# deep-art-project/Music

Measured on AMD Instinct MI355X. Metric: audio samples/sec trained (whole node), 30-layer WaveNet @16kHz, higher is better.
Workload: dtype f32 (forward + recompute: f16 2-term split operands, 2^-22 per element; backward products: bf16 2-term split, 2^-17 per element, f32 range; 3 MFMA per product, f32 accumulate)

## Files before the change

### include/wavenet_hip.h

```cpp
#ifndef WAVENET_HIP_H
#define WAVENET_HIP_H
#include <stdint.h>
#ifdef __cplusplus
extern "C" {
#endif

typedef void* wn_stream_t;
enum { WN_F16X3 = 0, WN_F16X1 = 1, WN_BF16X3 = 2, WN_BF16X1 = 3 };
#define WN_ABI_VERSION 9
#define WN_CE_NUM_PARTIALS 1024
#define WN_GUARD_NUM_PARTIALS 256
#define WN_GUARD_PARTIALS_BYTES (WN_GUARD_NUM_PARTIALS * 12)
#define WN_GUARD_STATE_BYTES 48

int wn_version(void);
const char* wn_last_error(void);

int wn_pack_weights(const float* flat, const int32_t* idx, uint16_t* out, int n, int mode,
                    wn_stream_t stream);

int wn_chan_gemm(const float* in0, const float* in1, int64_t in_bstride, int in_pitch, int in_lo, int in_hi,
                 int shift0, int shift1, int ks0, int ks1, const uint16_t* wpack, int mt, int m_valid,
                 float* out, int64_t out_bstride, int out_pitch, int out_shift, const float* bias,
                 const float* resid, int64_t resid_bstride, int resid_pitch, int resid_lo,
                 const float* mask, int64_t mask_bstride, int mask_pitch,
                 int t_lo, int t_hi, int relu_in, int batch, int mode, wn_stream_t stream);

int wn_resblock_fwd(const float* x_in, float* x_out, float* z_out, int64_t x_bstride, int64_t z_bstride,
                    int pitch, const uint16_t* wfg, const uint16_t* wd, const float* bias_f,
                    const float* bias_g, const float* bias_d, int n_f, int n_d, int ch, int d,
                    int t_lo, int t_hi, int z_lo, int write_x, const float* cond, int64_t cond_bstride,
                    int cond_pitch, int cond_mode, int cond_le, int cond_q, const uint16_t* cond_pack,
                    int64_t cond_pack_bstride, const uint8_t* cond_idx, int64_t z_half_stride, int batch, int mode,
                    wn_stream_t stream);

int wn_resblock_bwd(const float* x_in, const float* dy, const float* dz, float* dfg, float* z,
                    int64_t x_bstride, int64_t dz_bstride, int64_t dfg_bstride, int64_t z_bstride,
                    int pitch, const uint16_t* wfg, const uint16_t* wdT, const float* bias_f,
                    const float* bias_g, int n_f, int ch, int d, int t_lo, int t_hi, int z_lo,
                    const float* cond, int64_t cond_bstride, int cond_pitch, int cond_mode, int cond_le, int cond_q,
                    int batch, int mode_fwd, int mode_bwd, wn_stream_t stream);

int wn_skip_epilogue_fwd(const float* z, int64_t z_bstride, int pitch, int ks_skip, const uint16_t* w_skip, const float* bias_skip,
                         float* u, float* h, int64_t s_bstride, const uint16_t* w_p1c, const float* bias_p1,
                         const uint16_t* w_p2c, const float* bias_p2, float* o, int64_t o_bstride, int o_pitch,
                         int s_valid, int q_valid, int t_lo, int t_hi, int batch, int mode, wn_stream_t stream);

int wn_skip_epilogue_bwd(const float* d_o, int64_t o_bstride, int o_pitch, const float* h, const float* u, int64_t s_bstride, int pitch,
                         float* d_h, float* d_u, float* d_z, int64_t z_bstride, const uint16_t* w_p2T, const uint16_t* w_p1Tc,
                         const uint16_t* w_skipTc, int mt_z, int z_valid, int s_valid, int t_lo, int t_hi, int batch, int mode,
                         wn_stream_t stream);

int wn_enc_resblock_fwd(const float* x_in, float* x_out, float* h_out, int64_t x_bstride, int64_t h_bstride, int pitch,
                        const uint16_t* wdil, const uint16_t* wd, const float* bias_dil, const float* bias_d, int n_h,
                        int n_d, int ch, int d, int t_lo, int t_hi, int batch, int mode, wn_stream_t stream);

int wn_enc_resblock_bwd(const float* x_in, const float* dy, const float* h, float* dh, int64_t x_bstride,
                        int64_t h_bstride, int64_t dh_bstride, int pitch, const uint16_t* wdT, int ch, int d, int t_lo,
                        int t_hi, int y_lo, float* slab_dil, float* slab_d, int batch, int mode_bwd, wn_stream_t stream);
int wn_enc_resblock_bwd_slabs(int t_lo, int t_hi, int batch);
int wn_enc_resblock_bwd_pq(const float* x_in, const float* p_in, const float* q_in, int dn, int p_lo, const float* h,
                           float* p_out, float* q_out, int64_t x_bstride, int64_t h_bstride, int pitch, const uint16_t* wdT,
                           const uint16_t* wpq, int ch, int d, int t_lo, int t_hi, float* slab_dil, float* slab_d, int chain,
                           int batch, int mode_bwd, wn_stream_t stream);

int wn_resblock_bwd_ms(const float* x_in, const float* dy, const float* dz, float* dfg, int64_t x_bstride,
                       int64_t dz_bstride, int64_t dfg_bstride, int pitch, const uint16_t* wfg, const uint16_t* wdT,
                       const float* bias_f, const float* bias_g, int n_f, int ch, int d, int t_lo, int t_hi, int z_lo,
                       float* slab_fg, float* slab_d, const float* cond, int64_t cond_bstride, int cond_pitch,
                       int cond_mode, int cond_le, int cond_q, int batch, int mode_fwd, int mode_bwd,
                       wn_stream_t stream);
int wn_resblock_bwd_ms_slabs(int t_lo, int t_hi, int batch);

#define WN_COND_IDX_PAD 64
int wn_resblock_bwd_pq(const float* x_in, const float* p_in, const float* q_in, int dn, int p_lo, const float* dz,
                       float* p_out, float* q_out, int64_t x_bstride, int64_t dz_bstride, int pitch, const uint16_t* wfg,
                       const uint16_t* wdT, const uint16_t* wpq, int ch, int d, int t_lo, int t_hi, int z_lo,
                       float* slab_fg, float* slab_d, const float* cond, int64_t cond_bstride, int cond_pitch, int cond_le,
                       const uint8_t* cond_idx, float* cslab, int64_t dz_half_stride, int chain, int batch, int mode_fwd,
                       int mode_bwd, wn_stream_t stream);
int wn_resblock_bwd_pq_chain_ok(int t_lo, int t_hi, int batch, int d);
int wn_resblock_bwd_pq_slabs(int t_lo, int t_hi, int batch, int d, int chain);
int wn_resblock_bwd_pq_chain_items(int t_lo, int t_hi, int batch, int d, int wg, int* out, int cap);
int wn_resblock_bwd_pq_cond_floats(int t_lo, int t_hi, int batch);
int wn_resblock_bwd_pq_cond_reduce(const float* cslab, const int64_t* slab_off, const int* t_lo, int n_launches, int t_hi, int batch,
                                   int cond_le, float* out, int64_t out_lstride, int64_t out_bstride, int out_pitch,
                                   wn_stream_t stream);
int wn_gate_fwd(const float* fg, int64_t fg_bstride, int dp, int rows, float* z, int64_t z_bstride, int pitch, int t_lo, int t_hi,
                int batch, wn_stream_t stream);
int wn_gate_bwd(const float* fg, int64_t fg_bstride, int dp, int rows, const float* dz, int64_t dz_bstride, float* dfg,
                int64_t dfg_bstride, int pitch, int t_lo, int t_hi, int batch, wn_stream_t stream);
int wn_chunk_softmax_fwd(const float* x, float* y, int64_t nrows, int q, wn_stream_t stream);
int wn_chunk_softmax_bwd(const float* y, const float* dy, float* dx, int64_t nrows, int q, wn_stream_t stream);
int wn_chunk_softmax_ce(const float* x, const int64_t* target, float* probs, float* dx, float* loss_part, int64_t nrows, int q,
                        float inv_n, wn_stream_t stream);
int wn_split16(const float* x, uint16_t* hi, uint16_t* lo, int64_t n, int is_bf16, wn_stream_t stream);
int wn_shift_add(const float* p, const float* q, float* out, int64_t bstride, int pitch, int rows, int dn, int p_lo,
                 int t_lo, int t_hi, int batch, wn_stream_t stream);

int wn_wgrad(const float* a, int64_t a_bstride, int a_pitch, int a_shift, int a_cols,
             const float* b0, const float* b1, int64_t b_bstride, int b_pitch, int b_shift0,
             int b_shift1, int b_cols, int nt_per_tap, int mt, int relu_b, float* c, int ldc,
             int64_t c_slab_stride, int t_lo, int t_hi, int chunk, int batch, int mode, wn_stream_t stream);
int wn_wgrad_slabs(int t_lo, int t_hi, int chunk, int batch);
int wn_causal_wgrad_codes(const int32_t* codes, int scrambled, const float* dx, const float* dx_q, int dn, int p_lo,
                          int64_t dx_bstride, int pitch, int ch, int q, int t, int batch, float* slab, wn_stream_t stream);
int wn_causal_wgrad_codes_slabs(int t, int batch);
int wn_causal_fwd_codes(const int32_t* codes, int scrambled, const float* wt, const float* bias, int n_rows, float* x0,
                        int64_t x_bstride, int pitch, int ch, int q, int t, int batch, wn_stream_t stream);
int wn_reduce_slabs(const int64_t* desc, int n_ops, int64_t total_vec, const float* slab, float* out,
                    wn_stream_t stream);

int wn_bias_grad(const float* a, int64_t a_bstride, int a_pitch, int a_shift, int rows, int t_lo,
                 int t_hi, int batch, float* out, wn_stream_t stream);

int wn_chunk_softmax256_fwd(const float* x, float* y, int64_t nrows, wn_stream_t stream);
int wn_chunk_softmax256_bwd(const float* y, const float* dy, float* dx, int64_t nrows, wn_stream_t stream);
int wn_chunk_softmax256_ce(const float* x, const int64_t* target, float* probs, float* dx,
                           float* loss_part, int64_t nrows, float inv_n, wn_stream_t stream);

int wn_adam_flat(float* p, const float* g, float* m, float* v, int64_t n, float lr, float beta1,
                 float beta2, float eps, float bias_corr1, float bias_corr2, float gscale,
                 wn_stream_t stream);
int wn_sgd_flat(float* p, const float* g, float* momentum_buf, int64_t n, float lr, float momentum, float gscale,
                int first_step, wn_stream_t stream);
int wn_rmsprop_flat(float* p, const float* g, float* square_avg, float* momentum_buf, int64_t n, float lr, float alpha,
                    float eps, float momentum, float gscale, wn_stream_t stream);
typedef struct wn_guard_state {
    float norm;
    float coef;
    uint32_t nonfinite;
    uint32_t skip;
    uint64_t n_taken;
    uint64_t n_clipped;
    uint64_t n_skipped;
    float bc1;
    float bc2;
} wn_guard_state;
int wn_grad_guard(const float* g, int64_t n, float gscale, float max_norm, int skip_nonfinite, float beta1, float beta2,
                  void* partials, wn_guard_state* state, wn_stream_t stream);
int wn_adam_flat_guarded(float* p, const float* g, float* m, float* v, int64_t n, float lr, float beta1, float beta2, float eps,
                         float gscale, const wn_guard_state* state, wn_stream_t stream);
int wn_sgd_flat_guarded(float* p, const float* g, float* momentum_buf, int64_t n, float lr, float momentum, float gscale,
                        const wn_guard_state* state, wn_stream_t stream);
int wn_rmsprop_flat_guarded(float* p, const float* g, float* square_avg, float* momentum_buf, int64_t n, float lr, float alpha,
                            float eps, float momentum, float gscale, const wn_guard_state* state, wn_stream_t stream);
int wn_ema_flat(float* ema, const float* p, int64_t n, float decay, int warmup, int64_t t, const wn_guard_state* state,
                wn_stream_t stream);
int wn_step_softmax(const float* x, int64_t x_bstride, int x_pitch, float* probs, int w, int q, int batch, wn_stream_t stream);
int wn_step_nll(const float* x, int64_t x_bstride, int x_pitch, const int64_t* target, float* dx, int64_t dx_bstride, int dx_pitch,
                float* probs, float* row_nll, int32_t* row_hit, float* loss_part, int w, int q, int batch, float inv_n,
                wn_stream_t stream);
int wn_win_step_softmax(const float* x, int64_t x_bstride, int x_pitch, float* probs, int w, int q, int batch, const int32_t* win_host,
                        int win_period, const int64_t* win_pos, int64_t win_pos0, wn_stream_t stream);
int wn_win_step_nll(const float* x, int64_t x_bstride, int x_pitch, const int64_t* target, float* dx, int64_t dx_bstride, int dx_pitch,
                    float* probs, float* row_nll, int32_t* row_hit, float* loss_part, int w, int q, int batch, float inv_n,
                    const int32_t* win_host, int win_period, const int64_t* win_pos, int64_t win_pos0, wn_stream_t stream);
int wn_cond_proj_fwd(const float* enc, const float* flat, int64_t w_off, int64_t b_off, int64_t stage_stride, int64_t wf_off,
                     int64_t bf_off, float* tab, float* tab_pair, float* enf, int n_stages, int dd, int ch, int sd, int bw, int le,
                     int batch, wn_stream_t stream);
int wn_cond_proj_bwd(const float* d_tab, int pair, const float* d_enf, const float* enc, const float* flat, int64_t w_off,
                     int64_t b_off, int64_t stage_stride, int64_t wf_off, int64_t bf_off, float* d_enc, float* flat_grad,
                     int n_stages, int dd, int ch, int sd, int bw, int le, int batch, wn_stream_t stream);
#define WN_GCOND_MAX_CHANNELS 512
int wn_gcond_proj_fwd(const float* enc, const float* flat, int64_t w_off, int64_t b_off, int64_t stage_stride, int64_t wf_off,
                      int64_t bf_off, float* tab, float* tab_pair, float* enf, int n_stages, int dd, int ch, int sd, int bw, int le,
                      int batch, const int32_t* cls, int64_t gw_off, int64_t gstage_stride, int64_t gwf_off, int64_t emb_off, int ge,
                      int n_cls, wn_stream_t stream);
int wn_gcond_proj_bwd(const float* d_tab, int pair, const float* d_enf, const float* enc, const float* flat, int64_t w_off,
                      int64_t b_off, int64_t stage_stride, int64_t wf_off, int64_t bf_off, float* d_enc, float* flat_grad,
                      int n_stages, int dd, int ch, int sd, int bw, int le, int batch, const int32_t* cls, int64_t gw_off,
                      int64_t gstage_stride, int64_t gwf_off, int64_t emb_off, int ge, int n_cls, wn_stream_t stream);
#define WN_VQ_NUM_PARTIALS 256
#define WN_VQ_MAX_CODES 1024
#define WN_VQ_MAX_WIDTH 512
int wn_vq_fwd(const float* enc, const float* flat, int64_t cb_off, float* q_out, int32_t* idx, int32_t* counts, float* loss_part, int K,
              int bw, int le, int batch, wn_stream_t stream);
int wn_vq_bwd(const float* enc, const int32_t* idx, const float* d_q, const float* flat, int64_t cb_off, float beta, float g_scale,
              float* d_enc, float* flat_grad, int K, int bw, int le, int batch, wn_stream_t stream);
int wn_vq_lookup(const int32_t* idx, const float* flat, int64_t cb_off, float* q_out, int32_t* bad, int K, int bw, int le, int batch,
                 wn_stream_t stream);
#define WN_VQ_EMA_WORK_BYTES 4112
int wn_vq_bwd_stats(const float* enc, const int32_t* idx, const float* d_q, const float* flat, int64_t cb_off, float beta, float g_scale,
                    float* d_enc, float* flat_grad, float* stat, int K, int bw, int le, int batch, wn_stream_t stream);
int wn_vq_ema_update(float* flat, int64_t cb_off, const float* stat, float* state, void* work, int32_t* info, int K, int bw,
                     float decay, float eps, float restart, const wn_guard_state* guard_state, wn_stream_t stream);
#define WN_RVQ_MAX_STAGES 8
int wn_rvq_fwd(const float* enc, const float* flat, int64_t cb_off, float* q_out, int32_t* idx, int32_t* counts, float* res,
               float* loss_part, int S, int K, int bw, int le, int batch, wn_stream_t stream);
int wn_rvq_bwd(const float* enc, const int32_t* idx, const float* res, const float* d_q, const float* flat, int64_t cb_off, float beta,
               float g_scale, float* d_enc, float* flat_grad, int S, int K, int bw, int le, int batch, wn_stream_t stream);
int wn_rvq_bwd_stats(const float* enc, const int32_t* idx, const float* res, const float* d_q, const float* flat, int64_t cb_off, float beta,
                     float g_scale, float* d_enc, float* flat_grad, float* stat, int S, int K, int bw, int le, int batch,
                     wn_stream_t stream);
int wn_rvq_ema_update(float* flat, int64_t cb_off, const float* stat, float* state, void* work, int32_t* info, int S, int K, int bw,
                      float decay, float eps, float restart, const wn_guard_state* guard_state, wn_stream_t stream);
int wn_rvq_lookup(const int32_t* idx, const float* flat, int64_t cb_off, float* q_out, int32_t* bad, int S, int stages, int K, int bw,
                  int le, int batch, wn_stream_t stream);
int wn_rvq_fwd_n(const float* enc, const float* flat, int64_t cb_off, const int32_t* nstage, float* q_out, int32_t* idx, int32_t* counts,
                 float* res, float* loss_part, int S, int K, int bw, int le, int batch, wn_stream_t stream);
int wn_rvq_bwd_n(const float* enc, const int32_t* idx, const float* res, const int32_t* nstage, const float* d_q, const float* flat,
                 int64_t cb_off, float beta, float g_scale, float* d_enc, float* flat_grad, int S, int K, int bw, int le, int batch,
                 wn_stream_t stream);
int wn_rvq_bwd_stats_n(const float* enc, const int32_t* idx, const float* res, const int32_t* nstage, const float* d_q, const float* flat,
                       int64_t cb_off, float beta, float g_scale, float* d_enc, float* flat_grad, float* stat, int S, int K, int bw, int le,
                       int batch, wn_stream_t stream);
int wn_rvq_lookup_n(const int32_t* idx, const int32_t* nstage, const float* flat, int64_t cb_off, float* q_out, int32_t* bad, int S, int K,
                    int bw, int le, int batch, wn_stream_t stream);
int wn_coll_available(void);
int wn_comm_unique_id(char* id128);
int wn_comm_create(int nranks, int rank, const char* id128, void** comm);
int wn_comm_destroy(void* comm);
int wn_allreduce_flat(void* comm, float* buf, int64_t n, wn_stream_t stream);
int wn_gather_grads(const float* packed, const int32_t* idx, float* flat_grad, int n, wn_stream_t stream);
int wn_gather_grads2(const float* packed, const int32_t* idx, const int32_t* idx2, float* flat_grad, int n, wn_stream_t stream);

int wn_cond_expand(const float* tab, int64_t tab_bstride, int tab_pitch, int rows, int t_lo, int t_hi, int mode, int le, int q,
                   float* out, int64_t out_bstride, int out_pitch, int batch, wn_stream_t stream);
int wn_cond_grad(const float* in, int64_t in_bstride, int in_pitch, int rows, int t_lo, int t_hi, int mode, int le,
                 int q, float* out, int64_t out_bstride, int out_pitch, int batch, wn_stream_t stream);
int wn_avgpool_bwd(const float* denc, int64_t denc_bstride, int denc_pitch, int t0, int pool, int n_out, int rows,
                   float* out, int64_t out_bstride, int out_pitch, int t_hi, int batch, wn_stream_t stream);

int wn_avgpool(const float* in, int64_t in_bstride, int in_pitch, int t0, int pool, int n_out, int rows,
               float* out, int64_t out_bstride, int out_pitch, int batch, wn_stream_t stream);

int wn_onehot(const int32_t* codes, float* out, int batch, int q, int t, int scrambled, wn_stream_t stream);

int wn_mulaw_encode_tbl(const float* audio, const float* thresholds, uint8_t* codes, int64_t n, wn_stream_t stream);
int wn_mulaw_decode_lut(const uint8_t* codes, const float* table, float* audio, int64_t n, wn_stream_t stream);
int wn_mulaw_encode_q(const float* audio, const float* thresholds, int q, int32_t* codes, int64_t n, wn_stream_t stream);
int wn_mulaw_decode_q(const int32_t* codes, const float* table, int q, float* audio, int64_t n, wn_stream_t stream);

int wn_decode(int n_layers, int R, int D, int S, int Q, const int32_t* dilations_host, const int64_t* q_off_host,
              float* queues, const float* w_causal, const float* b_causal, const float* w_layers,
              int64_t layer_stride, const float* b_layers, const float* w_p1, const float* b_p1,
              const float* w_p2, const float* b_p2, const float* note0, const float* prev0, float* note_out,
              float* prev_out, const int32_t* forced, int32_t* codes_out, float* probs_out, int64_t step0,
              int n_steps, int push_input, uint64_t* sync, wn_stream_t stream);

int wn_decode_batch(int n_layers, int R, int D, int S, int Q, const int32_t* dilations_host, const int64_t* q_off_host,
                    float* queues, const float* w_causal, const float* b_causal, const float* w_layers,
                    int64_t layer_stride, const float* b_layers, const float* w_p1, const float* b_p1,
                    const float* w_p2, const float* b_p2, const float* note0, const float* prev0, float* note_out,
                    float* prev_out, const int32_t* forced, int32_t* codes_out, float* probs_out, int64_t step0,
                    int n_steps, int push_input, uint64_t* sync, int n_utt, int64_t queues_ustride, float temperature,
                    uint64_t seed, wn_stream_t stream);
int64_t wn_decode_sync_granules(int n_layers, int D, int S);
int wn_decode_batch_pk(int n_layers, int R, int D, int S, int Q, const int32_t* dilations_host, const int64_t* q_off_host,
                       float* queues, const float* w_causal, const float* b_causal, const float* w_layers,
                       int64_t layer_stride, const float* b_layers, const float* w_p1, const float* b_p1,
                       const float* w_p2, const float* b_p2, const float* note0, const float* prev0, float* note_out,
                       float* prev_out, const int32_t* forced, int32_t* codes_out, float* probs_out, int64_t step0,
                       int n_steps, int push_input, uint64_t* sync, int n_utt, int64_t queues_ustride, float temperature,
                       uint64_t seed, const uint16_t* pk, int64_t pk_fg0, int64_t pk_d0, int64_t pk_lstride, int64_t pk_skip,
                       int64_t pk_p1, int64_t pk_p2, wn_stream_t stream);
int wn_decode_batch_fw(int filter_width, int n_layers, int R, int D, int S, int Q, const int32_t* dilations_host,
                       const int64_t* q_off_host, float* queues, const float* w_causal, const float* b_causal,
                       const float* w_layers, int64_t layer_stride, const float* b_layers, const float* w_p1, const float* b_p1,
                       const float* w_p2, const float* b_p2, const float* note0, const float* prev0, float* note_out,
                       float* prev_out, const int32_t* forced, int32_t* codes_out, float* probs_out, int64_t step0,
                       int n_steps, int push_input, uint64_t* sync, int n_utt, int64_t queues_ustride, float temperature,
                       uint64_t seed, const uint16_t* pk, int64_t pk_fg0, int64_t pk_d0, int64_t pk_lstride, int64_t pk_skip,
                       int64_t pk_p1, int64_t pk_p2, wn_stream_t stream);
// ... 48 lines not shown
```

### music_amd/_lib.py

```python
import ctypes
import os

_HERE = os.path.dirname(os.path.abspath(__file__))
LIB_PATH = os.environ.get("WAVENET_HIP_LIB") or os.path.join(_HERE, "libwavenet_hip.so")

F16X3, F16X1, BF16X3, BF16X1 = 0, 1, 2, 3
MODE_NAMES = {"f16x3": F16X3, "f16x1": F16X1, "bf16x3": BF16X3, "bf16x1": BF16X1}
CE_NUM_PARTIALS = 1024
ABI_VERSION = 9
GUARD_NUM_PARTIALS = 256
GUARD_PARTIALS_BYTES = GUARD_NUM_PARTIALS * 12
VQ_NUM_PARTIALS = 256
VQ_MAX_CODES, VQ_MAX_WIDTH = 1024, 512
VQ_EMA_WORK_BYTES = 16 + 4 * VQ_MAX_CODES
RVQ_MAX_STAGES = 8
GCOND_MAX_CHANNELS = 512

_p = ctypes.c_void_p
_i = ctypes.c_int
_l = ctypes.c_int64
_f = ctypes.c_float
_DEC_HEAD = [_i] * 5 + [_p] * 6 + [_l] + [_p] * 12 + [_l, _i, _i, _p]
_DEC_BATCH = [_i, _l, _f, _l]
_DEC_PK = [_p] + [_l] * 6
_DEC_COND = [_p, _l, _p, _l, _p, _p, _i, _l]
_DEC_SAMP = [_p, _i, _f]
_DEC_WIN = [_p, _i, _l]
_SAMPLE_LOGITS = [_p, _l, _i, _l, _p, _f, _l, _i, _f, _l, _p, _p, _p]

SIGNATURES = {
    "wn_version": [],
    "wn_pack_weights": [_p, _p, _p, _i, _i, _p],
    "wn_chan_gemm": [_p, _p, _l, _i, _i, _i, _i, _i, _i, _i, _p, _i, _i,
                     _p, _l, _i, _i, _p,
                     _p, _l, _i, _i,
                     _p, _l, _i,
                     _i, _i, _i, _i, _i, _p],
    "wn_skip_epilogue_fwd": [_p, _l, _i, _i, _p, _p, _p, _p, _l, _p, _p, _p, _p, _p, _l, _i, _i, _i, _i, _i, _i, _i, _p],
    "wn_skip_epilogue_bwd": [_p, _l, _i, _p, _p, _l, _i, _p, _p, _p, _l, _p, _p, _p, _i, _i, _i, _i, _i, _i, _i, _p],
    "wn_resblock_fwd": [_p, _p, _p, _l, _l, _i, _p, _p, _p, _p, _p, _i, _i, _i, _i,
                        _i, _i, _i, _i, _p, _l, _i, _i, _i, _i, _p, _l, _p, _l, _i, _i, _p],
    "wn_enc_resblock_fwd": [_p, _p, _p, _l, _l, _i, _p, _p, _p, _p, _i, _i, _i, _i, _i, _i, _i, _i, _p],
    "wn_enc_resblock_bwd": [_p, _p, _p, _p, _l, _l, _l, _i, _p, _i, _i, _i, _i, _i, _p, _p, _i, _i, _p],
    "wn_enc_resblock_bwd_slabs": [_i, _i, _i],
    "wn_enc_resblock_bwd_pq": [_p, _p, _p, _i, _i, _p, _p, _p, _l, _l, _i, _p, _p, _i, _i, _i, _i, _p, _p, _i, _i, _i, _p],
    "wn_avgpool": [_p, _l, _i, _i, _i, _i, _i, _p, _l, _i, _i, _p],
    "wn_resblock_bwd": [_p, _p, _p, _p, _p, _l, _l, _l, _l, _i, _p, _p, _p, _p, _i, _i, _i, _i, _i, _i,
                        _p, _l, _i, _i, _i, _i, _i, _i, _i, _p],
    "wn_cond_expand": [_p, _l, _i, _i, _i, _i, _i, _i, _i, _p, _l, _i, _i, _p],
    "wn_cond_grad": [_p, _l, _i, _i, _i, _i, _i, _i, _i, _p, _l, _i, _i, _p],
    "wn_avgpool_bwd": [_p, _l, _i, _i, _i, _i, _i, _p, _l, _i, _i, _i, _p],
    "wn_wgrad": [_p, _l, _i, _i, _i, _p, _p, _l, _i, _i, _i, _i, _i, _i, _i, _p, _i,
                 _l, _i, _i, _i, _i, _i, _p],
    "wn_wgrad_slabs": [_i, _i, _i, _i],
    "wn_resblock_bwd_ms": [_p, _p, _p, _p, _l, _l, _l, _i, _p, _p, _p, _p, _i, _i, _i, _i, _i, _i, _p, _p,
                           _p, _l, _i, _i, _i, _i, _i, _i, _i, _p],
    "wn_resblock_bwd_ms_slabs": [_i, _i, _i],
    "wn_resblock_bwd_pq": [_p, _p, _p, _i, _i, _p, _p, _p, _l, _l, _i, _p, _p, _p, _i, _i, _i, _i, _i, _p, _p,
                           _p, _l, _i, _i, _p, _p, _l, _i, _i, _i, _i, _p],
    "wn_resblock_bwd_pq_chain_ok": [_i, _i, _i, _i],
    "wn_resblock_bwd_pq_slabs": [_i, _i, _i, _i, _i],
    "wn_resblock_bwd_pq_chain_items": [_i, _i, _i, _i, _i, _p, _i],
    "wn_resblock_bwd_pq_cond_floats": [_i, _i, _i],
    "wn_resblock_bwd_pq_cond_reduce": [_p, _p, _p, _i, _i, _i, _i, _p, _l, _l, _i, _p],
    "wn_split16": [_p, _p, _p, _l, _i, _p],
    "wn_shift_add": [_p, _p, _p, _l, _i, _i, _i, _i, _i, _i, _i, _p],
    "wn_causal_wgrad_codes": [_p, _i, _p, _p, _i, _i, _l, _i, _i, _i, _i, _i, _p, _p],
    "wn_causal_wgrad_codes_slabs": [_i, _i],
    "wn_causal_fwd_codes": [_p, _i, _p, _p, _i, _p, _l, _i, _i, _i, _i, _i, _p],
    "wn_reduce_slabs": [_p, _i, _l, _p, _p, _p],
    "wn_bias_grad": [_p, _l, _i, _i, _i, _i, _i, _i, _p, _p],
    "wn_chunk_softmax256_fwd": [_p, _p, _l, _p],
    "wn_chunk_softmax256_bwd": [_p, _p, _p, _l, _p],
    "wn_chunk_softmax256_ce": [_p, _p, _p, _p, _p, _l, _f, _p],
    "wn_gate_fwd": [_p, _l, _i, _i, _p, _l, _i, _i, _i, _i, _p],
    "wn_gate_bwd": [_p, _l, _i, _i, _p, _l, _p, _l, _i, _i, _i, _i, _p],
    "wn_chunk_softmax_fwd": [_p, _p, _l, _i, _p],
    "wn_chunk_softmax_bwd": [_p, _p, _p, _l, _i, _p],
    "wn_chunk_softmax_ce": [_p, _p, _p, _p, _p, _l, _i, _f, _p],
    "wn_adam_flat": [_p, _p, _p, _p, _l, _f, _f, _f, _f, _f, _f, _f, _p],
    "wn_sgd_flat": [_p, _p, _p, _l, _f, _f, _f, _i, _p],
    "wn_rmsprop_flat": [_p, _p, _p, _p, _l, _f, _f, _f, _f, _f, _p],
    "wn_grad_guard": [_p, _l, _f, _f, _i, _f, _f, _p, _p, _p],
    "wn_adam_flat_guarded": [_p, _p, _p, _p, _l, _f, _f, _f, _f, _f, _p, _p],
    "wn_sgd_flat_guarded": [_p, _p, _p, _l, _f, _f, _f, _p, _p],
    "wn_rmsprop_flat_guarded": [_p, _p, _p, _p, _l, _f, _f, _f, _f, _f, _p, _p],
    "wn_ema_flat": [_p, _p, _l, _f, _i, _l, _p, _p],
    "wn_step_softmax": [_p, _l, _i, _p, _i, _i, _i, _p],
    "wn_step_nll": [_p, _l, _i, _p, _p, _l, _i, _p, _p, _p, _p, _i, _i, _i, _f, _p],
    "wn_win_step_softmax": [_p, _l, _i, _p, _i, _i, _i, _p, _i, _p, _l, _p],
    "wn_win_step_nll": [_p, _l, _i, _p, _p, _l, _i, _p, _p, _p, _p, _i, _i, _i, _f, _p, _i, _p, _l, _p],
    "wn_cond_proj_fwd": [_p, _p, _l, _l, _l, _l, _l, _p, _p, _p, _i, _i, _i, _i, _i, _i, _i, _p],
    "wn_cond_proj_bwd": [_p, _i, _p, _p, _p, _l, _l, _l, _l, _l, _p, _p, _i, _i, _i, _i, _i, _i, _i, _p],
    "wn_gcond_proj_fwd": [_p, _p, _l, _l, _l, _l, _l, _p, _p, _p, _i, _i, _i, _i, _i, _i, _i, _p, _l, _l, _l, _l, _i, _i, _p],
    "wn_gcond_proj_bwd": [_p, _i, _p, _p, _p, _l, _l, _l, _l, _l, _p, _p, _i, _i, _i, _i, _i, _i, _i, _p, _l, _l, _l, _l, _i, _i, _p],
    "wn_vq_fwd": [_p, _p, _l, _p, _p, _p, _p, _i, _i, _i, _i, _p],
    "wn_vq_bwd": [_p, _p, _p, _p, _l, _f, _f, _p, _p, _i, _i, _i, _i, _p],
    "wn_vq_lookup": [_p, _p, _l, _p, _p, _i, _i, _i, _i, _p],
    "wn_vq_bwd_stats": [_p, _p, _p, _p, _l, _f, _f, _p, _p, _p, _i, _i, _i, _i, _p],
    "wn_vq_ema_update": [_p, _l, _p, _p, _p, _p, _i, _i, _f, _f, _f, _p, _p],
    "wn_rvq_fwd": [_p, _p, _l, _p, _p, _p, _p, _p, _i, _i, _i, _i, _i, _p],
    "wn_rvq_bwd": [_p, _p, _p, _p, _p, _l, _f, _f, _p, _p, _i, _i, _i, _i, _i, _p],
    "wn_rvq_bwd_stats": [_p, _p, _p, _p, _p, _l, _f, _f, _p, _p, _p, _i, _i, _i, _i, _i, _p],
    "wn_rvq_ema_update": [_p, _l, _p, _p, _p, _p, _i, _i, _i, _f, _f, _f, _p, _p],
    "wn_rvq_lookup": [_p, _p, _l, _p, _p, _i, _i, _i, _i, _i, _i, _p],
    "wn_rvq_fwd_n": [_p, _p, _l, _p, _p, _p, _p, _p, _p, _i, _i, _i, _i, _i, _p],
    "wn_rvq_bwd_n": [_p, _p, _p, _p, _p, _p, _l, _f, _f, _p, _p, _i, _i, _i, _i, _i, _p],
    "wn_rvq_bwd_stats_n": [_p, _p, _p, _p, _p, _p, _l, _f, _f, _p, _p, _p, _i, _i, _i, _i, _i, _p],
    "wn_rvq_lookup_n": [_p, _p, _p, _l, _p, _p, _i, _i, _i, _i, _i, _p],
    "wn_coll_available": [],
    "wn_comm_unique_id": [_p],
    "wn_comm_create": [_i, _i, _p, _p],
    "wn_comm_destroy": [_p],
    "wn_allreduce_flat": [_p, _p, _l, _p],
    "wn_gather_grads": [_p, _p, _p, _i, _p],
    "wn_gather_grads2": [_p, _p, _p, _p, _i, _p],
    "wn_onehot": [_p, _p, _i, _i, _i, _i, _p],
    "wn_mulaw_encode_tbl": [_p, _p, _p, _l, _p],
    "wn_mulaw_decode_lut": [_p, _p, _p, _l, _p],
    "wn_mulaw_encode_q": [_p, _p, _i, _p, _l, _p],
    "wn_mulaw_decode_q": [_p, _p, _i, _p, _l, _p],
    "wn_decode": _DEC_HEAD + [_p],
    "wn_decode_batch": _DEC_HEAD + _DEC_BATCH + [_p],
    "wn_decode_sync_granules": [_i, _i, _i],
    "wn_decode_batch_pk": _DEC_HEAD + _DEC_BATCH + _DEC_PK + [_p],
    "wn_decode_batch_fw": [_i] + _DEC_HEAD + _DEC_BATCH + _DEC_PK + [_p],
    "wn_decode_batch_cond": [_i] + _DEC_HEAD + _DEC_BATCH + _DEC_PK + _DEC_COND + [_p],
    "wn_decode_batch_samp": [_i] + _DEC_HEAD + _DEC_BATCH + _DEC_PK + _DEC_COND + _DEC_SAMP + [_p],
    "wn_sample_logits": _SAMPLE_LOGITS + [_p],
    "wn_win_decode_batch": [_i] + _DEC_HEAD + _DEC_BATCH + _DEC_PK + _DEC_COND + _DEC_SAMP + _DEC_WIN + [_p],
    "wn_win_sample_logits": _SAMPLE_LOGITS + _DEC_WIN + [_p],
}


class Sampling(ctypes.Structure):
    _fields_ = [("temperature", ctypes.c_float), ("top_p", ctypes.c_float), ("top_k", ctypes.c_int32),
                ("stream", ctypes.c_uint32), ("seed", ctypes.c_uint64)]


class GuardState(ctypes.Structure):
    _fields_ = [("norm", ctypes.c_float), ("coef", ctypes.c_float), ("nonfinite", ctypes.c_uint32), ("skip", ctypes.c_uint32),
                ("n_taken", ctypes.c_uint64), ("n_clipped", ctypes.c_uint64), ("n_skipped", ctypes.c_uint64),
                ("bc1", ctypes.c_float), ("bc2", ctypes.c_float)]


_lib = None


class WavenetHipError(RuntimeError):
    pass


def cpu_quota():
    try:
        q, per = open("/sys/fs/cgroup/cpu.max").read().split()[:2]
        return None if q == "max" else max(1, -(-int(q) // int(per)))
    except (OSError, ValueError):
        pass
    try:
        q = int(open("/sys/fs/cgroup/cpu/cpu.cfs_quota_us").read())
        per = int(open("/sys/fs/cgroup/cpu/cpu.cfs_period_us").read())
        return None if q <= 0 else max(1, -(-q // per))
    except (OSError, ValueError):
        return None


class StepThrottle:

    def __init__(self):
        self.depth = int(os.environ.get("WN_MAX_STEPS_IN_FLIGHT", "4"))
        self._ev = []

    def enter(self):
        if self.depth > 0 and len(self._ev) >= self.depth:
            self._ev.pop(0).synchronize()

    def leave(self):
        if self.depth > 0:
            import torch
            ev = torch.cuda.Event()
            ev.record()
            self._ev.append(ev)


def local_world_size(env=None):
    env = os.environ if env is None else env
    try:
        return max(1, int(env.get("LOCAL_WORLD_SIZE", "1")))
    except ValueError:
        return 1


def thread_budget(quota, local_world, cpus=None):
    total = quota if quota is not None else (cpus if cpus is not None else (os.cpu_count() or 1))
    return max(1, -(-int(total) // max(1, int(local_world))))


def respect_cpu_quota():
    import sys
    import torch
    if os.environ.get("WN_KEEP_TORCH_THREADS", "0") == "1":
        return
    q, lw = cpu_quota(), local_world_size()
    if q is None and lw == 1:
        return
    n = thread_budget(q, lw)
    if torch.get_num_threads() > n:
        print("music_amd: torch intra-op threads %d -> %d (%s shared by %d rank(s) of this host; WN_KEEP_TORCH_THREADS=1 keeps torch's "
              "own setting)" % (torch.get_num_threads(), n, "the container's CPU quota of %d" % q if q is not None else
                                "%d CPUs" % (os.cpu_count() or 1), lw), file=sys.stderr)
        torch.set_num_threads(n)


def load():
    global _lib
    if _lib is not None:
        return _lib
    if not os.path.exists(LIB_PATH):
        raise WavenetHipError(
            "libwavenet_hip.so not found at %s - build it with `python -c 'import __graft_entry__ as g; "
            "g.build()'` or `make -C music_amd/csrc`; there is no CPU fallback" % LIB_PATH)
    import torch
    lib = ctypes.CDLL(LIB_PATH)
    for name, args in SIGNATURES.items():
        try:
            fn = getattr(lib, name)
        except AttributeError:
            raise WavenetHipError("%s does not export %s: it was built from older sources - rebuild it (`make -C music_amd/csrc`)"
                                  % (LIB_PATH, name)) from None
        fn.argtypes = args
        fn.restype = ctypes.c_int
    lib.wn_decode_sync_granules.restype = ctypes.c_int64
    lib.wn_last_error.argtypes = []
    lib.wn_last_error.restype = ctypes.c_char_p
    if lib.wn_version() != ABI_VERSION:
        raise WavenetHipError("libwavenet_hip.so ABI version %d != expected %d" % (lib.wn_version(), ABI_VERSION))
    _lib = lib
    respect_cpu_quota()
    return lib


def wgrad_slabs(t_lo, t_hi, chunk, batch):
    return load().wn_wgrad_slabs(t_lo, t_hi, chunk, batch)


def causal_codes_slabs(t, batch):
    return load().wn_causal_wgrad_codes_slabs(t, batch)


COND_IDX_PAD = 64


def ms_slabs(t_lo, t_hi, batch):
    return load().wn_resblock_bwd_ms_slabs(t_lo, t_hi, batch)


def pq_chain_ok(t_lo, t_hi, batch, d):
    return bool(load().wn_resblock_bwd_pq_chain_ok(t_lo, t_hi, batch, d))


def pq_slabs(t_lo, t_hi, batch, d, chain):
    return load().wn_resblock_bwd_pq_slabs(t_lo, t_hi, batch, d, 1 if chain else 0)


def enc_slabs(t_lo, t_hi, batch):
    return load().wn_enc_resblock_bwd_slabs(t_lo, t_hi, batch)


def decode_sync_granules(n_layers, D, S):
    return int(load().wn_decode_sync_granules(n_layers, D, S))


def call(name, *args):
    lib = load()
    rc = getattr(lib, name)(*args)
    if rc != 0:
        raise WavenetHipError("%s failed (%d): %s" % (name, rc, lib.wn_last_error().decode()))


def ptr(t, offset=0):
    if t is None:
        return None
    return t.data_ptr() + offset * t.element_size()


def stream():
    import torch
    return torch.cuda.current_stream().cuda_stream


_side_streams = {}


def side_stream(device):
    import os
    import torch
    dev = torch.device(device)
    key = dev.index if dev.index is not None else torch.cuda.current_device()
    st = _side_streams.get(key)
    if st is None:
        st = _side_streams[key] = torch.cuda.Stream(device=dev, priority=-1)
    return st
```

### music_amd/csrc/wn_api.hip

```cpp
#include <stdio.h>
#include <stdlib.h>
#include <string.h>
#include "../../include/wavenet_hip.h"
#include "wn_common.h"
#include "wn_kernels.h"

static_assert(WN_COND_IDX_PAD == WN_PQ_IDX_PAD, "public and kernel-side pad of the bucket bytes differ");
static thread_local char g_err[512] = "";

int wn_set_error(hipError_t e, const char* file, int line) {
    snprintf(g_err, sizeof(g_err), "HIP error %d (%s) at %s:%d", (int)e, hipGetErrorString(e), file, line);
    return -1;
}
int wn_tile_origin(int t_lo) { return t_lo & ~63; }

int wn_num_cus() {
    static std::atomic<int> cus{0};
    int v = cus.load(std::memory_order_relaxed);
    if (v > 0) return v;
    int dev = 0;
    hipDeviceProp_t pr;
    if (hipGetDevice(&dev) != hipSuccess || hipGetDeviceProperties(&pr, dev) != hipSuccess || pr.multiProcessorCount <= 0) return 256;
    cus.store(pr.multiProcessorCount, std::memory_order_relaxed);
    return pr.multiProcessorCount;
}

int wn_xcd_swizzle_enabled() { return 1; }

int wn_set_error_msg(int code, const char* msg) {
    snprintf(g_err, sizeof(g_err), "%s", msg);
    return code;
}

static int wn_null_error(const char* fn, const char* names, int which) {
    const char* b = names;
    for (int i = 0; i < which && *b; ++b)
        if (*b == ',') ++i;
    while (*b == ' ') ++b;
    int len = 0;
    while (b[len] && b[len] != ',') ++len;
    snprintf(g_err, sizeof(g_err), "%s: argument '%.*s' must not be NULL", fn, len, b);
    return -4;
}
#define WN_REQUIRE(fn, ...)                                                          \
    do {                                                                             \
        const void* wn_req_[] = {__VA_ARGS__};                                       \
        for (int wn_i_ = 0; wn_i_ < (int)(sizeof(wn_req_) / sizeof(wn_req_[0])); ++wn_i_) \
            if (!wn_req_[wn_i_]) return wn_null_error(fn, #__VA_ARGS__, wn_i_);      \
    } while (0)

static_assert(WN_F16X3 == WN_MODE_F16X3 && WN_F16X1 == WN_MODE_F16X1 && WN_BF16X3 == WN_MODE_BF16X3 &&
              WN_BF16X1 == WN_MODE_BF16X1, "mode enums out of sync");
static_assert(WN_CE_NUM_PARTIALS == WN_CE_PARTIALS, "partials out of sync");
static_assert(WN_VQ_NUM_PARTIALS == WN_VQ_PARTIALS && WN_VQ_MAX_CODES == WN_DEC_MAX_Q, "vq constants out of sync");
static_assert(WN_VQ_MAX_CODES == WN_VQ_MAX_K && WN_VQ_EMA_WORK_BYTES == WN_VQ_EMA_WORK, "vq ema constants out of sync");
static_assert(WN_RVQ_MAX_STAGES == WN_RVQ_MAX_S, "rvq constants out of sync");

enum : unsigned {
    DEC_FW = 1,
    DEC_COND = 2,
    DEC_SAMP = 4,
    DEC_WIN = 8,
};

static int decode_refuse(const char* fn, const char* text) {
    snprintf(g_err, sizeof(g_err), "%s: %s", fn, text);
    return -4;
}

static int win_checked(const char* fn, const int32_t* win_host, int win_period, int64_t win_pos0, int Q, int& period, int& pos0,
                       int (&lo)[WN_WIN_MAX], int (&hi)[WN_WIN_MAX]) {
    if (win_period < 0 || win_period > WN_WIN_MAX) return decode_refuse(fn, "'win_period' must be 0 (no windows) .. 16 pairs");
    if (win_period > 0 && !win_host) return decode_refuse(fn, "'win_host' is NULL with win_period > 0");
    for (int j = 0; j < win_period; ++j)
        if (win_host[2 * j] < 0 || win_host[2 * j + 1] > Q || win_host[2 * j] >= win_host[2 * j + 1]) {
            snprintf(g_err, sizeof(g_err), "%s: 'win_host' pair %d is (%d, %d): every window needs 0 <= lo < hi <= Q", fn, j,
                     (int)win_host[2 * j], (int)win_host[2 * j + 1]);
            return -4;
        }
    if (win_pos0 < 0) return decode_refuse(fn, "'win_pos0' (stream position of the first step) must be >= 0");
    period = win_period;
    pos0 = win_period > 0 ? (int)(win_pos0 % win_period) : 0;
    for (int j = 0; j < win_period; ++j) { lo[j] = win_host[2 * j]; hi[j] = win_host[2 * j + 1]; }
    return 0;
}

static int decode_checked(const char* fn, unsigned checks, int64_t sync_ustride, int filter_width, int n_layers, int R, int D, int S,
                          int Q, const int32_t* dilations_host, const int64_t* q_off_host, float* queues, const float* w_causal,
                          const float* b_causal, const float* w_layers, int64_t layer_stride, const float* b_layers,
                          const float* w_p1, const float* b_p1, const float* w_p2, const float* b_p2, const float* note0,
                          const float* prev0, float* note_out, float* prev_out, const int32_t* forced, int32_t* codes_out,
                          float* probs_out, int64_t step0, int n_steps, int push_input, uint64_t* sync, int n_utt,
                          int64_t queues_ustride, float temperature, uint64_t seed, const uint16_t* pk, int64_t pk_fg0,
                          int64_t pk_d0, int64_t pk_lstride, int64_t pk_skip, int64_t pk_p1, int64_t pk_p2, const float* cond_fg,
                          int64_t cond_fg_ustride, const float* cond_p1, int64_t cond_p1_ustride, const int32_t* c_shift_host,
                          const int32_t* c_q_host, int le, int64_t pos0, const wn_sampling* samp, int top_k, float top_p,
                          const int32_t* win_host, int win_period, int64_t win_pos0, wn_stream_t stream) {
    const bool layers_ok = n_layers >= 1 && n_layers <= WN_DEC_MAX_LAYERS;
    if ((checks & DEC_SAMP) && !samp) {
        if (!(top_p >= 0.0f)) return decode_refuse(fn, "'top_p' must be a number >= 0 (0 or >= 1: no nucleus filter)");
        if (top_k < 0) return decode_refuse(fn, "'top_k' must be >= 0 (0 or >= Q: no top-k filter)");
    }
    if ((checks & DEC_FW) && filter_width < 1) return decode_refuse(fn, "filter_width must be >= 1");
    if (!push_input) {
        if (checks & DEC_COND) return decode_refuse(fn, "conditioned decode exists for the corrected recurrence only; pass push_input = 1");
        if ((checks & DEC_FW) && filter_width != 2)
            return decode_refuse(fn, "the as-written queue push (push_input = 0) exists for filter_width 2 only; pass push_input = 1 "
                                     "(the corrected recurrence)");
    }
    if ((checks & DEC_COND) && le < 1) return decode_refuse(fn, "le (columns of a conditioning table) must be >= 1");
    if ((checks & DEC_FW) && (Q < 1 || Q > WN_DEC_MAX_Q)) return decode_refuse(fn, "1 <= Q <= 1024 quantisation channels");
    if (checks & DEC_COND) {
        if (!layers_ok) return decode_refuse(fn, "1..64 layers supported");
        if (cond_fg || cond_p1) {
            if (!c_shift_host || !c_q_host)
                return decode_refuse(fn, "a conditioning table needs the schedule arrays 'c_shift_host' and 'c_q_host' (n_layers + 1 "
                                         "entries each)");
            for (int i = 0; i <= n_layers; ++i)
                if (c_q_host[i] < 0) return decode_refuse(fn, "c_q[i] must be >= 0 (stretch factor, or 0 = tile)");
        }
    }
    if ((checks & DEC_FW) && n_utt > 0 && n_steps > 0) {
        WN_REQUIRE(fn, note0, note_out, codes_out);
        if (filter_width > 1) WN_REQUIRE(fn, prev0, prev_out);
    }
    WnDecodeArgs a;
    memset(&a, 0, sizeof(a));
    if (checks & DEC_WIN) {
        const int rc = win_checked(fn, win_host, win_period, win_pos0, Q, a.win_period, a.win_pos0, a.win_lo, a.win_hi);
        if (rc) return rc;
    }
    if (n_utt <= 0) return 0;
    if (!layers_ok) return decode_refuse("wn_decode", "1..64 layers supported");
    WN_REQUIRE("wn_decode", dilations_host, q_off_host);
    if (n_steps > 0) WN_REQUIRE("wn_decode", queues, w_causal, w_layers, w_p1, w_p2, sync);
    a.n_layers = n_layers; a.R = R; a.D = D; a.S = S; a.Q = Q; a.fw = filter_width;
    for (int i = 0; i < n_layers; ++i) { a.dil[i] = dilations_host[i]; a.q_off[i] = q_off_host[i]; }
    a.queues = queues; a.w_causal = w_causal; a.b_causal = b_causal; a.w_layers = w_layers; a.layer_stride = layer_stride;
    a.b_layers = b_layers; a.w_p1 = w_p1; a.b_p1 = b_p1; a.w_p2 = w_p2; a.b_p2 = b_p2;
    a.note0 = note0; a.prev0 = prev0; a.note_out = note_out; a.prev_out = prev_out; a.forced = forced;
    a.codes_out = codes_out; a.probs_out = probs_out; a.step0 = step0; a.n_steps = n_steps; a.push_input = push_input;
    a.dbg = 0;
    a.sync = reinterpret_cast<unsigned long long*>(sync);
    a.sync_ustride = sync_ustride;
    a.n_utt = n_utt; a.queues_ustride = queues_ustride;
    a.sample = temperature > 0.0f ? 1 : 0; a.inv_temp = temperature > 0.0f ? 1.0f / temperature : 1.0f; a.seed = seed;
    a.samp = reinterpret_cast<const WnSampling*>(samp); a.top_k = top_k; a.top_p = top_p;
    a.pk_skip = -1;
    a.cond_fg = cond_fg; a.cond_fg_ustride = cond_fg_ustride; a.cond_p1 = cond_p1; a.cond_p1_ustride = cond_p1_ustride;
    a.le = le; a.pos0 = pos0;
    if (cond_fg || cond_p1)
        for (int i = 0; i <= n_layers; ++i) { a.c_shift[i] = c_shift_host[i]; a.c_q[i] = c_q_host[i]; }
    const bool any_bias = b_layers || b_causal || b_p1 || b_p2;
    const bool post_pk = (S == 256 || S == 512) && Q == 256 && pk_skip >= 0 && pk_p1 >= 0 && pk_p2 >= 0;
    if (pk && R == 64 && D == 64 && (post_pk || !any_bias)) {
        a.pk = pk; a.pk_fg0 = pk_fg0; a.pk_d0 = pk_d0; a.pk_lstride = pk_lstride;
        if (post_pk) { a.pk_skip = pk_skip; a.pk_p1 = pk_p1; a.pk_p2 = pk_p2; }
    }
    return wn_launch_decode(a, (hipStream_t)stream);
}

static int sample_checked(const char* fn, bool win, const float* logits, int64_t n, int Q, int64_t ld, const wn_sampling* samp,
                          float temperature, uint64_t seed, int top_k, float top_p, int64_t step0, const float* u, int32_t* codes,
                          float* probs, const int32_t* win_host, int win_period, int64_t win_pos0, wn_stream_t stream) {
    if (Q < 1 || Q > WN_DEC_MAX_Q) return decode_refuse(fn, "1 <= 'Q' <= 1024 entries per row");
    if (n < 0) return decode_refuse(fn, "'n' (rows) must be >= 0");
    if (ld < Q) return decode_refuse(fn, "'ld' (row stride) must be >= Q");
    if (!samp) {
        if (!(top_p >= 0.0f)) return decode_refuse(fn, "'top_p' must be a number >= 0 (0 or >= 1: no nucleus filter)");
        if (top_k < 0) return decode_refuse(fn, "'top_k' must be >= 0 (0 or >= Q: no top-k filter)");
    }
    WnWin w;
    memset(&w, 0, sizeof(w));
    if (win) {
        const int rc = win_checked(fn, win_host, win_period, win_pos0, Q, w.period, w.pos0, w.lo, w.hi);
        if (rc) return rc;
    }
    if (n == 0) return 0;
    WN_REQUIRE(fn, logits, codes);
    return wn_launch_sample_logits(logits, (long)n, Q, (long)ld, reinterpret_cast<const WnSampling*>(samp), temperature, seed, top_k,
                                   top_p, (long)step0, u, codes, probs, w, (hipStream_t)stream);
}

extern "C" {

int wn_version(void) { return WN_ABI_VERSION; }
const char* wn_last_error(void) { return g_err; }

int wn_pack_weights(const float* flat, const int32_t* idx, uint16_t* out, int n, int mode, wn_stream_t stream) {
    if (n % 512 != 0) return wn_set_error_msg(-4, "wn_pack_weights: n must be a multiple of 512");
    if (n > 0) WN_REQUIRE("wn_pack_weights", flat, idx, out);
    return wn_launch_pack(flat, idx, out, n, wn_mode_is_bf16(mode), wn_mode_ns(mode), (hipStream_t)stream);
}

int wn_chan_gemm(const float* in0, const float* in1, int64_t in_bstride, int in_pitch, int in_lo, int in_hi,
                 int shift0, int shift1, int ks0, int ks1, const uint16_t* wpack, int mt, int m_valid,
                 float* out, int64_t out_bstride, int out_pitch, int out_shift, const float* bias,
                 const float* resid, int64_t resid_bstride, int resid_pitch, int resid_lo,
                 const float* mask, int64_t mask_bstride, int mask_pitch,
                 int t_lo, int t_hi, int relu_in, int batch, int mode, wn_stream_t stream) {
    if (ks0 <= 0 || (ks1 > 0 && !in1) || mt <= 0) return wn_set_error_msg(-4, "wn_chan_gemm: bad shape");
    if (batch > 0 && t_hi > t_lo) WN_REQUIRE("wn_chan_gemm", in0, wpack, out);
    WnGemmArgs a;
    memset(&a, 0, sizeof(a));
    a.in0 = in0; a.in1 = ks1 > 0 ? in1 : nullptr; a.in_bstride = in_bstride; a.in_pitch = in_pitch; a.in_lo = in_lo; a.in_hi = in_hi;
    a.shift0 = shift0; a.shift1 = shift1; a.ks0 = ks0; a.ks1 = ks1 > 0 ? ks1 : 0; a.wpack = wpack; a.mt = mt; a.m_valid = m_valid;
    a.out = out; a.out_bstride = out_bstride; a.out_pitch = out_pitch; a.out_shift = out_shift; a.bias = bias;
    a.resid = resid; a.resid_bstride = resid_bstride; a.resid_pitch = resid_pitch; a.resid_lo = resid_lo;
    a.mask = mask; a.mask_bstride = mask_bstride; a.mask_pitch = mask_pitch;
    a.t_lo = t_lo; a.t_hi = t_hi; a.relu_in = relu_in;
    return wn_launch_gemm(a, batch, mode, (hipStream_t)stream);
}

int wn_skip_epilogue_fwd(const float* z, int64_t z_bstride, int pitch, int ks_skip, const uint16_t* w_skip, const float* bias_skip,
                         float* u, float* h, int64_t s_bstride, const uint16_t* w_p1c, const float* bias_p1,
                         const uint16_t* w_p2c, const float* bias_p2, float* o, int64_t o_bstride, int o_pitch,
                         int s_valid, int q_valid, int t_lo, int t_hi, int batch, int mode, wn_stream_t stream) {
    if (pitch % 4 != 0) return wn_set_error_msg(-4, "wn_skip_epilogue_fwd: pitch must be a multiple of 4");
    if (s_valid <= 0 || s_valid > 256 || q_valid <= 0 || q_valid > 256)
        return wn_set_error_msg(-4, "wn_skip_epilogue_fwd: at most 256 skip and 256 quantisation channels (wn_chan_gemm covers the rest)");
    if (batch > 0 && t_hi > t_lo) WN_REQUIRE("wn_skip_epilogue_fwd", z, w_skip, u, h, w_p1c, w_p2c, o);
    WnEpiFwdArgs a;
    memset(&a, 0, sizeof(a));
    a.z = z; a.z_bstride = z_bstride; a.pitch = pitch; a.ks_skip = ks_skip; a.w_skip = w_skip; a.bias_s = bias_skip;
    a.u = u; a.h = h; a.s_bstride = s_bstride; a.w_p1c = w_p1c; a.bias_1 = bias_p1; a.w_p2c = w_p2c; a.bias_2 = bias_p2;
    a.o = o; a.o_bstride = o_bstride; a.o_pitch = o_pitch; a.s_valid = s_valid; a.q_valid = q_valid; a.t_lo = t_lo; a.t_hi = t_hi;
    return wn_launch_skip_epilogue_fwd(a, batch, mode, (hipStream_t)stream);
}

int wn_skip_epilogue_bwd(const float* d_o, int64_t o_bstride, int o_pitch, const float* h, const float* u, int64_t s_bstride, int pitch,
                         float* d_h, float* d_u, float* d_z, int64_t z_bstride, const uint16_t* w_p2T, const uint16_t* w_p1Tc,
                         const uint16_t* w_skipTc, int mt_z, int z_valid, int s_valid, int t_lo, int t_hi, int batch, int mode,
                         wn_stream_t stream) {
    if (pitch % 4 != 0) return wn_set_error_msg(-4, "wn_skip_epilogue_bwd: pitch must be a multiple of 4");
    if (s_valid <= 0 || s_valid > 256) return wn_set_error_msg(-4, "wn_skip_epilogue_bwd: at most 256 skip channels");
    if (batch > 0 && t_hi > t_lo) WN_REQUIRE("wn_skip_epilogue_bwd", d_o, h, u, d_h, d_u, d_z, w_p2T, w_p1Tc, w_skipTc);
    WnEpiBwdArgs a;
    memset(&a, 0, sizeof(a));
    a.d_o = d_o; a.o_bstride = o_bstride; a.o_pitch = o_pitch; a.h = h; a.u = u; a.s_bstride = s_bstride; a.pitch = pitch;
    a.d_h = d_h; a.d_u = d_u; a.d_z = d_z; a.z_bstride = z_bstride; a.w_p2T = w_p2T; a.w_p1Tc = w_p1Tc; a.w_skipTc = w_skipTc;
    a.mt_z = mt_z; a.z_valid = z_valid; a.s_valid = s_valid; a.t_lo = t_lo; a.t_hi = t_hi;
    return wn_launch_skip_epilogue_bwd(a, batch, mode, (hipStream_t)stream);
}

int wn_enc_resblock_fwd(const float* x_in, float* x_out, float* h_out, int64_t x_bstride, int64_t h_bstride, int pitch,
                        const uint16_t* wdil, const uint16_t* wd, const float* bias_dil, const float* bias_d, int n_h,
                        int n_d, int ch, int d, int t_lo, int t_hi, int batch, int mode, wn_stream_t stream) {
    if (pitch % 4 != 0) return wn_set_error_msg(-4, "wn_enc_resblock_fwd: pitch must be a multiple of 4");
    if (t_lo < d + 1) return wn_set_error_msg(-4, "wn_enc_resblock_fwd: t_lo must be >= d + 1");
    if (batch > 0 && t_hi > t_lo) WN_REQUIRE("wn_enc_resblock_fwd", x_in, x_out, h_out, wdil, wd);
    WnResArgs a;
    memset(&a, 0, sizeof(a));
    a.x_in = x_in; a.x_out = x_out; a.z_out = h_out; a.x_bstride = x_bstride; a.z_bstride = h_bstride; a.pitch = pitch;
    a.wfg = wdil; a.wd = wd; a.bias_f = bias_dil; a.bias_g = nullptr; a.bias_d = bias_d; a.n_f = n_h; a.n_d = n_d;
    a.d = d; a.t_lo = t_lo; a.t_hi = t_hi; a.z_lo = t_lo; a.write_x = 1;
    return wn_launch_enc_resblock_fwd(a, ch, batch, mode, (hipStream_t)stream);
}

int wn_resblock_fwd(const float* x_in, float* x_out, float* z_out, int64_t x_bstride, int64_t z_bstride,
                    int pitch, const uint16_t* wfg, const uint16_t* wd, const float* bias_f,
                    const float* bias_g, const float* bias_d, int n_f, int n_d, int ch, int d,
                    int t_lo, int t_hi, int z_lo, int write_x, const float* cond, int64_t cond_bstride,
                    int cond_pitch, int cond_mode, int cond_le, int cond_q, const uint16_t* cond_pack,
                    int64_t cond_pack_bstride, const uint8_t* cond_idx, int64_t z_half_stride, int batch, int mode,
                    wn_stream_t stream) {
    if (pitch % 4 != 0) return wn_set_error_msg(-4, "wn_resblock_fwd: pitch must be a multiple of 4");
    if (cond && (cond_le <= 0 || (cond_mode == 1 && cond_q <= 0) || (cond_mode != 1 && cond_mode != 2)))
        return wn_set_error_msg(-4, "wn_resblock_fwd: bad conditioning arguments");
    if (t_lo < d + 1) return wn_set_error_msg(-4, "wn_resblock_fwd: t_lo must be >= d + 1");
    if (batch > 0 && t_hi > t_lo) {
        WN_REQUIRE("wn_resblock_fwd", x_in, wfg, wd, z_out);
        if (write_x) WN_REQUIRE("wn_resblock_fwd", x_out);
    }
    WnResArgs a;
    memset(&a, 0, sizeof(a));
    a.x_in = x_in; a.x_out = x_out; a.z_out = z_out; a.x_bstride = x_bstride; a.z_bstride = z_bstride; a.pitch = pitch;
    a.wfg = wfg; a.wd = wd; a.bias_f = bias_f; a.bias_g = bias_g; a.bias_d = bias_d; a.n_f = n_f; a.n_d = n_d;
    a.d = d; a.t_lo = t_lo; a.t_hi = t_hi; a.z_lo = z_lo; a.write_x = write_x;
    a.cond = cond; a.cond_bstride = cond_bstride; a.cond_pitch = cond_pitch; a.cond_mode = cond_mode;
    a.cond_le = cond_le; a.cond_q = cond_q;
    if (cond && cond_pack && cond_idx) { a.cond_pack = cond_pack; a.cond_pack_bstride = cond_pack_bstride; a.cond_idx = cond_idx; }
    if (z_half_stride && ch != 64) return wn_set_error_msg(-4, "wn_resblock_fwd: z_half_stride is for two 32-channel clips on the 64-channel block");
    a.z_half = z_half_stride;
    return wn_launch_resblock_fwd(a, ch, batch, mode, (hipStream_t)stream);
}

int wn_resblock_bwd(const float* x_in, const float* dy, const float* dz, float* dfg, float* z,
                    int64_t x_bstride, int64_t dz_bstride, int64_t dfg_bstride, int64_t z_bstride,
                    int pitch, const uint16_t* wfg, const uint16_t* wdT, const float* bias_f,
                    const float* bias_g, int n_f, int ch, int d, int t_lo, int t_hi, int z_lo,
                    const float* cond, int64_t cond_bstride, int cond_pitch, int cond_mode, int cond_le, int cond_q,
                    int batch, int mode_fwd, int mode_bwd, wn_stream_t stream) {
    if (pitch % 4 != 0) return wn_set_error_msg(-4, "wn_resblock_bwd: pitch must be a multiple of 4");
    if (batch > 0 && t_hi > t_lo) {
        WN_REQUIRE("wn_resblock_bwd", x_in, dz, dfg, wfg);
        if (dy) WN_REQUIRE("wn_resblock_bwd", wdT);
    }
    WnResBwdArgs a;
    memset(&a, 0, sizeof(a));
    a.x_in = x_in; a.dy = dy; a.dz = dz; a.dfg = dfg; a.z = z;
    a.x_bstride = x_bstride; a.dz_bstride = dz_bstride; a.dfg_bstride = dfg_bstride; a.z_bstride = z_bstride; a.pitch = pitch;
    a.wfg = wfg; a.wdT = wdT; a.bias_f = bias_f; a.bias_g = bias_g; a.n_f = n_f;
    a.d = d; a.t_lo = t_lo; a.t_hi = t_hi; a.z_lo = z_lo;
    a.cond = cond; a.cond_bstride = cond_bstride; a.cond_pitch = cond_pitch; a.cond_mode = cond_mode;
    a.cond_le = cond_le; a.cond_q = cond_q;
    return wn_launch_resblock_bwd(a, ch, batch, mode_fwd, mode_bwd, (hipStream_t)stream);
}

int wn_wgrad(const float* a_, int64_t a_bstride, int a_pitch, int a_shift, int a_cols,
             const float* b0, const float* b1, int64_t b_bstride, int b_pitch, int b_shift0,
             int b_shift1, int b_cols, int nt_per_tap, int mt, int relu_b, float* c, int ldc,
             int64_t c_slab_stride, int t_lo, int t_hi, int chunk, int batch, int mode, wn_stream_t stream) {
    if (c_slab_stride < (int64_t)mt * 16 * ldc) return wn_set_error_msg(-4, "wn_wgrad: slab stride smaller than C");
    if (batch > 0 && t_hi > t_lo) WN_REQUIRE("wn_wgrad", a_, b0, c);
    WnWgradArgs a;
    memset(&a, 0, sizeof(a));
    a.a = a_; a.a_bstride = a_bstride; a.a_pitch = a_pitch; a.a_shift = a_shift; a.a_cols = a_cols;
    a.b0 = b0; a.b1 = b1; a.b_bstride = b_bstride; a.b_pitch = b_pitch; a.b_shift0 = b_shift0; a.b_shift1 = b_shift1; a.b_cols = b_cols;
    a.nt_per_tap = nt_per_tap; a.mt = mt; a.relu_b = relu_b; a.c = c; a.ldc = ldc; a.c_slab_stride = c_slab_stride;
    a.t_lo = t_lo; a.t_hi = t_hi; a.chunk = chunk;
    return wn_launch_wgrad(a, batch, mode, (hipStream_t)stream);
}

int wn_wgrad_slabs(int t_lo, int t_hi, int chunk, int batch) { return wn_wgrad_num_slabs(t_lo, t_hi, chunk, batch); }

int wn_reduce_slabs(const int64_t* desc, int n_ops, int64_t total_vec, const float* slab, float* out, wn_stream_t stream) {
    if (n_ops > 0 && total_vec > 0) WN_REQUIRE("wn_reduce_slabs", desc, slab, out);
    return wn_launch_reduce_slabs(reinterpret_cast<const long*>(desc), n_ops, total_vec, slab, out, (hipStream_t)stream);
}

int wn_bias_grad(const float* a, int64_t a_bstride, int a_pitch, int a_shift, int rows, int t_lo,
                 int t_hi, int batch, float* out, wn_stream_t stream) {
    if (batch > 0 && t_hi > t_lo && rows > 0) WN_REQUIRE("wn_bias_grad", a, out);
    return wn_launch_bias_grad(a, a_bstride, a_pitch, a_shift, rows, t_lo, t_hi, batch, out, (hipStream_t)stream);
}

int wn_chunk_softmax256_fwd(const float* x, float* y, int64_t nrows, wn_stream_t stream) {
    if (nrows > 0) WN_REQUIRE("wn_chunk_softmax256_fwd", x, y);
    return wn_launch_softmax_fwd(x, y, nrows, (hipStream_t)stream);
}
int wn_chunk_softmax256_bwd(const float* y, const float* dy, float* dx, int64_t nrows, wn_stream_t stream) {
    if (nrows > 0) WN_REQUIRE("wn_chunk_softmax256_bwd", y, dy, dx);
    return wn_launch_softmax_bwd(y, dy, dx, nrows, (hipStream_t)stream);
}
int wn_chunk_softmax256_ce(const float* x, const int64_t* target, float* probs, float* dx,
                           float* loss_part, int64_t nrows, float inv_n, wn_stream_t stream) {
    if (nrows > 0) WN_REQUIRE("wn_chunk_softmax256_ce", x, target);
    return wn_launch_softmax_ce(x, target, probs, dx, loss_part, nrows, inv_n, (hipStream_t)stream);
}
int wn_adam_flat(float* p, const float* g, float* m, float* v, int64_t n, float lr, float beta1,
                 float beta2, float eps, float bias_corr1, float bias_corr2, float gscale, wn_stream_t stream) {
    if (n > 0) WN_REQUIRE("wn_adam_flat", p, g, m, v);
    return wn_launch_adam(p, g, m, v, n, lr, beta1, beta2, eps, bias_corr1, bias_corr2, gscale, (hipStream_t)stream);
}
int wn_sgd_flat(float* p, const float* g, float* momentum_buf, int64_t n, float lr, float momentum, float gscale, int first_step,
                wn_stream_t stream) {
    if (momentum != 0.f && !momentum_buf) return wn_set_error_msg(-4, "wn_sgd_flat: momentum needs its buffer");
    if (n > 0) WN_REQUIRE("wn_sgd_flat", p, g);
    return wn_launch_sgd(p, g, momentum_buf, n, lr, momentum, gscale, first_step, (hipStream_t)stream);
}
int wn_rmsprop_flat(float* p, const float* g, float* square_avg, float* momentum_buf, int64_t n, float lr, float alpha, float eps,
                    float momentum, float gscale, wn_stream_t stream) {
    if (!square_avg || (momentum > 0.f && !momentum_buf)) return wn_set_error_msg(-4, "wn_rmsprop_flat: missing state buffer");
    if (n > 0) WN_REQUIRE("wn_rmsprop_flat", p, g);
    return wn_launch_rmsprop(p, g, square_avg, momentum_buf, n, lr, alpha, eps, momentum, gscale, (hipStream_t)stream);
}

int wn_grad_guard(const float* g, int64_t n, float gscale, float max_norm, int skip_nonfinite, float beta1, float beta2, void* partials,
                  wn_guard_state* state, wn_stream_t stream) {
    WN_REQUIRE("wn_grad_guard", partials, state);
    if (n > 0) WN_REQUIRE("wn_grad_guard", g);
    if (n < 0) return wn_set_error_msg(-4, "wn_grad_guard: n is negative");
    if (((uintptr_t)g & 3) || ((uintptr_t)partials & 7) || ((uintptr_t)state & 7))
        return wn_set_error_msg(-4, "wn_grad_guard: g needs 4-byte, partials and state 8-byte alignment");
    return wn_launch_grad_guard(g, n, gscale, max_norm, skip_nonfinite, beta1, beta2, partials, state, (hipStream_t)stream);
}
int wn_adam_flat_guarded(float* p, const float* g, float* m, float* v, int64_t n, float lr, float beta1, float beta2, float eps,
                         float gscale, const wn_guard_state* state, wn_stream_t stream) {
    if (n > 0) WN_REQUIRE("wn_adam_flat_guarded", p, g, m, v, state);
    return wn_launch_adam_guarded(p, g, m, v, n, lr, beta1, beta2, eps, gscale, state, (hipStream_t)stream);
}
int wn_sgd_flat_guarded(float* p, const float* g, float* momentum_buf, int64_t n, float lr, float momentum, float gscale,
                        const wn_guard_state* state, wn_stream_t stream) {
    if (momentum != 0.f && !momentum_buf) return wn_set_error_msg(-4, "wn_sgd_flat_guarded: momentum needs its buffer");
    if (n > 0) WN_REQUIRE("wn_sgd_flat_guarded", p, g, state);
    return wn_launch_sgd_guarded(p, g, momentum_buf, n, lr, momentum, gscale, state, (hipStream_t)stream);
}
int wn_rmsprop_flat_guarded(float* p, const float* g, float* square_avg, float* momentum_buf, int64_t n, float lr, float alpha, float eps,
                            float momentum, float gscale, const wn_guard_state* state, wn_stream_t stream) {
    if (!square_avg || (momentum > 0.f && !momentum_buf)) return wn_set_error_msg(-4, "wn_rmsprop_flat_guarded: missing state buffer");
    if (n > 0) WN_REQUIRE("wn_rmsprop_flat_guarded", p, g, state);
    return wn_launch_rmsprop_guarded(p, g, square_avg, momentum_buf, n, lr, alpha, eps, momentum, gscale, state, (hipStream_t)stream);
}
int wn_ema_flat(float* ema, const float* p, int64_t n, float decay, int warmup, int64_t t, const wn_guard_state* state,
                wn_stream_t stream) {
    if (n < 0) return wn_set_error_msg(-4, "wn_ema_flat: n is negative");
    if (n == 0) return 0;
    WN_REQUIRE("wn_ema_flat", ema, p);
    if ((uintptr_t)ema % 4 != 0) return wn_set_error_msg(-4, "wn_ema_flat: argument 'ema' needs 4-byte alignment");
    if ((uintptr_t)p % 4 != 0) return wn_set_error_msg(-4, "wn_ema_flat: argument 'p' needs 4-byte alignment");
    if ((uintptr_t)state % 8 != 0) return wn_set_error_msg(-4, "wn_ema_flat: argument 'state' needs 8-byte alignment");
    if (!(decay >= 0.f && decay < 1.f)) return wn_set_error_msg(-4, "wn_ema_flat: argument 'decay' must lie in [0, 1)");
    if (!state && t < 1) return wn_set_error_msg(-4, "wn_ema_flat: argument 't' counts the updates from 1 when state is NULL");
    return wn_launch_ema(ema, p, n, decay, warmup ? 1 : 0, t, state, (hipStream_t)stream);
}
static int step_checked(const char* fn, const void* x, int64_t x_bstride, int x_pitch, int w, int q, int batch) {
    char msg[160];
    const char* bad = nullptr;
    if (batch < 0) bad = "'batch' must be >= 0";
    else if (w < 0) bad = "'w' must be >= 0";
    else if (q < 1 || q > 1024) bad = "'q' must lie in [1, 1024]";
    else if (x_pitch < w) bad = "'x_pitch' must be >= w";
    else if (x_bstride < (int64_t)q * x_pitch) bad = "'x_bstride' must be >= q * x_pitch";
    if (bad) {
        snprintf(msg, sizeof(msg), "%s: argument %s", fn, bad);
        return wn_set_error_msg(-4, msg);
    }
    if (batch > 0 && w > 0) WN_REQUIRE(fn, x);
    return 0;
}
int wn_step_softmax(const float* x, int64_t x_bstride, int x_pitch, float* probs, int w, int q, int batch, wn_stream_t stream) {
    if (int rc = step_checked("wn_step_softmax", x, x_bstride, x_pitch, w, q, batch)) return rc;
    if (batch == 0 || w == 0) return 0;
    WN_REQUIRE("wn_step_softmax", probs);
    return wn_launch_step_nll(x, (long)x_bstride, x_pitch, nullptr, nullptr, 0, 0, probs, nullptr, nullptr, nullptr, w, q, batch, 0.f,
                              nullptr, (hipStream_t)stream);
}
static int step_nll_checked(const char* fn, const float* x, int64_t x_bstride, int x_pitch, const int64_t* target, float* dx,
                            int64_t dx_bstride, int dx_pitch, float* probs, float* row_nll, int32_t* row_hit, float* loss_part, int w,
                            int q, int batch, float inv_n, const WnNllWin* win, wn_stream_t stream) {
    char msg[160];
    if (dx && dx_pitch < w) {
        snprintf(msg, sizeof(msg), "%s: argument 'dx_pitch' must be >= w", fn);
        return wn_set_error_msg(-4, msg);
    }
    if (dx && dx_bstride < (int64_t)q * dx_pitch) {
        snprintf(msg, sizeof(msg), "%s: argument 'dx_bstride' must be >= q * dx_pitch", fn);
        return wn_set_error_msg(-4, msg);
    }
    if (batch > 0 && w > 0) WN_REQUIRE(fn, target, loss_part);
    return wn_launch_step_nll(x, (long)x_bstride, x_pitch, target, dx, (long)dx_bstride, dx_pitch, probs, row_nll, row_hit, loss_part, w, q,
                              batch, inv_n, win, (hipStream_t)stream);
}
int wn_step_nll(const float* x, int64_t x_bstride, int x_pitch, const int64_t* target, float* dx, int64_t dx_bstride, int dx_pitch,
                float* probs, float* row_nll, int32_t* row_hit, float* loss_part, int w, int q, int batch, float inv_n,
                wn_stream_t stream) {
    if (int rc = step_checked("wn_step_nll", x, x_bstride, x_pitch, w, q, batch)) return rc;
    return step_nll_checked("wn_step_nll", x, x_bstride, x_pitch, target, dx, dx_bstride, dx_pitch, probs, row_nll, row_hit, loss_part, w,
                            q, batch, inv_n, nullptr, stream);
}
static int nll_win_checked(const char* fn, const int32_t* win_host, int win_period, const int64_t* win_pos, int64_t win_pos0, int q,
                           WnNllWin& win) {
    memset(&win, 0, sizeof(win));
    int pos0 = 0;
    if (int rc = win_checked(fn, win_host, win_period, win_pos0, q, win.period, pos0, win.lo, win.hi)) return rc;
    win.pos0 = (unsigned)pos0;
    win.pow32 = win_period > 0 ? (unsigned)((1ull << 32) % (unsigned)win_period) : 0;
    win.pos = win_pos;
    return 0;
}
int wn_win_step_softmax(const float* x, int64_t x_bstride, int x_pitch, float* probs, int w, int q, int batch, const int32_t* win_host,
                        int win_period, const int64_t* win_pos, int64_t win_pos0, wn_stream_t stream) {
    const char* fn = "wn_win_step_softmax";
    if (int rc = step_checked(fn, x, x_bstride, x_pitch, w, q, batch)) return rc;
    WnNllWin win;
    if (int rc = nll_win_checked(fn, win_host, win_period, win_pos, win_pos0, q, win)) return rc;
    if (batch == 0 || w == 0) return 0;
    WN_REQUIRE(fn, probs);
    return wn_launch_step_nll(x, (long)x_bstride, x_pitch, nullptr, nullptr, 0, 0, probs, nullptr, nullptr, nullptr, w, q, batch, 0.f,
                              &win, (hipStream_t)stream);
}
int wn_win_step_nll(const float* x, int64_t x_bstride, int x_pitch, const int64_t* target, float* dx, int64_t dx_bstride, int dx_pitch,
                    float* probs, float* row_nll, int32_t* row_hit, float* loss_part, int w, int q, int batch, float inv_n,
                    const int32_t* win_host, int win_period, const int64_t* win_pos, int64_t win_pos0, wn_stream_t stream) {
    const char* fn = "wn_win_step_nll";
    if (int rc = step_checked(fn, x, x_bstride, x_pitch, w, q, batch)) return rc;
    WnNllWin win;
    if (int rc = nll_win_checked(fn, win_host, win_period, win_pos, win_pos0, q, win)) return rc;
    return step_nll_checked(fn, x, x_bstride, x_pitch, target, dx, dx_bstride, dx_pitch, probs, row_nll, row_hit, loss_part, w, q, batch,
                            inv_n, &win, stream);
}
static int cond_proj_checked(const char* fn, int64_t w_off, int64_t b_off, int64_t stage_stride, int64_t wf_off, int64_t bf_off, int pair,
                             int n_stages, int dd, int ch, int sd, int bw, int le, int batch) {
    char msg[200];
    const char* bad = nullptr;
    if (batch < 0) bad = "'batch' must be >= 0";
    else if (n_stages < 1) bad = "'n_stages' must be >= 1";
    else if (dd < 1) bad = "'dd' must be >= 1";
    else if (sd < 1) bad = "'sd' must be >= 1";
    else if (bw < 1) bad = "'bw' must be >= 1";
    else if (le < 1) bad = "'le' must be >= 1";
    else if (ch < dd || ch % 32 != 0) bad = "'ch' must be a multiple of 32 and >= dd";
    else if (w_off < 0) bad = "'w_off' must be >= 0";
    else if (b_off < 0) bad = "'b_off' must be >= 0";
    else if (wf_off < 0) bad = "'wf_off' must be >= 0";
    else if (bf_off < 0) bad = "'bf_off' must be >= 0";
    else if (n_stages > 1 && stage_stride < (int64_t)2 * dd * bw) bad = "'stage_stride' must be >= 2 * dd * bw (the stages' weights overlap)";
    else if (pair && batch % 2 != 0) bad = "'batch' must be even for a table of clip pairs";
    if (bad) {
        snprintf(msg, sizeof(msg), "%s: argument %s", fn, bad);
        return wn_set_error_msg(-4, msg);
    }
// ... 570 lines not shown
```

### music_amd/csrc/wn_elem.hip

```cpp
#include "wn_common.h"
#include "wn_kernels.h"
#include "wn_optim.h"

__device__ __forceinline__ float wave_max(float v) {
#pragma unroll
    for (int o = 32; o > 0; o >>= 1) v = fmaxf(v, __shfl_xor(v, o, 64));
    return v;
}
__device__ __forceinline__ float wave_sum(float v) {
#pragma unroll
    for (int o = 32; o > 0; o >>= 1) v += __shfl_xor(v, o, 64);
    return v;
}

__global__ __launch_bounds__(256) void softmax256_fwd_k(const float* __restrict__ x, float* __restrict__ y, long nrows) {
    const int lane = threadIdx.x & 63;
    long row = (long)blockIdx.x * 4 + (threadIdx.x >> 6);
    const long stride = (long)gridDim.x * 4;
    for (; row < nrows; row += stride) {
        f32x4 v = ld4(x + row * 256 + lane * 4);
        float m = wave_max(fmaxf(fmaxf(v[0], v[1]), fmaxf(v[2], v[3])));
        f32x4 e = {expf(v[0] - m), expf(v[1] - m), expf(v[2] - m), expf(v[3] - m)};
        float s = wave_sum((e[0] + e[1]) + (e[2] + e[3]));
        float inv = 1.0f / s;
// ... 21 lines not shown
                                                                 float* __restrict__ probs, float* __restrict__ dx,
                                                                 float* __restrict__ loss_part, long nrows, float inv_n) {
    __shared__ float red[CE_WAVES];
    const int lane = threadIdx.x & 63;
    long row = (long)blockIdx.x * CE_WAVES + (threadIdx.x >> 6);
    const long stride = (long)gridDim.x * CE_WAVES;
    float lacc = 0.f;
    long rc = row < nrows ? row : nrows - 1;
    f32x4 v = ld4(x + rc * 256 + lane * 4);
    long y = target[rc];
    for (; row < nrows; row += stride) {
        const long rn = row + stride < nrows ? row + stride : nrows - 1;
        const f32x4 vn = ld4(x + rn * 256 + lane * 4);
        const long yn = target[rn];
        float m = wave_max(fmaxf(fmaxf(v[0], v[1]), fmaxf(v[2], v[3])));
        f32x4 e = {expf(v[0] - m), expf(v[1] - m), expf(v[2] - m), expf(v[3] - m)};
        float inv = 1.0f / wave_sum((e[0] + e[1]) + (e[2] + e[3]));
        f32x4 p = {e[0] * inv, e[1] * inv, e[2] * inv, e[3] * inv};
        if (probs) *reinterpret_cast<f32x4*>(probs + row * 256 + lane * 4) = p;
        f32x4 e2 = {expf(p[0]), expf(p[1]), expf(p[2]), expf(p[3])};
        float s2 = wave_sum((e2[0] + e2[1]) + (e2[2] + e2[3]));
        const bool bad = (unsigned long)y > 255ul;
        const int yl = (int)(y >> 2) & 63, ye = (int)y & 3;
        float py = __shfl(ye == 0 ? p[0] : ye == 1 ? p[1] : ye == 2 ? p[2] : p[3], yl, 64);
        lacc += bad ? __builtin_nanf("") : logf(s2) - py;
        if (dx) {
            float is2 = inv_n / s2;
            f32x4 dp = {e2[0] * is2, e2[1] * is2, e2[2] * is2, e2[3] * is2};
            if (lane == yl) dp[ye] -= inv_n;
            float dot = wave_sum((p[0] * dp[0] + p[1] * dp[1]) + (p[2] * dp[2] + p[3] * dp[3]));
            f32x4 r = {p[0] * (dp[0] - dot), p[1] * (dp[1] - dot), p[2] * (dp[2] - dot), p[3] * (dp[3] - dot)};
            if (bad) r = f32x4{__builtin_nanf(""), __builtin_nanf(""), __builtin_nanf(""), __builtin_nanf("")};
            *reinterpret_cast<f32x4*>(dx + row * 256 + lane * 4) = r;
        }
        v = vn;
        y = yn;
    }
    if (lane == 0) red[threadIdx.x >> 6] = lacc * inv_n;
    __syncthreads();
    if (threadIdx.x == 0 && loss_part) {
        float t = 0.f;
#pragma unroll
        for (int w = 0; w < CE_WAVES; ++w) t += red[w];
        loss_part[blockIdx.x] = t;
    }
}

static inline int sm_grid(long nrows) {
    long g = (nrows + 3) / 4;
    return (int)(g > 8192 ? 8192 : (g < 1 ? 1 : g));
}
int wn_launch_softmax_fwd(const float* x, float* y, long nrows, hipStream_t st) {
    if (nrows <= 0) return 0;
    hipLaunchKernelGGL(softmax256_fwd_k, dim3(sm_grid(nrows)), dim3(256), 0, st, x, y, nrows);
    WN_CHECK_LAUNCH();
    return 0;
}
int wn_launch_softmax_bwd(const float* y, const float* dy, float* dx, long nrows, hipStream_t st) {
    if (nrows <= 0) return 0;
    hipLaunchKernelGGL(softmax256_bwd_k, dim3(sm_grid(nrows)), dim3(256), 0, st, y, dy, dx, nrows);
    WN_CHECK_LAUNCH();
    return 0;
}
int wn_launch_softmax_ce(const float* x, const int64_t* target, float* probs, float* dx, float* loss_part,
                         long nrows, float inv_n, hipStream_t st) {
    if (nrows <= 0) return 0;
    hipLaunchKernelGGL(softmax256_ce_k, dim3(WN_CE_PARTIALS), dim3(64 * CE_WAVES), 0, st, x, target, probs, dx,
                       loss_part, nrows, inv_n);
    WN_CHECK_LAUNCH();
    return 0;
}

__global__ void shift_add_k(const float* __restrict__ p, const float* __restrict__ q, float* __restrict__ out,
                            long bstride, int pitch, int dn, int p_lo, int t_lo, int t_hi) {
    const int t = t_lo + blockIdx.x * blockDim.x + threadIdx.x;
    if (t >= t_hi) return;
    const size_t o = (size_t)blockIdx.z * bstride + (size_t)blockIdx.y * pitch + t;
    const float a = t >= p_lo ? p[o] : 0.f;
    const float b = t + dn < t_hi ? q[o + dn] : 0.f;
    out[o] = a + b;
}
int wn_launch_shift_add(const float* p, const float* q, float* out, long bstride, int pitch, int rows, int dn,
                        int p_lo, int t_lo, int t_hi, int batch, hipStream_t st) {
    if (t_hi <= t_lo || rows <= 0 || batch <= 0) return 0;
    hipLaunchKernelGGL(shift_add_k, dim3((t_hi - t_lo + 255) / 256, rows, batch), dim3(256), 0, st, p, q, out, bstride,
                       pitch, dn, p_lo, t_lo, t_hi);
    WN_CHECK_LAUNCH();
    return 0;
}

__global__ void adam_k(float* __restrict__ p, const float* __restrict__ g, float* __restrict__ m,
                       float* __restrict__ v, long n, float lr, float b1, float b2, float eps, float bc1,
                       float bc2, float gscale) {
    long i = (long)blockIdx.x * blockDim.x + threadIdx.x;
    const long stride = (long)gridDim.x * blockDim.x;
    wn_adam_body<false>(p, g, m, v, i, stride, n, lr, b1, b2, eps, bc1, bc2, gscale, 1.0f);
}
int wn_launch_adam(float* p, const float* g, float* m, float* v, long n, float lr, float b1, float b2,
                   float eps, float bc1, float bc2, float gscale, hipStream_t st) {
    if (n <= 0) return 0;
    long grid = (n + 255) / 256;
    if (grid > 2048) grid = 2048;
    hipLaunchKernelGGL(adam_k, dim3((int)grid), dim3(256), 0, st, p, g, m, v, n, lr, b1, b2, eps, bc1, bc2, gscale);
    WN_CHECK_LAUNCH();
    return 0;
}

__global__ void sgd_k(float* __restrict__ p, const float* __restrict__ g, float* __restrict__ buf, long n, float lr, float momentum,
                      float gscale, int first) {
    long i = (long)blockIdx.x * blockDim.x + threadIdx.x;
    const long stride = (long)gridDim.x * blockDim.x;
    wn_sgd_body<false>(p, g, buf, i, stride, n, lr, momentum, gscale, first, 1.0f);
}
int wn_launch_sgd(float* p, const float* g, float* buf, long n, float lr, float momentum, float gscale, int first, hipStream_t st) {
    if (n <= 0) return 0;
    long grid = (n + 255) / 256;
    if (grid > 2048) grid = 2048;
    hipLaunchKernelGGL(sgd_k, dim3((int)grid), dim3(256), 0, st, p, g, buf, n, lr, momentum, gscale, first);
    WN_CHECK_LAUNCH();
    return 0;
}
__global__ void rmsprop_k(float* __restrict__ p, const float* __restrict__ g, float* __restrict__ sq, float* __restrict__ buf, long n,
                          float lr, float alpha, float eps, float momentum, float gscale) {
    long i = (long)blockIdx.x * blockDim.x + threadIdx.x;
    const long stride = (long)gridDim.x * blockDim.x;
    wn_rmsprop_body<false>(p, g, sq, buf, i, stride, n, lr, alpha, eps, momentum, gscale, 1.0f);
}
int wn_launch_rmsprop(float* p, const float* g, float* sq, float* buf, long n, float lr, float alpha, float eps, float momentum,
                      float gscale, hipStream_t st) {
    if (n <= 0) return 0;
    long grid = (n + 255) / 256;
    if (grid > 2048) grid = 2048;
    hipLaunchKernelGGL(rmsprop_k, dim3((int)grid), dim3(256), 0, st, p, g, sq, buf, n, lr, alpha, eps, momentum, gscale);
    WN_CHECK_LAUNCH();
    return 0;
}

__global__ void gather_grads_k(const float* __restrict__ packed, const int32_t* __restrict__ idx,
                               float* __restrict__ flat, int n) {
    int i = blockIdx.x * blockDim.x + threadIdx.x;
    if (i < n) flat[i] = idx[i] >= 0 ? packed[idx[i]] : 0.f;
}
__global__ void gather_grads2_k(const float* __restrict__ packed, const int32_t* __restrict__ idx, const int32_t* __restrict__ idx2,
                                float* __restrict__ flat, int n) {
    int i = blockIdx.x * blockDim.x + threadIdx.x;
    if (i < n) flat[i] = (idx[i] >= 0 ? packed[idx[i]] : 0.f) + (idx2[i] >= 0 ? packed[idx2[i]] : 0.f);
}
int wn_launch_gather_grads2(const float* packed, const int32_t* idx, const int32_t* idx2, float* flat_grad, int n, hipStream_t st) {
    if (n <= 0) return 0;
    hipLaunchKernelGGL(gather_grads2_k, dim3((n + 255) / 256), dim3(256), 0, st, packed, idx, idx2, flat_grad, n);
    WN_CHECK_LAUNCH();
    return 0;
}
int wn_launch_gather_grads(const float* packed, const int32_t* idx, float* flat_grad, int n, hipStream_t st) {
    if (n <= 0) return 0;
    hipLaunchKernelGGL(gather_grads_k, dim3((n + 255) / 256), dim3(256), 0, st, packed, idx, flat_grad, n);
    WN_CHECK_LAUNCH();
    return 0;
}

__global__ void onehot_k(const int32_t* __restrict__ idx, float* __restrict__ out, int q, int t, int scrambled, long total) {
    long i = (long)blockIdx.x * blockDim.x + threadIdx.x;
    if (i >= total) return;
    long b = i / t, s = i % t;
    int code = idx[i];
    if (code < 0 || code >= q) return;
    long pos = scrambled ? (s * q + code) : ((long)code * t + s);
    out[b * (long)q * t + pos] = 1.0f;
}
int wn_launch_onehot(const int32_t* idx, float* out, int batch, int q, int t, int scrambled, hipStream_t st) {
    if (batch <= 0 || q <= 0 || t <= 0) return 0;
    long total = (long)batch * t;
    hipError_t e = hipMemsetAsync(out, 0, (size_t)total * q * sizeof(float), st);
    if (e != hipSuccess) return wn_set_error(e, __FILE__, __LINE__);
    hipLaunchKernelGGL(onehot_k, dim3((int)((total + 255) / 256)), dim3(256), 0, st, idx, out, q, t, scrambled, total);
    WN_CHECK_LAUNCH();
    return 0;
}

__global__ void mulaw_encode_k(const float* __restrict__ audio, const float* __restrict__ thr,
                               uint8_t* __restrict__ codes, long n) {
    __shared__ float s_thr[256];
    if (threadIdx.x < 255) s_thr[threadIdx.x] = thr[threadIdx.x];
    __syncthreads();
    long i = (long)blockIdx.x * blockDim.x + threadIdx.x;
    const long stride = (long)gridDim.x * blockDim.x;
    for (; i < n; i += stride) {
        float a = audio[i];
        int lo = 0, hi = 255;
        while (lo < hi) {
            int mid = (lo + hi) >> 1;
            if (s_thr[mid] <= a) lo = mid + 1; else hi = mid;
        }
        codes[i] = (uint8_t)lo;
    }
}
__global__ void mulaw_decode_k(const uint8_t* __restrict__ codes, const float* __restrict__ table,
                               float* __restrict__ audio, long n) {
    long i = (long)blockIdx.x * blockDim.x + threadIdx.x;
    const long stride = (long)gridDim.x * blockDim.x;
    for (; i < n; i += stride) audio[i] = table[codes[i]];
}
__global__ void mulaw_encode_q_k(const float* __restrict__ audio, const float* __restrict__ thr, int n_thr,
                                 int32_t* __restrict__ codes, long n) {
    long i = (long)blockIdx.x * blockDim.x + threadIdx.x;
    const long stride = (long)gridDim.x * blockDim.x;
    for (; i < n; i += stride) {
        const float a = audio[i];
        int lo = 0, hi = n_thr;
        while (lo < hi) {
            const int mid = (lo + hi) >> 1;
            if (thr[mid] <= a) lo = mid + 1; else hi = mid;
        }
        codes[i] = lo;
    }
}
__global__ void mulaw_decode_q_k(const int32_t* __restrict__ codes, const float* __restrict__ table, int q,
                                 float* __restrict__ audio, long n) {
    long i = (long)blockIdx.x * blockDim.x + threadIdx.x;
    const long stride = (long)gridDim.x * blockDim.x;
    for (; i < n; i += stride) {
        const int c = codes[i];
        audio[i] = table[c < 0 ? 0 : (c >= q ? q - 1 : c)];
    }
}
int wn_launch_mulaw_encode_q(const float* audio, const float* thr, int n_thr, int32_t* codes, long n, hipStream_t st) {
    if (n <= 0) return 0;
    long grid = (n + 255) / 256; if (grid > 2048) grid = 2048;
    hipLaunchKernelGGL(mulaw_encode_q_k, dim3((int)grid), dim3(256), 0, st, audio, thr, n_thr, codes, n);
    WN_CHECK_LAUNCH();
    return 0;
}
int wn_launch_mulaw_decode_q(const int32_t* codes, const float* table, int q, float* audio, long n, hipStream_t st) {
    if (n <= 0) return 0;
    long grid = (n + 255) / 256; if (grid > 2048) grid = 2048;
    hipLaunchKernelGGL(mulaw_decode_q_k, dim3((int)grid), dim3(256), 0, st, codes, table, q, audio, n);
    WN_CHECK_LAUNCH();
    return 0;
}
int wn_launch_mulaw_encode(const float* audio, const float* thr, uint8_t* codes, long n, hipStream_t st) {
    if (n <= 0) return 0;
    long grid = (n + 255) / 256; if (grid > 2048) grid = 2048;
    hipLaunchKernelGGL(mulaw_encode_k, dim3((int)grid), dim3(256), 0, st, audio, thr, codes, n);
    WN_CHECK_LAUNCH();
    return 0;
}
int wn_launch_mulaw_decode(const uint8_t* codes, const float* table, float* audio, long n, hipStream_t st) {
    if (n <= 0) return 0;
    long grid = (n + 255) / 256; if (grid > 2048) grid = 2048;
    hipLaunchKernelGGL(mulaw_decode_k, dim3((int)grid), dim3(256), 0, st, codes, table, audio, n);
    WN_CHECK_LAUNCH();
    return 0;
}

__global__ __launch_bounds__(256) void bias_grad_k(const float* __restrict__ a, long a_bstride, int a_pitch, int a_shift,
                                                   int t_lo, int t_hi, int batch, float* __restrict__ out) {
    __shared__ float red[4];
    const int row = blockIdx.x;
    float s = 0.f;
    for (int b = 0; b < batch; ++b) {
        const float* p = a + (size_t)b * a_bstride + (size_t)row * a_pitch + a_shift;
        for (int t = t_lo + threadIdx.x; t < t_hi; t += 256) s += p[t];
    }
    s = wave_sum(s);
    if ((threadIdx.x & 63) == 0) red[threadIdx.x >> 6] = s;
    __syncthreads();
    if (threadIdx.x == 0) out[row] = (red[0] + red[1]) + (red[2] + red[3]);
}
int wn_launch_bias_grad(const float* a, long a_bstride, int a_pitch, int a_shift, int rows, int t_lo,
                        int t_hi, int batch, float* out, hipStream_t st) {
    if (rows <= 0 || batch <= 0 || t_hi <= t_lo) return 0;
    hipLaunchKernelGGL(bias_grad_k, dim3(rows), dim3(256), 0, st, a, a_bstride, a_pitch, a_shift, t_lo, t_hi, batch, out);
    WN_CHECK_LAUNCH();
    return 0;
}

__global__ __launch_bounds__(256) void avgpool_k(const float* __restrict__ in, long in_bstride, int in_pitch, int t0,
                                                 int pool, int n_out, int rows, float* __restrict__ out,
                                                 long out_bstride, int out_pitch) {
    const int lane = threadIdx.x & 63;
    const long item = (long)blockIdx.x * 4 + (threadIdx.x >> 6);
    const int b = blockIdx.y;
    if (item >= (long)rows * n_out) return;
    const int row = (int)(item / n_out), j = (int)(item % n_out);
    const float* p = in + (size_t)b * in_bstride + (size_t)row * in_pitch + t0 + (size_t)j * pool;
    float s = 0.f;
    for (int k = lane; k < pool; k += 64) s += p[k];
    s = wave_sum(s);
    if (lane == 0) out[(size_t)b * out_bstride + (size_t)row * out_pitch + j] = s / (float)pool;
}
int wn_launch_avgpool(const float* in, long in_bstride, int in_pitch, int t0, int pool, int n_out, int rows,
                      float* out, long out_bstride, int out_pitch, int batch, hipStream_t st) {
    if (rows <= 0 || n_out <= 0 || batch <= 0) return 0;
    long items = (long)rows * n_out;
    hipLaunchKernelGGL(avgpool_k, dim3((unsigned)((items + 3) / 4), batch), dim3(256), 0, st, in, in_bstride, in_pitch, t0,
                       pool, n_out, rows, out, out_bstride, out_pitch);
    WN_CHECK_LAUNCH();
    return 0;
}

__global__ __launch_bounds__(256) void cond_grad_k(const float* __restrict__ in, long in_bstride, int in_pitch, int t_lo,
                                                   int t_hi, int mode, int le, int q, float* __restrict__ out,
                                                   long out_bstride, int out_pitch) {
    __shared__ float part[4][64];
    const int row = blockIdx.x, b = blockIdx.y;
    const int lane = threadIdx.x & 63, wave = threadIdx.x >> 6;
    const float* p = in + (size_t)b * in_bstride + (size_t)row * in_pitch + t_lo;
    float* o = out + (size_t)b * out_bstride + (size_t)row * out_pitch;
// ... 128 lines not shown
```

### music_amd/csrc/wn_gemm.hip

```cpp
#include <type_traits>
#include "wn_common.h"
#include "wn_kernels.h"

template <class T>
__global__ void pack_weights_k(const float* __restrict__ flat, const int32_t* __restrict__ idx,
                               uint16_t* __restrict__ out, int n, int ns) {
    int p = blockIdx.x * blockDim.x + threadIdx.x;
    if (p >= n) return;
    int src = idx[p];
    float v = src >= 0 ? flat[src] : 0.0f;
    typename T::elem h = T::cvt(v);
    int frag = p >> 9, r = p & 511;
    size_t o = (size_t)frag * (ns == 3 ? 1024 : 512) + r;
    out[o] = __builtin_bit_cast(uint16_t, h);
    if (ns == 3) {
        typename T::elem l = T::cvt(v - T::back(h));
        out[o + 512] = __builtin_bit_cast(uint16_t, l);
    }
}

int wn_launch_pack(const float* flat, const int32_t* idx, uint16_t* out, int n, int is_bf16, int ns,
                   hipStream_t st) {
    if (n <= 0) return 0;
    dim3 g((n + 255) / 256), b(256);
    if (is_bf16) hipLaunchKernelGGL(pack_weights_k<BF16>, g, b, 0, st, flat, idx, out, n, ns);
    else hipLaunchKernelGGL(pack_weights_k<F16>, g, b, 0, st, flat, idx, out, n, ns);
    WN_CHECK_LAUNCH();
    return 0;
}

template <class T, int NS, int MTW, int WM>
__global__ __launch_bounds__(512) void chan_gemm_k(WnGemmArgs a) {
    constexpr int WN = 8 / WM;
    constexpr int PF = MTW > 4 ? 1 : 2;
    const int lane = threadIdx.x & 63, wave = threadIdx.x >> 6;
    const int c = lane & 15, q = lane >> 4;
    const WnBlock blk = wn_block(a.swz);
    const int b = blk.z;
    const int wm = wave / WN, wn = wave % WN;
    const int t0 = a.t_base + (blk.x * WN + wn) * 64;
    const int tl = t0 + 4 * c;
    const int m0 = (blk.y * WM + wm) * MTW;
    if (t0 >= a.t_hi || m0 >= a.mt) return;
    const int KS = a.ks0 + a.ks1;

    f32x4 acc[MTW][4];
#pragma unroll
    for (int m = 0; m < MTW; ++m) {
        f32x4 init = {0.f, 0.f, 0.f, 0.f};
        if (a.bias != nullptr) {
#pragma unroll
            for (int i = 0; i < 4; ++i) {
                int row = (m0 + m) * 16 + 4 * q + i;
                init[i] = row < a.m_valid ? a.bias[row] : 0.f;
            }
        }
#pragma unroll
        for (int n = 0; n < 4; ++n) acc[m][n] = init;
    }

    const float* in0 = a.in0 + (size_t)b * a.in_bstride;
    const float* in1 = a.in1 ? a.in1 + (size_t)b * a.in_bstride : nullptr;
    const int col0 = tl + a.shift0, col1 = tl + a.shift1;

    const int t0u = __builtin_amdgcn_readfirstlane(t0);
    const bool inner0 = t0u + a.shift0 >= a.in_lo && t0u + 64 + a.shift0 <= a.in_hi;
    const bool inner1 = t0u + a.shift1 >= a.in_lo && t0u + 64 + a.shift1 <= a.in_hi;
    const bool weave = a.ks1 == a.ks0;
    auto kmap = [&](int s) { return weave ? ((s & 1) ? a.ks0 + (s >> 1) : (s >> 1)) : s; };
    auto issue = [&](f32x4* raw, int s0) {
        const int s = kmap(s0);
        const float* base; int col; int ch; bool inner;
        if (s < a.ks0) { base = in0; col = col0; ch = s * 32; inner = inner0; }
        else { base = in1; col = col1; ch = (s - a.ks0) * 32; inner = inner1; }
        const float* p = base + (size_t)(ch + 8 * q) * a.in_pitch + col;
        if (inner) {
#pragma unroll
            for (int j = 0; j < 8; ++j) raw[j] = ld4u(p + (size_t)j * a.in_pitch);
        } else {
#pragma unroll
            for (int j = 0; j < 8; ++j) raw[j] = ld4g(p + (size_t)j * a.in_pitch, col, a.in_lo, a.in_hi);
        }
    };
    auto step = [&](f32x4* raw, int s0) {
        const int s = kmap(s0);
        Frag<T> bf[4];
#pragma unroll
        for (int n = 0; n < 4; ++n) {
            float v[8];
#pragma unroll
            for (int j = 0; j < 8; ++j) {
                float x = raw[j][n];
                v[j] = a.relu_in ? fmaxf(x, 0.f) : x;
            }
            split8<T, NS>(bf[n], v);
        }
        if (s0 + PF < KS) issue(raw, s0 + PF);
        Frag<T> af[2];
        load_a<T, NS>(af[0], a.wpack, m0 * KS + s, lane);
#pragma unroll
        for (int m = 0; m < MTW; ++m) {
            if (m + 1 < MTW && m0 + m + 1 < a.mt) load_a<T, NS>(af[(m + 1) & 1], a.wpack, (m0 + m + 1) * KS + s, lane);
            if (m0 + m < a.mt) {
#pragma unroll
                for (int n = 0; n < 4; ++n) mma<T, NS>(acc[m][n], af[m & 1], bf[n]);
            }
        }
    };
    const bool early_resid = a.resid != nullptr && a.mask == nullptr;
    auto add_resid = [&]() {
        const float* resid = a.resid + (size_t)b * a.resid_bstride;
        const int r_lo = a.resid_lo > a.t_lo ? a.resid_lo : a.t_lo;
#pragma unroll
        for (int m = 0; m < MTW; ++m) {
            if (m0 + m >= a.mt) continue;
#pragma unroll
            for (int i = 0; i < 4; ++i) {
                const int row = (m0 + m) * 16 + 4 * q + i;
                if (row >= a.m_valid) continue;
                const float* rp = resid + (size_t)row * a.resid_pitch + tl;
                const f32x4 r = ld4g(rp, tl, r_lo, a.t_hi);
#pragma unroll
                for (int n = 0; n < 4; ++n) acc[m][n][i] += r[n];
            }
        }
    };
    if (PF == 2) {
        f32x4 raw0[8], raw1[8];
        issue(raw0, 0);
        if (KS > 1) issue(raw1, 1);
        if (early_resid) add_resid();
        for (int s = 0; s < KS; s += 2) {
            step(raw0, s);
            if (s + 1 < KS) step(raw1, s + 1);
        }
    } else {
        f32x4 raw0[8];
        issue(raw0, 0);
        if (early_resid) add_resid();
        for (int s = 0; s < KS; ++s) step(raw0, s);
    }

    float* out = a.out + (size_t)b * a.out_bstride;
    const float* resid = (a.resid && !early_resid) ? a.resid + (size_t)b * a.resid_bstride : nullptr;
    const float* mask = a.mask ? a.mask + (size_t)b * a.mask_bstride : nullptr;
    const bool full = tl >= a.t_lo && tl + 3 < a.t_hi;
#pragma unroll
    for (int m = 0; m < MTW; ++m) {
        if (m0 + m >= a.mt) continue;
#pragma unroll
        for (int i = 0; i < 4; ++i) {
            int row = (m0 + m) * 16 + 4 * q + i;
            if (row >= a.m_valid) continue;
            f32x4 v = {acc[m][0][i], acc[m][1][i], acc[m][2][i], acc[m][3][i]};
            if (mask) {
                const float* mp = mask + (size_t)row * a.mask_pitch + tl;
                if (full) {
                    f32x4 mv = ld4u(mp);
#pragma unroll
                    for (int e = 0; e < 4; ++e) v[e] = mv[e] > 0.f ? v[e] : 0.f;
                } else {
#pragma unroll
                    for (int e = 0; e < 4; ++e)
                        if (tl + e >= a.t_lo && tl + e < a.t_hi) v[e] = mp[e] > 0.f ? v[e] : 0.f;
                }
            }
            if (resid) {
                const float* rp = resid + (size_t)row * a.resid_pitch + tl;
                if (full && tl >= a.resid_lo) {
                    v += ld4u(rp);
                } else {
#pragma unroll
                    for (int e = 0; e < 4; ++e)
                        if (tl + e >= a.resid_lo && tl + e >= a.t_lo && tl + e < a.t_hi) v[e] += rp[e];
                }
            }
            float* op = out + (size_t)row * a.out_pitch + tl + a.out_shift;
            if (full) {
                F4U u = {{v[0], v[1], v[2], v[3]}};
// ... 230 lines not shown
```

### music_amd/csrc/wn_kernels.h

```cpp
#pragma once
#include <hip/hip_runtime.h>
#include <stdint.h>

enum { WN_MODE_F16X3 = 0, WN_MODE_F16X1 = 1, WN_MODE_BF16X3 = 2, WN_MODE_BF16X1 = 3 };
static inline int wn_mode_is_bf16(int m) { return m >= 2; }
static inline int wn_mode_ns(int m) { return (m & 1) ? 1 : 3; }
static inline size_t wn_frag_halfs(int mode) { return wn_mode_ns(mode) == 3 ? 1024 : 512; }

struct WnGemmArgs {
    const float* in0; const float* in1;
    long in_bstride; int in_pitch; int in_lo, in_hi;
    int shift0, shift1;
    int ks0, ks1;
    const uint16_t* wpack;
    int mt, m_valid;
    float* out; long out_bstride; int out_pitch; int out_shift;
    const float* bias;
    const float* resid; long resid_bstride; int resid_pitch; int resid_lo;
    const float* mask; long mask_bstride; int mask_pitch;
    int t_lo, t_hi, t_base;
    int relu_in;
    int swz;
};
int wn_launch_gemm(const WnGemmArgs& a, int batch, int mode, hipStream_t st);
int wn_launch_gemm_rw(const WnGemmArgs& a, int batch, int mode, hipStream_t st);
int wn_launch_gemm_bst(const WnGemmArgs& a, int batch, int mode, hipStream_t st);
struct WnEpiFwdArgs {
    const float* z; long z_bstride; int pitch;
    int ks_skip;
    const uint16_t* w_skip; const float* bias_s;
    float* u; float* h; long s_bstride;
    const uint16_t* w_p1c; const float* bias_1;
    const uint16_t* w_p2c; const float* bias_2;
    float* o; long o_bstride; int o_pitch;
    int s_valid, q_valid;
    int t_lo, t_hi, t_base, ntx;
    int stagger_n, stagger_cycles;
};
int wn_launch_skip_epilogue_fwd(const WnEpiFwdArgs& a, int batch, int mode, hipStream_t st);
struct WnEpiBwdArgs {
    const float* d_o; long o_bstride; int o_pitch;
    const float* h; const float* u; long s_bstride; int pitch;
    float* d_h; float* d_u;
    float* d_z; long z_bstride;
    const uint16_t* w_p2T; const uint16_t* w_p1Tc; const uint16_t* w_skipTc;
    int mt_z, z_valid, s_valid;
    int t_lo, t_hi, t_base, ntx;
    int nt_dz;
    int n_whole;
};
int wn_launch_skip_epilogue_bwd(const WnEpiBwdArgs& a, int batch, int mode, hipStream_t st);
struct WnResArgs;
int wn_launch_enc_resblock_fwd(const WnResArgs& a, int ch, int batch, int mode, hipStream_t st);
int wn_launch_pack(const float* flat, const int32_t* idx, uint16_t* out, int n, int is_bf16, int ns,
                   hipStream_t st);

struct WnResArgs {
    const float* x_in; float* x_out; float* z_out;
    long x_bstride, z_bstride; int pitch;
    const uint16_t* wfg; const uint16_t* wd;
    const float* bias_f; const float* bias_g; const float* bias_d;
    int n_f, n_d;
    int d, t_lo, t_hi, z_lo, t_base;
    int write_x;
    const float* cond; long cond_bstride; int cond_pitch;
    int cond_mode, cond_le, cond_q;
    const uint16_t* cond_pack; long cond_pack_bstride; const uint8_t* cond_idx;
    long z_half;
    int swz;
};
int wn_launch_resblock_fwd(const WnResArgs& a, int ch, int batch, int mode, hipStream_t st);
int wn_launch_resblock_fwd_nt(const WnResArgs& a, int ch, int batch, int mode, hipStream_t st);

struct WnResBwdArgs {
    const float* x_in;
    const float* dy;
    const float* dz;
    float* dfg;
    float* z;
    long x_bstride, dz_bstride, dfg_bstride, z_bstride; int pitch;
    const uint16_t* wfg;
    const uint16_t* wdT;
    const float* bias_f; const float* bias_g; int n_f;
    int d, t_lo, t_hi, z_lo, t_base;
    const float* cond; long cond_bstride; int cond_pitch;
    int cond_mode, cond_le, cond_q;
    int swz;
};
int wn_launch_resblock_bwd(const WnResBwdArgs& a, int ch, int batch, int mode_fwd, int mode_bwd,
                           hipStream_t st);

struct WnResMsArgs {
    const float* x_in; const float* dy; const float* dz;
    float* dfg;
    long x_bstride, dz_bstride, dfg_bstride; int pitch;
    const uint16_t* wfg; const uint16_t* wdT;
    const float* bias_f; const float* bias_g; int n_f;
    float* slab_fg; float* slab_d;
    int d, t_lo, t_hi, z_lo, t_base;
    int steps_per_clip, items_per_wg, batch;
    int swz;
    const float* cond; long cond_bstride; int cond_pitch;
    int cond_mode, cond_le, cond_q;
};
int wn_launch_resblock_bwd_ms(const WnResMsArgs& a, int ch, int batch, int mode_fwd, int mode_bwd, hipStream_t st);
int wn_resms_slabs(int t_lo, int t_hi, int batch);
int wn_launch_resblock_bwd_rw(const WnResMsArgs& a, int batch, hipStream_t st);
void wn_resrw_plan(int t_lo, int t_hi, int batch, int& t_base, int& steps, int& ipw, int& nwg);
struct WnResPqArgs {
    const float* x_in;
    const float* p_in; const float* q_in; int dn, p_lo;
    const float* dz;
    float* p_out; float* q_out;
    long x_bstride, dz_bstride; int pitch;
    const uint16_t* wfg; const uint16_t* wdT; const uint16_t* wpq;
    float* slab_fg; float* slab_d;
    int d, t_lo, t_hi, z_lo, t_base;
    int steps_per_clip, items_per_wg, batch;
    int swz;
    const float* cond; long cond_bstride; int cond_pitch; int cond_le;
    const uint8_t* cond_idx; float* cslab; int cslab_slots;
    long dz_half;
    int chain, ch_s, ch_qn, ch_rm, ch_g, ch_nchain;
};
#define WN_PQ_IDX_PAD 64
int wn_launch_resblock_bwd_pq(const WnResPqArgs& a, int batch, hipStream_t st);
int wn_pq_chain_ok(int t_lo, int t_hi, int batch, int d);
void wn_pq_chain_plan(int t_lo, int t_hi, int batch, int d, int& t_base, int& steps, int& s, int& qn, int& rm, int& g, int& nchain, int& nwg);
int wn_pq_slabs(int t_lo, int t_hi, int batch, int d, int chain);
int wn_pq_chain_items(int t_lo, int t_hi, int batch, int d, int wg, int* out, int cap);
int wn_pq_cond_slots(int t_lo, int t_hi, int batch);
int wn_pq_cond_slab_floats(int t_lo, int t_hi, int batch);
int wn_launch_pq_cond_reduce(const float* cslab, const long* off, const int* t_lo, int n, int t_hi, int batch, int le, float* out,
                             long out_lstride, long out_bstride, int out_pitch, hipStream_t st);
int wn_launch_split16(const float* x, uint16_t* hi, uint16_t* lo, long n, int is_bf16, hipStream_t st);
int wn_launch_shift_add(const float* p, const float* q, float* out, long bstride, int pitch, int rows, int dn,
                        int p_lo, int t_lo, int t_hi, int batch, hipStream_t st);
int wn_launch_enc_bwd_rw(const WnResMsArgs& a, int ch, int batch, int mode_bwd, hipStream_t st);
int wn_enc_bwd_slabs(int t_lo, int t_hi, int batch);
struct WnEncPqArgs {
    const float* x_in;
    const float* p_in; const float* q_in; int dn, p_lo;
    const float* h; long h_bstride;
    float* p_out; float* q_out;
    long x_bstride; int pitch;
    const uint16_t* wdT; const uint16_t* wpq;
    float* slab_dil; float* slab_d;
    int d, t_lo, t_hi, t_base;
    int steps_per_clip, items_per_wg, batch, swz;
    int chain, ch_s, ch_qn, ch_rm, ch_g, ch_nchain;
};
int wn_launch_enc_bwd_pq(const WnEncPqArgs& a, int ch, int batch, int mode_bwd, hipStream_t st);

struct WnWgradArgs {
    const float* a; long a_bstride; int a_pitch; int a_shift; int a_cols;
    const float* b0; const float* b1; long b_bstride; int b_pitch; int b_shift0, b_shift1; int b_cols;
    int nt_per_tap;
    int mt;
    int relu_b;
    float* c; int ldc;
    long c_slab_stride;
    int t_lo, t_hi, t_base; int chunk;
    int swz;
};
int wn_launch_wgrad(const WnWgradArgs& a, int batch, int mode, hipStream_t st);
int wn_launch_wgrad2(const WnWgradArgs* a1, const WnWgradArgs* a2, int batch, int mode, hipStream_t st);
int wn_wgrad_num_slabs(int t_lo, int t_hi, int chunk, int batch);
int wn_launch_reduce_slabs(const long* desc, int n_ops, long total_vec, const float* slab, float* out, hipStream_t st);

int wn_launch_causal_wgrad_codes(const int32_t* codes, int scrambled, const float* dx, const float* dxq, int dn, int p_lo,
                                 long dx_bstride, int pitch, int ch, int T, int batch, float* slab, hipStream_t st);
int wn_causal_codes_slabs(int T, int batch);
int wn_launch_causal_fwd_codes(const int32_t* codes, int scrambled, const float* wt, const float* bias, int n_rows, float* x0,
                               long x_bstride, int pitch, int ch, int T, int batch, hipStream_t st);

int wn_launch_softmax_fwd(const float* x, float* y, long nrows, hipStream_t st);
int wn_launch_softmax_bwd(const float* y, const float* dy, float* dx, long nrows, hipStream_t st);
#define WN_CE_PARTIALS 1024
int wn_launch_softmax_ce(const float* x, const int64_t* target, float* probs, float* dx,
                         float* loss_part, long nrows, float inv_n, hipStream_t st);
int wn_launch_adam(float* p, const float* g, float* m, float* v, long n, float lr, float b1, float b2,
                   float eps, float bc1, float bc2, float gscale, hipStream_t st);
int wn_launch_sgd(float* p, const float* g, float* buf, long n, float lr, float momentum, float gscale, int first, hipStream_t st);
int wn_launch_rmsprop(float* p, const float* g, float* sq, float* buf, long n, float lr, float alpha, float eps, float momentum,
                      float gscale, hipStream_t st);
struct wn_guard_state;
int wn_launch_grad_guard(const float* g, long n, float gscale, float max_norm, int skip_nonfinite, float beta1, float beta2,
                         void* partials, wn_guard_state* state, hipStream_t st);
int wn_launch_adam_guarded(float* p, const float* g, float* m, float* v, long n, float lr, float b1, float b2, float eps, float gscale,
                           const wn_guard_state* state, hipStream_t st);
int wn_launch_sgd_guarded(float* p, const float* g, float* buf, long n, float lr, float momentum, float gscale,
                          const wn_guard_state* state, hipStream_t st);
int wn_launch_rmsprop_guarded(float* p, const float* g, float* sq, float* buf, long n, float lr, float alpha, float eps, float momentum,
                              float gscale, const wn_guard_state* state, hipStream_t st);
int wn_launch_ema(float* ema, const float* p, long n, float decay, int warmup, long t, const wn_guard_state* state, hipStream_t st);
int wn_launch_gather_grads(const float* packed, const int32_t* idx, float* flat_grad, int n, hipStream_t st);
int wn_launch_gather_grads2(const float* packed, const int32_t* idx, const int32_t* idx2, float* flat_grad, int n, hipStream_t st);
int wn_launch_onehot(const int32_t* idx, float* out, int batch, int q, int t, int scrambled, hipStream_t st);
int wn_launch_mulaw_encode(const float* audio, const float* thr, uint8_t* codes, long n, hipStream_t st);
int wn_launch_mulaw_decode(const uint8_t* codes, const float* table, float* audio, long n, hipStream_t st);
int wn_launch_mulaw_encode_q(const float* audio, const float* thr, int n_thr, int32_t* codes, long n, hipStream_t st);
int wn_launch_mulaw_decode_q(const int32_t* codes, const float* table, int q, float* audio, long n, hipStream_t st);
int wn_launch_bias_grad(const float* a, long a_bstride, int a_pitch, int a_shift, int rows, int t_lo,
                        int t_hi, int batch, float* out, hipStream_t st);

int wn_launch_cond_expand(const float* tab, long tab_bstride, int tab_pitch, int rows, int t_lo, int t_hi, int mode, int le, int q,
                          float* out, long out_bstride, int out_pitch, int batch, hipStream_t st);
int wn_launch_cond_grad(const float* in, long in_bstride, int in_pitch, int rows, int t_lo, int t_hi, int mode, int le,
                        int q, float* out, long out_bstride, int out_pitch, int batch, hipStream_t st);
int wn_launch_avgpool_bwd(const float* denc, long denc_bstride, int denc_pitch, int t0, int pool, int n_out, int rows,
                          float* out, long out_bstride, int out_pitch, int t_hi, int batch, hipStream_t st);
int wn_launch_avgpool(const float* in, long in_bstride, int in_pitch, int t0, int pool, int n_out, int rows,
                      float* out, long out_bstride, int out_pitch, int batch, hipStream_t st);

struct WnCondProj {
    const float* enc; const float* flat;
    long w_off, b_off, stage_stride, wf_off, bf_off;
    float* tab; float* tab_pair; float* enf;
    const float* d_tab; int d_pair; const float* d_enf; float* d_enc; float* flat_grad;
    int n_stages, dd, ch, sd, bw, le, batch;
};
int wn_launch_cond_proj_fwd(const WnCondProj& p, hipStream_t st);
int wn_launch_cond_proj_bwd(const WnCondProj& p, hipStream_t st);
bool wn_cond_denc_fits(const WnCondProj& p);
int wn_launch_cond_denc(const WnCondProj& p, hipStream_t st);
#define WN_GCOND_MAX_E 512
struct WnGcond {
    const int32_t* cls;
    long gw_off, gstage_stride, gwf_off, emb_off;
    int ge, n_cls;
};
int wn_launch_gcond_proj_fwd(const WnCondProj& p, const WnGcond& g, hipStream_t st);
int wn_launch_gcond_proj_bwd(const WnCondProj& p, const WnGcond& g, hipStream_t st);
#define WN_VQ_PARTIALS 256
#define WN_RVQ_MAX_S 8
struct WnVq {
    const float* enc; const float* flat; long cb_off;
    float* q_out; int32_t* idx; int32_t* counts; float* loss_part;
    const float* d_q; float* d_enc; float* flat_grad;
    int K, bw, le, batch;
    int S; float* res;
    const int32_t* nstage;
};
int wn_launch_vq_fwd(const WnVq& p, hipStream_t st);
int wn_launch_vq_bwd(const WnVq& p, float beta, float g_scale, float* stat, hipStream_t st);
int wn_launch_vq_lookup(const int32_t* idx, const int32_t* nstage, const float* flat, long cb_off, float* q_out, int32_t* bad, int stages,
                        int K, int bw, int le, int batch, hipStream_t st);
#define WN_VQ_MAX_K 1024
#define WN_VQ_EMA_WORK (16 + 4 * WN_VQ_MAX_K)
int wn_launch_vq_ema_update(float* flat, long cb_off, const float* stat, float* state, void* work, int32_t* info, int S, int K, int bw,
                            float decay, float eps, float restart, const wn_guard_state* guard, hipStream_t st);
#define WN_WIN_MAX 16
struct WnNllWin { int period; unsigned pos0, pow32; const int64_t* pos; int lo[WN_WIN_MAX], hi[WN_WIN_MAX]; };
int wn_launch_step_nll(const float* x, long x_bs, int x_pitch, const int64_t* target, float* dx, long dx_bs, int dx_pitch, float* probs,
                       float* row_nll, int32_t* row_hit, float* loss_part, int w, int q, int batch, float inv_n, const WnNllWin* win,
                       hipStream_t st);
int wn_launch_gate_fwd(const float* fg, long fg_bstride, int dp, int rows, float* z, long z_bstride, int pitch, int t_lo, int t_hi,
                       int batch, hipStream_t st);
int wn_launch_gate_bwd(const float* fg, long fg_bstride, int dp, int rows, const float* dz, long dz_bstride, float* dfg,
                       long dfg_bstride, int pitch, int t_lo, int t_hi, int batch, hipStream_t st);
int wn_launch_softmaxq_fwd(const float* x, float* y, long nrows, int q, hipStream_t st);
int wn_launch_softmaxq_bwd(const float* y, const float* dy, float* dx, long nrows, int q, hipStream_t st);
int wn_launch_softmaxq_ce(const float* x, const int64_t* target, float* probs, float* dx, float* loss_part, long nrows, int q,
                          float inv_n, hipStream_t st);

#define WN_DEC_MAX_LAYERS 64
struct WnSampling { float temperature; float top_p; int32_t top_k; uint32_t stream; uint64_t seed; };
static_assert(sizeof(WnSampling) == 24, "wn_sampling is 24 bytes");
struct WnDecodeArgs {
    int n_layers, R, D, S, Q;
    int dil[WN_DEC_MAX_LAYERS];
    long q_off[WN_DEC_MAX_LAYERS];
    float* queues;
    const float* w_causal; const float* b_causal;
    const float* w_layers; long layer_stride;
    const float* b_layers;
    const float* b_skip_sum;
    const float* w_p1; const float* b_p1; const float* w_p2; const float* b_p2;
    const float* note0; const float* prev0;
    float* note_out; float* prev_out;
    const int32_t* forced;
    int32_t* codes_out; float* probs_out;
    long step0; int n_steps; int push_input;
    int dbg;
    unsigned long long* sync;
    long sync_ustride;
    int n_utt; long queues_ustride;
    int sample; float inv_temp; unsigned long long seed;
    const uint16_t* pk; long pk_fg0, pk_d0, pk_lstride;
    long pk_skip, pk_p1, pk_p2;
    int fw;
    const float* cond_fg; long cond_fg_ustride;
    const float* cond_p1; long cond_p1_ustride;
    int c_shift[WN_DEC_MAX_LAYERS + 1], c_q[WN_DEC_MAX_LAYERS + 1];
    int le; long pos0;
    const WnSampling* samp; int top_k; float top_p;
    int win_period, win_pos0;
    int win_lo[WN_WIN_MAX], win_hi[WN_WIN_MAX];
};
__host__ __device__ inline int wn_dec_cond_idx(int c, int q, int le) {
    if (c < 0) return 0;
    if (q > 0) { const int i = c / q; return i < le ? i : le - 1; }
    return c % le;
}
int wn_launch_decode(const WnDecodeArgs& a, hipStream_t st);
size_t dec_k_lds_bytes(const WnDecodeArgs& a);
#define WN_DEC_MAX_Q 1024
long wn_decode_granules(int n_layers, int D, int S);
struct WnWin { int period, pos0; int lo[WN_WIN_MAX], hi[WN_WIN_MAX]; };
int wn_launch_sample_logits(const float* logits, long n, int Q, long ld, const WnSampling* samp, float temperature,
                            unsigned long long seed, int top_k, float top_p, long step0, const float* u, int32_t* codes,
                            float* probs, const WnWin& win, hipStream_t st);

int wn_coll_loaded();
int wn_coll_unique_id(char* id128);
int wn_coll_create(int nranks, int rank, const char* id128, void** comm);
int wn_coll_destroy(void* comm);
int wn_coll_allreduce_flat(void* comm, float* buf, int64_t n, hipStream_t st);
```

### music_amd/csrc/wn_wgrad.hip

```cpp
#include <type_traits>
#include "wn_common.h"
#include "wn_kernels.h"

struct WgRaw { f32x4 u0, u1; };

__device__ __forceinline__ WgRaw wg_load(const float* row, int col, int ncols) {
    WgRaw r;
    r.u0 = ld4g(row + col, col, 0, ncols);
    r.u1 = ld4g(row + col + 4, col + 4, 0, ncols);
    return r;
}

template <class T, int NS>
__device__ __forceinline__ void wg_frag(Frag<T>& f, const WgRaw& r, int t, int t_lo, int t_hi, bool masked, bool relu) {
    float v[8] = {r.u0[0], r.u0[1], r.u0[2], r.u0[3], r.u1[0], r.u1[1], r.u1[2], r.u1[3]};
    if (masked) {
#pragma unroll
        for (int j = 0; j < 8; ++j)
            if (t + j < t_lo || t + j >= t_hi) v[j] = 0.f;
    }
    if (relu) {
#pragma unroll
        for (int j = 0; j < 8; ++j) v[j] = fmaxf(v[j], 0.f);
    }
// ... 217 lines not shown
            dst[lane] = __builtin_bit_cast(u32x4, f.hi);
            if (NS == 3) dst[64 + lane] = __builtin_bit_cast(u32x4, f.lo);
        }
    };
    auto run = [&](auto guarded) {
        auto issue = [&](int tb) {
            const int t = tb + 8 * q;
#pragma unroll
            for (int k = 0; k < 4; ++k) {
                if (decltype(guarded)::value) {
                    raw[k] = wg_load(lrow[k], t + lshift[k], lcols[k]);
                } else {
                    const float* p = lrow[k] + t + lshift[k];
                    raw[k].u0 = ld4u(p);
                    raw[k].u1 = ld4u(p + 4);
                }
            }
        };
        auto issue_piece = [&](int tb, int k, int half) {
            const int t = tb + 8 * q;
            if (decltype(guarded)::value) {
                if (half == 0) raw[k] = wg_load(lrow[k], t + lshift[k], lcols[k]);
            } else {
                const float* p = lrow[k] + t + lshift[k];
                if (half == 0) raw[k].u0 = ld4u(p);
                else raw[k].u1 = ld4u(p + 4);
            }
        };
        const int tb_last = tc0 + ((tc1 - 1 - tc0) & ~31);
        if (tc0 < tc1) {
            issue(tc0);
            park(0, tc0);
            issue(tc0 + 32 < tc1 ? tc0 + 32 : tb_last);
        }
        __syncthreads();
        int it = 0;
        for (int tb = tc0; tb < tc1; tb += 32, ++it) {
            const int tb1 = tb + 32 < tc1 ? tb + 32 : tb_last, tb2 = tb + 64 < tc1 ? tb + 64 : tb_last;
            const uint16_t* base = l_f + (size_t)(it & 1) * 32 * FR;
            Frag<T> bf[4], af[2];
#pragma unroll
            for (int n = 0; n < 4; ++n) load_a<T, NS>(bf[n], base, 16 + wn * 4 + n, lane);
            load_a<T, NS>(af[0], base, wm * 8, lane);
#pragma unroll
            for (int m = 0; m < 8; ++m) {
                if (m + 1 < 8) load_a<T, NS>(af[(m + 1) & 1], base, wm * 8 + m + 1, lane);
                if (m == 4) {
                    __builtin_amdgcn_sched_barrier(0);
                    park((it + 1) & 1, tb1);
                    __builtin_amdgcn_sched_barrier(0);
                }
                if (m >= 4) {
                    issue_piece(tb2, m - 4, 0);
                    issue_piece(tb2, m - 4, 1);
                }
#pragma unroll
                for (int n = 0; n < 4; ++n) mma<T, NS>(acc[m][n], af[m & 1], bf[n]);
                __builtin_amdgcn_sched_barrier(0);
            }
            __syncthreads();
        }
    };
    {
        const int last_tb = tc0 + ((tc1 - 1 - tc0) & ~31);
        if (tc0 >= tb_lo && last_tb <= tb_hi) run(std::false_type{});
        else run(std::true_type{});
    }
    const int n_chunks = (a.t_hi - a.t_base + a.chunk - 1) / a.chunk;
    float* cs = a.c + ((size_t)b * n_chunks + wb.x) * a.c_slab_stride;
#pragma unroll
    for (int m = 0; m < 8; ++m) {
        const int mt = mg * 16 + wm * 8 + m;
        if (mt >= a.mt) continue;
#pragma unroll
        for (int n = 0; n < 4; ++n) {
            const int nt = ng * 16 + wn * 4 + n;
            if (nt >= nt_total) continue;
#pragma unroll
            for (int i = 0; i < 4; ++i)
                cs[(size_t)(mt * 16 + 4 * q + i) * a.ldc + nt * 16 + c] = acc[m][n][i];
        }
    }
}

static void wg_prepare(WnWgradArgs& k, int& nchunks, int& ygroups) {
    k.t_base = k.t_lo & ~31;
    k.swz = wn_xcd_swizzle_enabled();
    if (k.chunk < 128) k.chunk = 128;
    k.chunk = (k.chunk + 127) & ~127;
    const int nt_total = k.nt_per_tap * (k.b1 ? 2 : 1);
    const int nblk = ((nt_total + 3) / 4) * ((k.mt + 3) / 4);
    nchunks = (k.t_hi - k.t_base + k.chunk - 1) / k.chunk;
    ygroups = (nblk + 3) / 4;
}

int wn_launch_wgrad2(const WnWgradArgs* a1, const WnWgradArgs* a2, int batch, int mode, hipStream_t st) {
    if (batch <= 0) return 0;
    WnWgradPair pr;
    int n = 0, nch[2] = {0, 0}, yg[2] = {0, 0};
    const WnWgradArgs* src[2] = {a1, a2};
    for (int i = 0; i < 2; ++i) {
        if (!src[i] || src[i]->t_hi <= src[i]->t_lo) continue;
        pr.p[n] = *src[i];
        wg_prepare(pr.p[n], nch[n], yg[n]);
        ++n;
    }
    if (n == 0) return 0;
    if (n == 1) {
        const WnWgradArgs& k = pr.p[0];
        const int nt_total = k.nt_per_tap * (k.b1 ? 2 : 1);
        if (k.mt >= 16 && nt_total >= 16) {
            const int ns = wn_mode_ns(mode);
            const size_t sh = (size_t)2 * 32 * (ns == 3 ? 1024 : 512) * sizeof(uint16_t);
            dim3 g(nch[0], ((k.mt + 15) / 16) * ((nt_total + 15) / 16), batch), b(512);
            int dev = 0;
            (void)hipGetDevice(&dev);
            static WnDevOnce done[4];
#define WN_BIG(TT, NN, slot) do { \
                if (done[slot].need(dev)) { \
                    (void)hipFuncSetAttribute(reinterpret_cast<const void*>(&wgrad_big_k<TT, NN>), \
                                              hipFuncAttributeMaxDynamicSharedMemorySize, (int)sh); \
                    done[slot].done(dev); } \
                hipLaunchKernelGGL((wgrad_big_k<TT, NN>), g, b, sh, st, k); } while (0)
            switch (mode) {
                case WN_MODE_BF16X3: WN_BIG(BF16, 3, 0); break;
                case WN_MODE_BF16X1: WN_BIG(BF16, 1, 1); break;
                case WN_MODE_F16X3: WN_BIG(F16, 3, 2); break;
                case WN_MODE_F16X1: WN_BIG(F16, 1, 3); break;
                default: return wn_set_error_msg(-2, "wgrad: bad mode");
            }
#undef WN_BIG
            WN_CHECK_LAUNCH();
            return 0;
        }
        pr.p[1] = pr.p[0]; yg[1] = 0; nch[1] = 0;
    }
    pr.y_split = yg[0];
    dim3 g(nch[0] > nch[1] ? nch[0] : nch[1], yg[0] + yg[1], batch), b(512);
    switch (mode) {
        case WN_MODE_BF16X3: hipLaunchKernelGGL((wgrad_k<BF16, 3>), g, b, 0, st, pr); break;
        case WN_MODE_BF16X1: hipLaunchKernelGGL((wgrad_k<BF16, 1>), g, b, 0, st, pr); break;
        case WN_MODE_F16X3: hipLaunchKernelGGL((wgrad_k<F16, 3>), g, b, 0, st, pr); break;
        case WN_MODE_F16X1: hipLaunchKernelGGL((wgrad_k<F16, 1>), g, b, 0, st, pr); break;
        default: return wn_set_error_msg(-2, "wgrad: bad mode");
    }
    WN_CHECK_LAUNCH();
    return 0;
}

int wn_launch_wgrad(const WnWgradArgs& a, int batch, int mode, hipStream_t st) {
    return wn_launch_wgrad2(&a, nullptr, batch, mode, st);
}

__global__ __launch_bounds__(256) void reduce_slabs_k(const long* __restrict__ desc, int n_ops, long total_vec,
                                                      const float* __restrict__ slab, float* __restrict__ out) {
    long v = (long)blockIdx.x * blockDim.x + threadIdx.x;
    if (v >= total_vec) return;
    int lo = 0, hi = n_ops - 1;
    while (lo < hi) {
        int mid = (lo + hi + 1) >> 1;
        if (desc[mid * 6] <= v) lo = mid; else hi = mid - 1;
    }
    const long* d = desc + lo * 6;
    const long e = (v - d[0]) * 4, n = d[5], stride = d[3];
    const int ns = (int)d[2];
    const float* sp = slab + d[1] + e;
    float* op = out + d[4] + e;
    if (e + 3 < n) {
        f32x4 s8[8];
#pragma unroll
        for (int k = 0; k < 8; ++k) s8[k] = f32x4{0.f, 0.f, 0.f, 0.f};
        int i = 0;
        for (; i + 8 <= ns; i += 8) {
            f32x4 t[8];
#pragma unroll
            for (int k = 0; k < 8; ++k) t[k] = ld4u(sp + (size_t)(i + k) * stride);
#pragma unroll
            for (int k = 0; k < 8; ++k) s8[k] += t[k];
        }
        for (; i < ns; ++i) s8[0] += ld4u(sp + (size_t)i * stride);
        const f32x4 s = ((s8[0] + s8[1]) + (s8[2] + s8[3])) + ((s8[4] + s8[5]) + (s8[6] + s8[7]));
        op[0] = s[0]; op[1] = s[1]; op[2] = s[2]; op[3] = s[3];
    } else {
        for (long k = 0; e + k < n; ++k) {
            float s = 0.f;
            for (int i = 0; i < ns; ++i) s += sp[(size_t)i * stride + k];
            op[k] = s;
        }
    }
}

int wn_launch_reduce_slabs(const long* desc, int n_ops, long total_vec, const float* slab, float* out, hipStream_t st) {
    if (total_vec <= 0 || n_ops <= 0) return 0;
    hipLaunchKernelGGL(reduce_slabs_k, dim3((unsigned)((total_vec + 255) / 256)), dim3(256), 0, st, desc, n_ops,
                       total_vec, slab, out);
    WN_CHECK_LAUNCH();
    return 0;
}
```

### music_amd/engine.py

```python
import math
import os

import numpy as np
import torch

from . import _lib
from ._lib import call, ptr
from .engine_base import SLACK, PAD_BACK, EngineBase, SlabPlan, WorkspaceHold, WorkspacePool, _Spec, _pad
from .packs import PackSet, causal_mats, epilogue_mats, gated_mats, pack_index, pack_positions, pair_mats
from .stack import EpiBias, GatedStack, SkipEpilogue


class WaveNetEngine(EngineBase):
    def __init__(self, dilations, residual_channels, dilation_channels, skip_channels,
                 quantization_channels=256, filter_width=2, use_bias=False,
                 mode_fwd="f16x3", mode_bwd="bf16x3", device=None):
        if filter_width != 2:
            raise NotImplementedError("HIP path implements filter_width == 2 (the reference's only configuration)")
        if quantization_channels != 256:
            raise NotImplementedError("HIP path implements quantization_channels == 256 (chunk softmax width)")
        self.dil = [int(d) for d in dilations]
        self.N = len(self.dil)
        self.R, self.D, self.S, self.Q = residual_channels, dilation_channels, skip_channels, quantization_channels
        self.fused_loss_ok = True
        self.use_bias = bool(use_bias)
        self.CH = _pad(max(self.R, self.D), 32)
        if self.CH not in (32, 64):
            raise NotImplementedError("HIP path supports residual/dilation channels <= 64")
        self.SP = _pad(self.S, 32)
        self.rf = sum(self.dil) + 2
        self.off = [1]
        for d in self.dil:
            self.off.append(self.off[-1] + d)
        assert self.off[-1] == self.rf - 1
        self.mode_fwd = _lib.MODE_NAMES[mode_fwd] if isinstance(mode_fwd, str) else mode_fwd
        self.mode_bwd = _lib.MODE_NAMES[mode_bwd] if isinstance(mode_bwd, str) else mode_bwd
        self.pair_ok = (self.CH == 32 and not self.use_bias and self.mode_fwd == _lib.F16X3 and self.mode_bwd == _lib.BF16X3
                        and os.environ.get("WN_PAIR32", "1") == "1" and os.environ.get("WN_PQ_BWD", "1") == "1")
        self.device = torch.device(device if device is not None else "cuda")
        _lib.load()
        self._build_spec()
        self._build_packs()
        self._init_state()
        self.epi_chains = 2
        self.epi_fused = os.environ.get("WN_EPI_FUSED", "1") == "1"
        self.epi_fused_bwd = os.environ.get("WN_EPI_FUSED_BWD", "1") == "1"
        self.ms_bwd = None
        self.fine_marks = False
        self.z_from_fwd = True
        bn = "dilation_layer_stack.%d.bias"
        self.stack = GatedStack(self, "", self.CH, self.R, self.D, self._fr, self._br,
                                lambda i: (self._bias_ptr(bn % (4 * i)), self._bias_ptr(bn % (4 * i + 1)), self._bias_ptr(bn % (4 * i + 2))),
                                self.mode_fwd, self.mode_bwd, fmark=self.fmark, side_wgrad=True, zero_tail=True)
        bias = EpiBias([bn % (4 * i + 3) for i in range(self.N)], "post_process_1.bias", "post_process_2.bias", self._bias_ptr,
                       lambda name: ptr(self.gpack, self.gp_bias_off[name]),
                       [self.spec.off[bn % (4 * i + 3)] for i in range(self.N)]) if self.use_bias else None
        self.epilogue = SkipEpilogue(self, ("skip", "p1", "p2"), ("U", "H", None, "dH"), self.CH, self.S, self.SP, self._fr, self._br,
                                     self.mode_fwd, self.mode_bwd, bias=bias, fmark=self.fmark)

    def fmark(self, name):
        if self.fine_marks:
            self.mark(name)

    def _build_spec(self):
        names = [("causal_layer.weight", (self.R, self.Q, 2))]
        if self.use_bias:
            names.append(("causal_layer.bias", (self.R,)))
        for i in range(self.N):
            for k, shp in enumerate([(self.D, self.R, 2), (self.D, self.R, 2), (self.R, self.D, 1), (self.S, self.D, 1)]):
                names.append(("dilation_layer_stack.%d.weight" % (4 * i + k), shp))
                if self.use_bias:
                    names.append(("dilation_layer_stack.%d.bias" % (4 * i + k), (shp[0],)))
        names.append(("post_process_1.weight", (self.S, self.S, 1)))
        if self.use_bias:
            names.append(("post_process_1.bias", (self.S,)))
        names.append(("post_process_2.weight", (self.Q, self.S, 1)))
        if self.use_bias:
            names.append(("post_process_2.bias", (self.Q,)))
        self.spec = _Spec(names)
        self.param_names = [n for n, _ in names]
        dev = self.device
        self.flat = torch.zeros(self.spec.total, dtype=torch.float32, device=dev)
        self.flat_grad = torch.zeros(self.spec.total, dtype=torch.float32, device=dev)

    def param_view(self, name, grad=False):
        o, shp = self.spec.off[name], self.spec.shape[name]
        n = int(np.prod(shp))
        return (self.flat_grad if grad else self.flat)[o:o + n].view(shp)

    def load_state_dict_tensors(self, sd):
        with torch.no_grad():
            for n in self.param_names:
                self.param_view(n).copy_(sd[n])

    def _bias_ptr(self, name):
        if not self.use_bias:
            return None
        return ptr(self.flat, self.spec.off[name])

    def _fr(self, name):
        return ptr(self.pk_f, self.pk_f_off[name])

    def _br(self, name):
        return ptr(self.pk_b, self.pk_b_off[name])

    def _build_packs(self):
        sp, CH, N, dev = self.spec, self.CH, self.N, self.device
        wn = "dilation_layer_stack.%d.weight"
        pk = PackSet(sp.total)
        causal = causal_mats(sp.conv("causal_layer.weight"), CH)
        pk.fwd("causal", causal.w)
        pk.bwd("causalT", causal.wT)
        for i in range(N):
            g = gated_mats(sp.conv(wn % (4 * i)), sp.conv(wn % (4 * i + 1)), sp.conv(wn % (4 * i + 2))[:, :, 0], CH)
            pk.fwd("fg%d" % i, g.fg)
            pk.fwd("d%d" % i, g.d, chained=True)
            pk.bwd("dT%d" % i, g.dT)
            pk.bwd("fgT%d" % i, g.fgT)
            pk.bwd("pq%d" % i, g.pq)
            if self.pair_ok:
                g2 = pair_mats(g)
                pk.fwd("fg2_%d" % i, g2.fg, pair=True)
                pk.fwd("d2_%d" % i, g2.d, chained=True, pair=True)
                pk.bwd("dT2_%d" % i, g2.dT)
                pk.bwd("pq2_%d" % i, g2.pq)
        pk.epilogue(epilogue_mats([sp.conv(wn % (4 * i + 3))[:, :, 0] for i in range(N)], sp.conv("post_process_1.weight")[:, :, 0],
                                  sp.conv("post_process_2.weight")[:, :, 0], CH, self.SP), "skip", "p1", "p2", chained_fwd=True)
        for name in self.param_names if self.use_bias else ():
            if name.endswith(".bias"):
                pk.bias(name, sp.off[name], sp.shape[name][0])
        self.pk_f_off, self.pk_f_idx, self.pk_f = pk.finish(pk.f, self.mode_fwd, dev)
        self.pk_b_off, self.pk_b_idx, self.pk_b = pk.finish(pk.b, self.mode_bwd, dev)
        self.gp_off, self.gp_bias_off = pk.gp_off, pk.gp_bias_off
        self.gpack = torch.zeros(pk.go, dtype=torch.float32, device=dev)
        gidx, ga, gb = pk.gather_maps()
        assert (gidx >= 0).all()
        self.gidx = torch.from_numpy(gidx.astype(np.int32)).to(dev)
        if self.pair_ok:
            self.gidx_pa = torch.from_numpy(ga.astype(np.int32)).to(dev)
            self.gidx_pb = torch.from_numpy(gb.astype(np.int32)).to(dev)
        self.wt_idx = torch.from_numpy(causal.taps).to(dev)
        self.wt = torch.zeros(causal.taps.size, dtype=torch.float32, device=dev)

    def pack_weights(self):
        st = _lib.stream()
        call("wn_pack_weights", ptr(self.flat), ptr(self.pk_f_idx), ptr(self.pk_f), self.pk_f_idx.numel(), self.mode_fwd, st)
        call("wn_pack_weights", ptr(self.flat), ptr(self.pk_b_idx), ptr(self.pk_b), self.pk_b_idx.numel(), self.mode_bwd, st)

    def _make_workspace(self, B, T):
        dev = self.device
        pitch = _pad(T, 256) + 512
        W = T - self.rf + 1
        buf = lambda rows: self.act_buf(B, rows, pitch)
        ws = dict(B=B, T=T, W=W, pitch=pitch)
        ws["X"] = buf((self.N + 1) * self.CH)
        ws["Z"] = buf(self.N * self.CH)
        ws["U"] = buf(self.SP)
        ws["H"] = buf(self.SP)
        ws["O"] = torch.zeros(B * self.Q * W + PAD_BACK, dtype=torch.float32, device=dev)
        ws["bwd"] = None
        ws["ms"], ws["pq"] = self._use_ms(), self._use_pq()
        ws["pair"] = self.pair_ok and B % 2 == 0
        ws["pair_fwd"] = ws["pair"] and (B // 2) * ((T + 511) // 512) >= 200
        return ws

    def _bwd_workspace(self, ws):
        if ws["bwd"] is not None:
            return ws["bwd"]
        B, pitch, W, dev = ws["B"], ws["pitch"], ws["W"], self.device
        buf = lambda rows: self.act_buf(B, rows, pitch)
        bw = dict(dO=torch.zeros(B * self.Q * W + PAD_BACK, dtype=torch.float32, device=dev),
                  dH=buf(self.SP), dU=buf(self.SP), dZ=buf(self.N * self.CH),
                  dX=[buf(self.CH), buf(self.CH)], dfg=[buf(2 * self.CH), buf(2 * self.CH)],
                  zs=[buf(self.CH), buf(self.CH)])
        T, lo = ws["T"], self.rf - 1
        ms = ws["ms"]
        bw["ms"] = ms
        bw["pq"] = ws["pq"]
        pair = bw["pair"] = ws["pair"]
        if bw["pq"] or pair:
            bw["PQ"] = [(buf(self.CH), buf(self.CH)), (buf(self.CH), buf(self.CH))]
        ck = [int(v) for v in os.environ.get("WN_EPI_WGRAD_CHUNKS", "2048,2048,2048").split(",")]
        if "WN_EPI_WGRAD_CHUNKS" not in os.environ:
            span = T - (lo & ~31)

            def even(c):
                n = -(-span // c)
                return -(-(-(-span // n)) // 32) * 32
            ck = [even(c) for c in ck]
        plan = SlabPlan(self.gp_off)
        for name, c in zip(("p2", "p1", "skip"), ck):
            plan.add(name, _lib.wgrad_slabs(lo, T, c, B), c)
        Bp = B // 2 if pair else B
        want = os.environ.get("WN_PQ_CHAIN", "1") == "1"
        bw["chain"] = [want and bool(bw["pq"] or pair) and _lib.pq_chain_ok(self.off[i + 1], T, Bp, self.dil[i]) for i in range(self.N)]
        sfx = "2_" if pair else ""
        for i in range(self.N):
            t_lo = self.off[i + 1]
            if bw["pq"] or pair:
                ns, chunk = _lib.pq_slabs(t_lo, T, Bp, self.dil[i], bw["chain"][i]), None
            elif ms:
                ns, chunk = _lib.ms_slabs(t_lo, T, B), None
            else:
                ns, chunk = _lib.wgrad_slabs(t_lo, T, 512, B), 512
            plan.add("fg%s%d" % (sfx, i), ns, chunk)
            if i < self.N - 1:
                plan.add("d%s%d" % (sfx, i), ns, chunk)
        plan.add("causal", _lib.wgrad_slabs(1, T, 512, B), 512)
        plan.add_alternative("causal", "causal_codes", _lib.causal_codes_slabs(T, B))
        bw.update(plan.finish(dev))
        ws["bwd"] = bw
        return bw

    def _use_ms(self):
        ok = self.CH == 64 and self.mode_fwd == _lib.F16X3 and self.mode_bwd == _lib.BF16X3
        if self.ms_bwd is None:
            return ok and os.environ.get("WN_MS_BWD", "1") == "1"
        if self.ms_bwd and not ok:
            raise NotImplementedError("ms_bwd needs 64 padded channels and precision (f16x3, bf16x3)")
        return bool(self.ms_bwd)

    def _use_pq(self):
        return self._use_ms() and not self.use_bias and os.environ.get("WN_PQ_BWD", "1") == "1"

    def _x(self, ws, i):
        return ptr(ws["X"], SLACK + i * ws["B"] * self.CH * ws["pitch"])

    def forward_logits(self, x, ws=None, codes=None):
        if x is None:
            B, T = codes[0].shape
            Q = self.Q
            assert codes[0].is_cuda and codes[0].dtype == torch.int32 and codes[0].is_contiguous()
        else:
            B, Q, T = x.shape
            assert Q == self.Q and x.is_contiguous() and x.dtype == torch.float32 and x.is_cuda
        W = T - self.rf + 1
        if W <= 0:
            raise ValueError("wave sample not long enough")
        ws = ws or self._ws.get(B, T)
        st = _lib.stream()
        CH, pitch, mf = self.CH, ws["pitch"], self.mode_fwd
        self._gen += 1
        ws["gen"] = self._gen
        ws["x_in"] = x
        ws["x_codes"] = (codes[0], bool(codes[1])) if x is None else self.tagged_codes(x, B, T)
        ws["x_ver"] = None if x is None else x._version
        ws["codes_ver"] = None if ws["x_codes"] is None else ws["x_codes"][0]._version
        self.causal_fwd(ws, x, self.wt_idx, self.wt, self._fr("causal"), self._bias_ptr("causal_layer.bias"), self.R, CH, self._x(ws, 0), st, mf)
        self.mark("causal_fwd")
        z_whole = self.z_from_fwd and not ws["ms"] and not ws["pair"]
        self.stack.forward(B, T, pitch, ws["X"], ws["Z"], z_whole, st, pair=ws["pair_fwd"])
        self.mark("stack_fwd")
        self.epilogue.forward(ws, self.epilogue.skip_bias(ws), st, self.epi_fused, int(self.epi_chains))
        self.mark("epilogue_fwd")
        return ws

    def forward(self, x):
        self.pack_weights()
        ws = self.forward_logits(x)
        B, W = ws["B"], ws["W"]
        probs = torch.empty(B * W, self.Q, dtype=torch.float32, device=self.device)
        call("wn_chunk_softmax256_fwd", ptr(ws["O"]), ptr(probs), B * W, _lib.stream())
        ws["probs"] = probs
        return probs, ws

    def backward_from_dlogits(self, ws):
        bw = self._bwd_workspace(ws)
        st = _lib.stream()
        self.epilogue.backward(self.epilogue.begin_backward(ws, bw), st, self.epi_fused_bwd and not self.use_bias,
                               side_skip=os.environ.get("WN_EPI_BWD_ORDER", "1") != "1")
        self.mark("epilogue_bwd")
        return self._backward_stack(ws, bw, st)

    def _backward_stack(self, ws, bw, st):
        B, T, pitch, CH = ws["B"], ws["T"], ws["pitch"], self.CH

        def bias_grads(i, dfg, dy, t_lo, s_):
            if self.use_bias:
                bo, bn = self.gp_bias_off, "dilation_layer_stack.%d.bias"
                call("wn_bias_grad", dfg, 2 * CH * pitch, pitch, 0, self.D, t_lo, T, B, ptr(self.gpack, bo[bn % (4 * i)]), s_)
                call("wn_bias_grad", dfg + 4 * CH * pitch, 2 * CH * pitch, pitch, 0, self.D, t_lo, T, B, ptr(self.gpack, bo[bn % (4 * i + 1)]), s_)
                if dy is not None:
                    call("wn_bias_grad", dy, CH * pitch, pitch, 0, self.R, t_lo, T, B, ptr(self.gpack, bo[bn % (4 * i + 2)]), s_)
        form = "pq" if bw["pq"] or bw["pair"] else "ms" if bw["ms"] else "rw"
        self.stack.backward(form, B, T, pitch, ws["X"], ws["Z"], bw, bw["dX"], st, chain=bw["chain"], dfg=bw["dfg"],
                            zs=None if self.z_from_fwd else bw["zs"], pair=bw["pair"], hook=bias_grads)
        self.join_side()
        self.mark("stack_bwd")
        dx0 = ptr(bw["dX"][0], SLACK)
        self._check_input_unchanged(ws)
        x_codes = self.codes_for_backward(ws)
        self.causal_wgrad(ws, bw, x_codes, "causal", dx0, CH, st, self.mode_bwd)
        if self.use_bias:
            call("wn_bias_grad", dx0, CH * pitch, pitch, 0, self.R, 1, T, B, ptr(self.gpack, self.gp_bias_off["causal_layer.bias"]), st)
        self.mark("causal_bwd")
        self.reduce_and_gather(bw, x_codes is not None, st)
        self.mark("slab_reduce")

    def input_grad(self, ws):
        bw = ws["bwd"]
        if bw is None:
            raise RuntimeError("music_amd: input_grad() needs the backward of this forward to have run")
        return self.causal_input_grad(ws, bw["dX"][0], self.CH, self._br("causalT"), self.mode_bwd)

    def backward(self, ws, dprobs):
        bw = self._bwd_workspace(ws)
        dprobs = dprobs.contiguous()
        call("wn_chunk_softmax256_bwd", ptr(ws["probs"]), ptr(dprobs), ptr(bw["dO"]), ws["B"] * ws["W"], _lib.stream())
        self.backward_from_dlogits(ws)

    def loss_and_grad_codes(self, codes, target, scrambled=True, want_probs=False, objective=None, windows=None, window_pos=None):
        return self.loss_and_grad(None, target, want_probs, codes=(codes, scrambled), objective=objective, windows=windows,
                                  window_pos=window_pos)

    def loss_and_grad(self, x, target, want_probs=False, codes=None, objective=None, windows=None, window_pos=None):
        def step():
            self.mark("begin")
            self.pack_weights()
            self.mark("pack")
            return self._fused_tail(self.forward_logits(x, codes=codes), target, want_probs, objective, windows, window_pos)
        return self._throttled(step)

    def softmax_ce(self, *args):
        super().softmax_ce(*args)
        self.mark("softmax_ce")

    def adam_step(self, gscale=1.0):
        super().adam_step(gscale)
        self.mark("adam")

    def onehot(self, codes, scrambled=True):
        B, T = codes.shape
        out = torch.empty(B, self.Q, T, dtype=torch.float32, device=self.device)
        call("wn_onehot", ptr(codes), ptr(out), B, self.Q, T, 1 if scrambled else 0, _lib.stream())
        self.mark("onehot")
        if codes.is_contiguous() and codes.dtype == torch.int32:
            out._wn_codes = (codes, bool(scrambled), out._version, codes._version)
        return out
```

### music_amd/engine_base.py

```python
import ctypes
import weakref
from collections import namedtuple

import numpy as np
import torch

from . import _lib, guard, vq_dropout
from ._lib import call, ptr

SLACK = 64
PAD_BACK = 2048


def _pad(n, m):
    return (n + m - 1) // m * m


class WorkspacePool:
    MAX_SHAPES = 4
    MAX_PER_SHAPE = 4

    def __init__(self, make):
        from collections import OrderedDict
        self._make = make
        self._d = OrderedDict()
        self._last = {}

    def peek(self, B, T):
        ws = self._last.get((B, T))
        return ws if ws is not None else self.get(B, T)

    def get(self, B, T):
        key = (B, T)
        lst = self._d.get(key)
        if lst is None:
            if len(self._d) >= self.MAX_SHAPES:
                for k, wl in self._d.items():
                    if not any(w.get("held") for w in wl):
                        del self._d[k]
                        self._last.pop(k, None)
                        break
            lst = self._d[key] = []
        self._d.move_to_end(key)
        for ws in lst:
            if not ws.get("held"):
                self._last[key] = ws
                return ws
        if len(lst) >= self.MAX_PER_SHAPE:
            import warnings
            warnings.warn("music_amd: %d forwards of shape %s are waiting for their backward; the oldest one's activations are "
                          "reused (run backward(), drop the outputs, or use torch.no_grad() for inference)" % (len(lst), key))
            ws = min(lst, key=lambda w: w.get("gen", 0))
            ws["held"] = False
            self._last[key] = ws
            return ws
        ws = self._make(B, T)
        lst.append(ws)
        self._last[key] = ws
        return ws

    def clear(self):
        self._d.clear()
        self._last.clear()

    def __len__(self):
        return sum(len(v) for v in self._d.values())


class WorkspaceHold:

    def __init__(self, ws):
        self.ws, self.gen = ws, ws["gen"]
        ws["held"] = True

    def release(self):
        if self.ws is not None and self.ws.get("gen") == self.gen:
            self.ws["held"] = False
        self.ws = None

    def __del__(self):
        self.release()


class _Spec:

    def __init__(self, named_shapes):
        self.off, self.shape = {}, {}
        o = 0
        for name, shape in named_shapes:
            self.off[name] = o
            self.shape[name] = tuple(shape)
            o += int(np.prod(shape))
        self.total = o

    def conv(self, name):
        shp = self.shape[name]
        return self.off[name] + np.arange(int(np.prod(shp)), dtype=np.int64).reshape(shp)


OBJECTIVES = ("reference", "nll")


class NllWindows:

    def __init__(self, windows, Q):
        try:
            pairs = [(int(lo), int(hi)) for lo, hi in windows]
        except (TypeError, ValueError):
            raise ValueError("windows must be a sequence of (lo, hi) pairs") from None
        if not 1 <= len(pairs) <= 16:
            raise ValueError("windows must hold 1..16 (lo, hi) pairs, got %d" % len(pairs))
        for lo, hi in pairs:
            if not 0 <= lo < hi <= Q:
                raise ValueError("every window needs 0 <= lo < hi <= Q = %d, got (%d, %d)" % (Q, lo, hi))
        self.pairs = pairs
        self.host = (ctypes.c_int32 * (2 * len(pairs)))(*[v for pr in pairs for v in pr])
        self.pos = None

    def tail(self, window_pos, B, device):
        pos, pos0 = None, 0
        if isinstance(window_pos, torch.Tensor) and window_pos.dim() > 0:
            pos = window_pos.reshape(-1)
            if pos.dtype != torch.int64:
                raise ValueError("window_pos as a tensor is int64, one stream position per clip, got %s" % pos.dtype)
            pos = pos.to(device).contiguous()
        elif window_pos is not None and not isinstance(window_pos, (int, np.integer, torch.Tensor)):
            vals = [int(v) for v in window_pos]
            if any(v < 0 for v in vals):
                raise ValueError("window_pos (the stream position of a clip's first target) must be >= 0, got %d" % min(vals))
            pos = torch.tensor(vals, dtype=torch.int64).to(device)
        elif window_pos is not None:
            pos0 = int(window_pos)
            if pos0 < 0:
                raise ValueError("window_pos (the stream position of a clip's first target) must be >= 0, got %d" % pos0)
        if pos is not None and pos.numel() != B:
            raise ValueError("window_pos holds %d positions for %d clips" % (pos.numel(), B))
        self.pos = pos
        return ctypes.cast(self.host, ctypes.c_void_p), len(self.pairs), ptr(pos), pos0


SlabOp = namedtuple("SlabOp", "so n chunk ns")


class SlabPlan:

    def __init__(self, gp_off):
        self.gp_off, self.ops, self.desc, self.row, self.alt = gp_off, {}, [], {}, []
        self.so = self.vs = 0

    def __getitem__(self, name):
        return self.ops[name]

    def _region(self, name, n, chunk, ns):
        op = self.ops[name] = SlabOp(self.so, n, chunk, ns)
        self.so += ns * n
        return op

    def add(self, name, ns, chunk=None, grad=None):
        go, r, c = self.gp_off[grad or name]
        op = self._region(name, r * c, chunk, ns)
        self.row[name] = len(self.desc)
        self.desc.append([self.vs, op.so, ns, op.n, go, op.n])
        self.vs += (op.n + 3) // 4

    def add_alternative(self, of, name, ns):
        op = self._region(name, self.ops[of].n, None, ns)
        self.alt.append((self.row[of], [op.so, ns]))

    def finish(self, device):
        out = dict(slab=torch.empty(self.so, dtype=torch.float32, device=device), plan=self, vec=self.vs, nops=len(self.desc),
                   desc=torch.tensor(self.desc, dtype=torch.int64, device=device))
        if self.alt:
            rows = [list(r) for r in self.desc]
            for i, so_ns in self.alt:
                rows[i][1:3] = so_ns
            out["desc_codes"] = torch.tensor(rows, dtype=torch.int64, device=device)
        return out


class VqStats:

    def __init__(self, part, counts, frames, beta, coef=None, final_res=None):
        self.part, self.counts, self.frames, self.beta = part, counts, frames, beta
        self.coef = 1.0 + beta if coef is None else coef
        self.final_res = final_res

    @property
    def stage_frames(self):
        return self.counts.reshape(-1, self.counts.shape[-1]).sum(dim=1)

    @property
    def stage_mse_active(self):
        n = self.stage_frames.to(torch.float32)
        return torch.where(n > 0, self.stage_mse * float(self.frames) / n.clamp_min(1.0), torch.zeros_like(n))

    @property
    def stage_mse(self):
        return self.part.reshape(-1, self.part.shape[-1]).sum(dim=1)

    @property
    def stage_perplexity(self):
        if self.final_res is not None:
            p = self.counts.to(torch.float64) / self.stage_frames.clamp_min(1).to(torch.float64)[:, None]
            return torch.exp(-(p * torch.log(p.clamp_min(1e-300))).sum(dim=1)).float()
        p = self.counts.reshape(-1, self.counts.shape[-1]).to(torch.float64) / self.frames
        return torch.exp(-(p * torch.log(p.clamp_min(1e-300))).sum(dim=1)).float()

    @property
    def stage_codes_used(self):
        return (self.counts.reshape(-1, self.counts.shape[-1]) > 0).sum(dim=1)

    @property
    def mse(self):
        if self.final_res is not None:
            return self.final_res.square().sum() / self.final_res.numel()
        return self.part.sum() if self.part.dim() == 1 else self.part[-1].sum()

    @property
    def vq_loss(self):
        return self.part.sum() * self.coef

    @property
    def perplexity(self):
        p = (self.counts if self.counts.dim() == 1 else self.counts[0]).to(torch.float64) / self.frames
        return torch.exp(-(p * torch.log(p.clamp_min(1e-300))).sum()).float()

    @property
    def codes_used(self):
        return ((self.counts if self.counts.dim() == 1 else self.counts[0]) > 0).sum()


class EngineBase:

    objective = "reference"
    nll_windows = None

    def _init_state(self):
        self._ws = WorkspacePool(self._make_workspace)
        self._gen = 0
        self.adam_state = None
        self.marks = None
        self.mark_only = None
        self._throttle = _lib.StepThrottle()
        self._side = None
        self.overlap_wgrad = True

    def mark(self, name):
        if self.marks is not None and (self.mark_only is None or name in self.mark_only):
            ev = torch.cuda.Event(enable_timing=True)
            ev.record()
            self.marks.append((name, ev))

    def workspace(self, B, T):
        return self._ws.peek(B, T)

    def act_buf(self, B, rows, pitch):
        return torch.zeros(SLACK + B * rows * pitch + PAD_BACK, dtype=torch.float32, device=self.device)

    def _gemm(self, st, B, mode, wpack, in0, in1, in_bs, in_pitch, in_lo, in_hi, s0, s1, ks0, ks1, mt, m_valid, out, out_bs,
              out_pitch, out_shift, bias, resid, mask, t_lo, t_hi, relu_in):
        call("wn_chan_gemm", in0, in1, in_bs, in_pitch, in_lo, in_hi, s0, s1, ks0, ks1, wpack, mt, m_valid,
             out, out_bs, out_pitch, out_shift, bias, resid[0], resid[1], resid[2], resid[3] if len(resid) > 3 else 0,
             mask[0], mask[1], mask[2], t_lo, t_hi, relu_in, B, mode, st)

    def _check_input_unchanged(self, ws):
        if ws.get("x_ver") is not None and ws["x_in"]._version != ws["x_ver"]:
            raise RuntimeError("music_amd: the input of this forward was modified in place before backward()")

    learned = False
    n_cond = 0

    vq = False
    n_vq = 0
    last_vq = None
    vq_S = 1
    vq_ema = False
    gcond = False
    n_gcond = 0

    @property
    def n_gather(self):
        return self.spec.total - self.n_cond - self.n_vq - self.n_gcond

    @property
    def gathered_param_names(self):
        N = len(self.dil)
        return self.param_names[:len(self.param_names) - (2 * (N + 1) if self.learned else 0) - (1 if self.vq else 0) - (N + 2 if self.gcond else 0)]

    def _plan_cond(self, net):
        self.learned = getattr(net, "conditioning", "random") == "learned"
        self.vq = getattr(net, "bottleneck", "continuous") == "vq"
        self.gcond = int(getattr(net, "global_classes", 0)) > 0
        if self.gcond:
            if not self.learned:
                raise ValueError('music_amd: global_classes > 0 requires conditioning="learned"')
            o, N = self.spec.off, len(self.dil)
            E, n = self.g_E, self.g_n = int(net.global_channels), int(net.global_classes)
            gw0, gwf, emb = o["de_gcond_layer_stack.0.weight"], o["connection_gcond.weight"], o["global_embedding.weight"]
            gstride = 2 * self.Dd * E
            assert all(o["de_gcond_layer_stack.%d.weight" % i] == gw0 + i * gstride for i in range(N)) and gwf == gw0 + N * gstride \
                and emb == gwf + self.Sd * E and emb + n * E == self.spec.total
            self.gcond_off = (gw0, gstride, gwf, emb)
            self.n_gcond = self.spec.total - gw0
        if self.vq:
            if not self.learned:
                raise ValueError('music_amd: bottleneck="vq" requires conditioning="learned"')
            S = self.vq_S = int(getattr(net, "vq_stages", 1))
            self.vq_K, self.vq_beta = int(net.vq_codebook.num_embeddings) // S, float(net.vq_beta)
            self.vq_off = self.spec.off["vq_codebook.weight"]
            self.n_vq = S * self.vq_K * self.Bw
            assert self.spec.shape["vq_codebook.weight"] == (S * self.vq_K, self.Bw) and self.vq_off + self.n_vq == self.spec.total - self.n_gcond
            self.vq_ema = getattr(net, "vq_update", "gradient") == "ema"
            if self.vq_ema:
                self.vq_decay, self.vq_eps, self.vq_restart = float(net.vq_decay), float(net.vq_eps), float(net.vq_restart)
                self.vq_stat = torch.zeros(S * self.vq_K * (self.Bw + 1), dtype=torch.float32, device=self.device)
                self.vq_ema_work = torch.zeros(S * _lib.VQ_EMA_WORK_BYTES // 4, dtype=torch.int32, device=self.device)
                self.vq_ema_info = torch.zeros(2 * S, dtype=torch.int32, device=self.device)
                self._vq_net = weakref.ref(net)
        if not self.learned:
            return
        o, N = self.spec.off, len(self.dil)
        w0, b0 = o["de_cond_layer_stack.0.weight"], o["de_cond_layer_stack.0.bias"]
        stride = 2 * self.Dd * self.Bw + 2 * self.Dd
        wf, bf = o["connection_cond.weight"], o["connection_cond.bias"]
        assert all(o["de_cond_layer_stack.%d.weight" % i] == w0 + i * stride and o["de_cond_layer_stack.%d.bias" % i] == b0 + i * stride
                   for i in range(N)) and wf == w0 + N * stride and bf + self.Sd == self.spec.total - self.n_vq - self.n_gcond
        self.cond_off = (w0, b0, stride, wf, bf)
        self.n_cond = self.spec.total - self.n_vq - self.n_gcond - w0

    def vq_stage_counts(self, stages, B):
        n = vq_dropout.stage_counts(stages, B, self.vq_S if self.vq else 1)
        return None if n is None else torch.from_numpy(n).to(self.device, non_blocking=True)

    def vq_fwd(self, ws, enc, st, nstage=None):
        B, _, Le = enc.shape
        dev = self.device
        S, chain = self.vq_S, self.vq_S > 1
        lead = (S,) if chain else ()
        nstage = nstage if chain else None
        q = torch.empty_like(enc)
        idx = torch.empty(lead + (B, Le), dtype=torch.int32, device=dev)
        counts = torch.empty(lead + (self.vq_K,), dtype=torch.int32, device=dev)
        part = torch.empty(lead + (_lib.VQ_NUM_PARTIALS,), dtype=torch.float32, device=dev)
        res = torch.empty(lead + tuple(enc.shape), dtype=torch.float32, device=dev) if chain else None
        call("wn_vq_fwd" if not chain else "wn_rvq_fwd" if nstage is None else "wn_rvq_fwd_n",
             ptr(enc), ptr(self.flat), self.vq_off, *([ptr(nstage)] if nstage is not None else []), ptr(q), ptr(idx), ptr(counts),
             *([ptr(res)] if chain else []), ptr(part), *([S] if chain else []), self.vq_K, self.Bw, Le, B, st)
        ws.update(enc_pre=enc, vq_idx=idx, vq_counts=counts, vq_part=part, vq_g=1.0, **(dict(vq_res=res, vq_nstage=nstage) if chain else {}))
        self.last_vq = VqStats(part, counts, B * Le, self.vq_beta, self.vq_loss_coef, final_res=None if nstage is None else res[S - 1])
        return q

    def vq_bwd(self, ws, d_q, st):
        B, _, Le = d_q.shape
        chain = self.vq_S > 1
        nstage = ws.get("vq_nstage") if chain else None
        call(("wn_rvq_bwd" if chain else "wn_vq_bwd") + ("_stats" if self.vq_ema else "") + ("_n" if nstage is not None else ""),
             ptr(ws["enc_pre"]), ptr(ws["vq_idx"]), *([ptr(ws["vq_res"])] if chain else []), *([ptr(nstage)] if nstage is not None else []),
             ptr(d_q), ptr(self.flat), self.vq_off, self.vq_beta, float(ws.get("vq_g", 1.0)), ptr(d_q), ptr(self.flat_grad),
             *([ptr(self.vq_stat)] if self.vq_ema else []), *([self.vq_S] if chain else []), self.vq_K, self.Bw, Le, B, st)

    @property
    def vq_loss_coef(self):
        return self.vq_beta if self.vq_ema else 1.0 + self.vq_beta

    def vq_codes_of(self, ws):
        idx = ws["vq_idx"].to(torch.int64)
        return idx if self.vq_S == 1 else idx.permute(1, 0, 2)

    def vq_ema_state(self):
        net = self._vq_net()
        state = None if net is None else getattr(net, "vq_ema_state", None)
        if state is None or state.device != self.flat.device or state.dtype != torch.float32 or state.numel() != self.vq_stat.numel():
            raise RuntimeError("music_amd: the model's vq_ema_state buffer is gone, or not where its parameters are")
        return state

    def vq_ema_step(self, guard=None):
        chain = self.vq_S > 1
        call("wn_rvq_ema_update" if chain else "wn_vq_ema_update", ptr(self.flat), self.vq_off, ptr(self.vq_stat), ptr(self.vq_ema_state()),
             ptr(self.vq_ema_work), ptr(self.vq_ema_info), *([self.vq_S] if chain else []), self.vq_K, self.Bw, self.vq_decay, self.vq_eps,
             self.vq_restart, None if guard is None else guard.state_ptr(), _lib.stream())

    def vq_restarted(self):
        n = int(self.vq_ema_info[0::2].sum().item())
        self.vq_ema_info[0::2] = 0
        return n

    def vq_backward_scaled(self, ws, dloss, dvq):
        ws["vq_g"] = 0.0 if dvq is None else float(dvq)
        d_o = self._bwd_workspace(ws)["dO"][:ws["B"] * ws["W"] * self.Q]
        keep = d_o.clone()
        if dloss is None:
            d_o.zero_()
        else:
            d_o.mul_(dloss)
        self.backward_from_dlogits(ws)
        d_o.copy_(keep)

    def vq_lookup(self, codes):
        S, chain, dev = self.vq_S, self.vq_S > 1, self.device
        nstage = None
        if chain:
            if codes.dim() != 3 or not 1 <= codes.shape[1] <= S:
                raise ValueError("music_amd: vq_stages = %d: codes must be (B, n, Le) with 1 <= n <= %d, not %s" % (S, S, tuple(codes.shape)))
            nstage = None if codes.is_floating_point() else vq_dropout.counts_of_codes(codes, S)
        elif codes.dim() != 2:
            raise ValueError("music_amd: codes must be (B, Le), not %s" % (tuple(codes.shape),))
        idx = codes.to(device=dev, dtype=torch.int32)
        if chain:
            idx = idx.permute(1, 0, 2)
        n = idx.shape[0] if chain else 1
        if nstage is not None:
            full = torch.full((S,) + tuple(idx.shape[1:]), -1, dtype=torch.int32, device=dev)
            full[:n] = idx
            idx, nstage = full, torch.from_numpy(nstage).to(dev)
        idx = idx.contiguous()
        B, Le = idx.shape[-2:]
        q = torch.empty(B, self.Bw, Le, dtype=torch.float32, device=dev)
        bad = torch.zeros(1, dtype=torch.int32, device=dev)
        call("wn_vq_lookup" if not chain else "wn_rvq_lookup" if nstage is None else "wn_rvq_lookup_n",
             ptr(idx), *([ptr(nstage)] if nstage is not None else []), ptr(self.flat), self.vq_off, ptr(q), ptr(bad), *([S] if chain else []),
             *([n] if chain and nstage is None else []), self.vq_K, self.Bw, Le, B, _lib.stream())
        if int(bad.item()):
            raise ValueError("music_amd: a code lies outside [0, %d)" % self.vq_K)
        return q

    def _check_cond(self, cond):
        if self.learned and cond is not None:
            raise ValueError('music_amd: conditioning="learned": the projections are the model\'s parameters, pass cond=None')
        if not self.learned and cond is None:
            raise ValueError('music_amd: conditioning="random": pass the drawn projections (net.conditioning_projections()) as cond')

    def stage_classes(self, classes, B):
        if not self.gcond:
            if classes is not None:
                raise ValueError("music_amd: global_classes is 0: this model takes no classes, pass classes=None")
            return None
        if classes is None:
            raise ValueError("music_amd: global_classes = %d: pass classes, one integer in [0, %d) per clip" % (self.g_n, self.g_n))
        cls = classes if torch.is_tensor(classes) else torch.as_tensor(list(classes))
        if cls.dim() != 1 or cls.numel() != B or cls.is_floating_point() or cls.is_complex() or cls.dtype == torch.bool:
            raise ValueError("music_amd: classes must be %d integers, one per clip, not %s of shape %s" % (B, cls.dtype, tuple(cls.shape)))
        if cls.device.type == "cpu" and B and not (0 <= int(cls.min()) and int(cls.max()) < self.g_n):
            raise ValueError("music_amd: a class lies outside [0, %d) (global_classes)" % self.g_n)
        return cls.to(device=self.device, dtype=torch.int32, non_blocking=True).contiguous()

    def _gcond_args(self, cls):
        return (ptr(cls),) + self.gcond_off + (self.g_E, self.g_n)

    def cond_proj_fwd(self, enc, tab, tab_pair, enf, ch, st, cls=None):
        B, _, Le = enc.shape
        args = (ptr(enc), ptr(self.flat)) + self.cond_off + (ptr(tab), ptr(tab_pair), ptr(enf), len(self.dil), self.Dd, ch, self.Sd, self.Bw,
                                                            Le, B)
        if self.gcond:
            return call("wn_gcond_proj_fwd", *args, *self._gcond_args(cls), st)
        call("wn_cond_proj_fwd", *args, st)

    def cond_proj_bwd(self, d_tab, pair, d_enf, enc, d_enc, ch, st, cls=None):
        B, _, Le = enc.shape
        args = (ptr(d_tab), 1 if pair else 0, ptr(d_enf), ptr(enc), ptr(self.flat)) + self.cond_off + (
            ptr(d_enc), ptr(self.flat_grad), len(self.dil), self.Dd, ch, self.Sd, self.Bw, Le, B)
        if self.gcond:
            return call("wn_gcond_proj_bwd", *args, *self._gcond_args(cls), st)
        call("wn_cond_proj_bwd", *args, st)

    def _side_stream(self):
        if self._side is None:
            self._side = _lib.side_stream(self.device)
        return self._side

    def on_side(self, fn):
        if not self.overlap_wgrad:
            return fn(_lib.stream())
        side, ev = self._side_stream(), torch.cuda.Event()
        ev.record(torch.cuda.current_stream())
        side.wait_event(ev)
        with torch.cuda.stream(side):
            fn(_lib.stream())

    def join_side(self):
        if self.overlap_wgrad:
            ev = torch.cuda.Event()
            ev.record(self._side_stream())
            torch.cuda.current_stream().wait_event(ev)

    def wgrad(self, bw, B, mode, st, name, *args):
        op = bw["plan"][name]
        head, (ldc, t_lo, t_hi) = args[:-3], args[-3:]
        call("wn_wgrad", *head, ptr(bw["slab"], op.so), ldc, op.n, t_lo, t_hi, op.chunk, B, mode, st)

    def wgrad_s(self, bw, B, mode, name, *args):
        self.on_side(lambda s2: self.wgrad(bw, B, mode, s2, name, *args))

    def reduce_and_gather(self, bw, from_codes, st):
        call("wn_reduce_slabs", ptr(bw["desc_codes"] if from_codes else bw["desc"]), bw["nops"], bw["vec"], ptr(bw["slab"]), ptr(self.gpack), st)
        if bw["pair"]:
            call("wn_gather_grads2", ptr(self.gpack), ptr(self.gidx_pa), ptr(self.gidx_pb), ptr(self.flat_grad), self.n_gather, st)
        else:
            call("wn_gather_grads", ptr(self.gpack), ptr(self.gidx), ptr(self.flat_grad), self.n_gather, st)

    @staticmethod
    def tagged_codes(x, B, T):
        tag = getattr(x, "_wn_codes", None) if x is not None else None
        if tag is not None:
            codes, scrambled, version, cversion = tag
            if (x._version == version and codes._version == cversion and codes.is_cuda and codes.dtype == torch.int32 and
                    codes.is_contiguous() and tuple(codes.shape) == (B, T)):
                return codes, scrambled
        return None

    def causal_fwd(self, ws, x, wt_idx, wt, wpack, bias, R, CH, out, st, mode):
        B, T, pitch, Q = ws["B"], ws["T"], ws["pitch"], self.Q
        if ws["x_codes"] is None:
            return call("wn_chan_gemm", ptr(x), ptr(x), Q * T, T, 0, T, -1, 0, Q // 32, Q // 32, wpack, CH // 16, R, out, CH * pitch, pitch, 0, bias,
                        None, 0, 0, 0, None, 0, 0, 1, T, 0, B, mode, st)
        codes, scrambled = ws["x_codes"]
        call("wn_gather_grads", ptr(self.flat), ptr(wt_idx), ptr(wt), wt.numel(), st)
        call("wn_causal_fwd_codes", ptr(codes), 1 if scrambled else 0, ptr(wt), bias, R, out, CH * pitch, pitch, CH, Q, T, B, st)

    def codes_for_backward(self, ws):
        x_codes, cv = ws.get("x_codes"), ws.get("codes_ver")
        if x_codes is not None and cv is not None and x_codes[0]._version != cv:
            if ws["x_in"] is None:
                raise RuntimeError("music_amd: the integer codes of this forward were modified in place before backward()")
            return None
        return x_codes

    def causal_wgrad(self, ws, bw, x_codes, name, dx0, CH, st, mode):
        B, T, pitch, Q, x = ws["B"], ws["T"], ws["pitch"], self.Q, ws["x_in"]
        if x_codes is not None:
            return call("wn_causal_wgrad_codes", ptr(x_codes[0]), 1 if x_codes[1] else 0, dx0, None, 0, 0, CH * pitch, pitch, CH, Q, T, B,
                        ptr(bw["slab"], bw["plan"][name + "_codes"].so), st)
        self.wgrad(bw, B, mode, st, name, dx0, CH * pitch, pitch, 0, pitch, ptr(x), ptr(x), Q * T, T, -1, 0, T, Q // 16, CH // 16, 0, 2 * Q, 1, T)

    def causal_input_grad(self, ws, dx0, CH, wpackT, mode):
        B, T, pitch, Q = ws["B"], ws["T"], ws["pitch"], self.Q
        din = torch.empty(B, Q, T, dtype=torch.float32, device=self.device)
        dx0 = ptr(dx0, SLACK)
        call("wn_chan_gemm", dx0, dx0, CH * pitch, pitch, 1, T, 0, 1, CH // 32, CH // 32, wpackT, Q // 16, Q,
             ptr(din), Q * T, T, 0, None, None, 0, 0, 0, None, 0, 0, 0, T, 0, B, mode, _lib.stream())
        return din

    def softmax_ce(self, logits, target, probs, dlogits, loss_part, n):
        call("wn_chunk_softmax256_ce", ptr(logits), ptr(target), ptr(probs), ptr(dlogits), ptr(loss_part), n, 1.0 / n, _lib.stream())

    def _resolve_objective(self, objective):
        objective = self.objective if objective is None else objective
        if objective not in OBJECTIVES:
            raise ValueError("music_amd: objective must be one of %s, not %r" % (", ".join(OBJECTIVES), objective))
        return objective

    def _resolve_windows(self, windows, window_pos=None):
        windows = self.nll_windows if windows is None else windows
        if windows is None:
            if window_pos is not None:
                raise ValueError("music_amd: window_pos is the position inside a window table: pass windows= (or set nll_windows) with it")
            return None
        return windows if isinstance(windows, NllWindows) else NllWindows(windows, self.Q)

    def step_nll(self, ws, target, dlogits=None, probs=None, row_nll=None, row_hit=None, windows=None, window_pos=None):
        B, W, Q = ws["B"], ws["W"], self.Q
        win = self._resolve_windows(windows, window_pos)
        if "loss_part" not in ws:
            ws["loss_part"] = torch.zeros(_lib.CE_NUM_PARTIALS, dtype=torch.float32, device=self.device)
        if win is None:
            call("wn_step_nll", ptr(ws["O"]), Q * W, W, ptr(target), ptr(dlogits), Q * W, W, ptr(probs), ptr(row_nll), ptr(row_hit),
                 ptr(ws["loss_part"]), W, Q, B, 1.0 / (B * W), _lib.stream())
        else:
            ws["nll_win"] = win
            call("wn_win_step_nll", ptr(ws["O"]), Q * W, W, ptr(target), ptr(dlogits), Q * W, W, ptr(probs), ptr(row_nll), ptr(row_hit),
                 ptr(ws["loss_part"]), W, Q, B, 1.0 / (B * W), *win.tail(window_pos, B, self.device), _lib.stream())
        self.mark("step_nll")

    def score_logits(self, ws, target, windows=None, window_pos=None):
        n = ws["B"] * ws["W"]
        target = target.reshape(-1)
        assert target.numel() == n and target.dtype == torch.int64 and target.is_cuda
        row_nll = torch.empty(n, dtype=torch.float32, device=self.device)
        row_hit = torch.empty(n, dtype=torch.int32, device=self.device)
        self.step_nll(ws, target, row_nll=row_nll, row_hit=row_hit, windows=windows, window_pos=window_pos)
        return row_nll, row_hit

    def step_probs(self, ws, windows=None, window_pos=None):
        B, W, Q = ws["B"], ws["W"], self.Q
        win = self._resolve_windows(windows, window_pos)
        probs = torch.empty(B * W, Q, dtype=torch.float32, device=self.device)
        if win is None:
            call("wn_step_softmax", ptr(ws["O"]), Q * W, W, ptr(probs), W, Q, B, _lib.stream())
        else:
            ws["nll_win"] = win
            call("wn_win_step_softmax", ptr(ws["O"]), Q * W, W, ptr(probs), W, Q, B, *win.tail(window_pos, B, self.device), _lib.stream())
        return probs

    def _throttled(self, step):
        self._throttle.enter()
        out = step()
        self._throttle.leave()
        return out

    def _fused_tail(self, ws, target, want_probs=False, objective=None, windows=None, window_pos=None):
        objective = self._resolve_objective(objective)
        win = self._resolve_windows(windows, window_pos)
        if win is not None and objective != "nll":
            raise ValueError('music_amd: position windows (nll_windows) apply to objective "nll" only, not %r' % objective)
        bw = self._bwd_workspace(ws)
        n = ws["B"] * ws["W"]
        target = target.reshape(-1)
        assert target.numel() == n and target.dtype == torch.int64 and target.is_cuda
        if "loss_part" not in ws:
            ws["loss_part"] = torch.zeros(_lib.CE_NUM_PARTIALS, dtype=torch.float32, device=self.device)
        probs = None
        if want_probs:
            probs = torch.empty(n, self.Q, dtype=torch.float32, device=self.device)
            ws["probs"] = probs
        if objective == "nll":
            self.step_nll(ws, target, bw["dO"], probs, windows=win, window_pos=window_pos)
        else:
            self.softmax_ce(ws["O"], target, probs, bw["dO"], ws["loss_part"], n)
        if self.vq:
            ws["vq_g"] = 1.0
            self.backward_from_dlogits(ws)
            return torch.add(ws["loss_part"].sum(), ws["vq_part"].sum(), alpha=self.vq_loss_coef)
        self.backward_from_dlogits(ws)
        return ws["loss_part"].sum()

    def adam_init(self, lr=1e-4, betas=(0.9, 0.999), eps=1e-8, max_grad_norm=None, skip_nonfinite=False, ema_decay=None,
                  ema_warmup=False):
        from . import ema
        self.adam_state = dict(m=torch.zeros_like(self.flat), v=torch.zeros_like(self.flat), t=0,
                               lr=lr, b1=betas[0], b2=betas[1], eps=eps)
        guard.adam_init_guard(self.adam_state, self.flat.device, max_grad_norm, skip_nonfinite)
        shadow = self.adam_state["ema"] = ema.make(ema_decay, ema_warmup)
        if shadow is not None:
            shadow.bind_engine(self)

    @property
    def ema(self):
        return None if self.adam_state is None else self.adam_state.get("ema")

    def guard_report(self):
        return guard.engine_guard_report(self)

    def adam_step(self, gscale=1.0):
        guard.engine_adam_step(self, gscale)
```

Measured before the change: 30.04 million.

## Fuse per-step weight packing and gradient reduce/gather plumbing into fewer kernels

Adds a multi-descriptor pack kernel that packs the forward, backward and causal-tap weight tables in one launch. It also adds a reduce-slabs variant that scatters reduced gradients straight into flat_grad through a precomputed inverse map and zeroes unreached entries, removing the separate gather kernel. The existing pack and gather kernels are vectorized to 8 or 4 elements per thread, and the causal weight gather is skipped when the multi-pack already refreshed it. The aim is to cut per-step launch count and small-kernel memory traffic. The cost is more host-side bookkeeping, such as cached descriptor tables and inverse maps built on the first call, plus generation checks that could go stale.

```diff
diff --git a/include/wavenet_hip.h b/include/wavenet_hip.h
--- a/include/wavenet_hip.h
+++ b/include/wavenet_hip.h
@@ -18,6 +18,18 @@
 
 int wn_pack_weights(const float* flat, const int32_t* idx, uint16_t* out, int n, int mode,
                     wn_stream_t stream);
+
+enum { WN_PACK_COPY32 = 4 };
+typedef struct wn_pack_desc {
+    const int32_t* idx;
+    void* out;
+    int32_t n;
+    int32_t mode;
+} wn_pack_desc;
+int wn_pack_blocks(int n);
+int wn_pack_weights_multi(const float* flat, const wn_pack_desc* desc, int ndesc, int64_t total_blocks, wn_stream_t stream);
+
+int wn_step_plumbing(int on);
 
 int wn_chan_gemm(const float* in0, const float* in1, int64_t in_bstride, int in_pitch, int in_lo, int in_hi,
                  int shift0, int shift1, int ks0, int ks1, const uint16_t* wpack, int mt, int m_valid,
@@ -110,6 +122,8 @@
                         int64_t x_bstride, int pitch, int ch, int q, int t, int batch, wn_stream_t stream);
 int wn_reduce_slabs(const int64_t* desc, int n_ops, int64_t total_vec, const float* slab, float* out,
                     wn_stream_t stream);
+int wn_reduce_slabs_to(const int64_t* desc, int n_ops, int64_t total_vec, const float* slab, float* out, const int32_t* map,
+                       float* flat_grad, const int32_t* zero_idx, int64_t n_zero, wn_stream_t stream);
 
 int wn_bias_grad(const float* a, int64_t a_bstride, int a_pitch, int a_shift, int rows, int t_lo,
                  int t_hi, int batch, float* out, wn_stream_t stream);
diff --git a/music_amd/_lib.py b/music_amd/_lib.py
--- a/music_amd/_lib.py
+++ b/music_amd/_lib.py
@@ -31,6 +31,9 @@
 SIGNATURES = {
     "wn_version": [],
     "wn_pack_weights": [_p, _p, _p, _i, _i, _p],
+    "wn_pack_blocks": [_i],
+    "wn_pack_weights_multi": [_p, _p, _i, _l, _p],
+    "wn_step_plumbing": [_i],
     "wn_chan_gemm": [_p, _p, _l, _i, _i, _i, _i, _i, _i, _i, _p, _i, _i,
                      _p, _l, _i, _i, _p,
                      _p, _l, _i, _i,
@@ -69,6 +72,7 @@
     "wn_causal_wgrad_codes_slabs": [_i, _i],
     "wn_causal_fwd_codes": [_p, _i, _p, _p, _i, _p, _l, _i, _i, _i, _i, _i, _p],
     "wn_reduce_slabs": [_p, _i, _l, _p, _p, _p],
+    "wn_reduce_slabs_to": [_p, _i, _l, _p, _p, _p, _p, _p, _l, _p],
     "wn_bias_grad": [_p, _l, _i, _i, _i, _i, _i, _i, _p, _p],
     "wn_chunk_softmax256_fwd": [_p, _p, _l, _p],
     "wn_chunk_softmax256_bwd": [_p, _p, _p, _l, _p],
@@ -138,6 +142,13 @@
                 ("stream", ctypes.c_uint32), ("seed", ctypes.c_uint64)]
 
 
+PACK_COPY32 = 4
+
+
+class PackDesc(ctypes.Structure):
+    _fields_ = [("idx", ctypes.c_void_p), ("out", ctypes.c_void_p), ("n", ctypes.c_int32), ("mode", ctypes.c_int32)]
+
+
 class GuardState(ctypes.Structure):
     _fields_ = [("norm", ctypes.c_float), ("coef", ctypes.c_float), ("nonfinite", ctypes.c_uint32), ("skip", ctypes.c_uint32),
                 ("n_taken", ctypes.c_uint64), ("n_clipped", ctypes.c_uint64), ("n_skipped", ctypes.c_uint64),
@@ -263,6 +274,14 @@
     return load().wn_resblock_bwd_pq_slabs(t_lo, t_hi, batch, d, 1 if chain else 0)
 
 
+def pack_blocks(n):
+    return load().wn_pack_blocks(n)
+
+
+def step_plumbing(on=-1):
+    return load().wn_step_plumbing(on)
+
+
 def enc_slabs(t_lo, t_hi, batch):
     return load().wn_enc_resblock_bwd_slabs(t_lo, t_hi, batch)
 
diff --git a/music_amd/csrc/wn_api.hip b/music_amd/csrc/wn_api.hip
--- a/music_amd/csrc/wn_api.hip
+++ b/music_amd/csrc/wn_api.hip
@@ -25,6 +25,17 @@
     return pr.multiProcessorCount;
 }
 
+static std::atomic<int> g_step_plumbing{-1};
+int wn_step_plumbing_on() {
+    int v = g_step_plumbing.load(std::memory_order_relaxed);
+    if (v < 0) {
+        const char* e = getenv("WN_STEP_PLUMBING");
+        v = (e && atoi(e) == 0) ? 0 : 1;
+        g_step_plumbing.store(v, std::memory_order_relaxed);
+    }
+    return v;
+}
+
 int wn_xcd_swizzle_enabled() { return 1; }
 
 int wn_set_error_msg(int code, const char* msg) {
@@ -52,6 +63,7 @@
 static_assert(WN_F16X3 == WN_MODE_F16X3 && WN_F16X1 == WN_MODE_F16X1 && WN_BF16X3 == WN_MODE_BF16X3 &&
               WN_BF16X1 == WN_MODE_BF16X1, "mode enums out of sync");
 static_assert(WN_CE_NUM_PARTIALS == WN_CE_PARTIALS, "partials out of sync");
+static_assert(sizeof(wn_pack_desc) == sizeof(WnPackDesc) && WN_PACK_COPY32 == WN_PACK_MODE_COPY32, "pack descriptor out of sync");
 static_assert(WN_VQ_NUM_PARTIALS == WN_VQ_PARTIALS && WN_VQ_MAX_CODES == WN_DEC_MAX_Q, "vq constants out of sync");
 static_assert(WN_VQ_MAX_CODES == WN_VQ_MAX_K && WN_VQ_EMA_WORK_BYTES == WN_VQ_EMA_WORK, "vq ema constants out of sync");
 static_assert(WN_RVQ_MAX_STAGES == WN_RVQ_MAX_S, "rvq constants out of sync");
@@ -193,6 +205,22 @@
     return wn_launch_pack(flat, idx, out, n, wn_mode_is_bf16(mode), wn_mode_ns(mode), (hipStream_t)stream);
 }
 
+int wn_step_plumbing(int on) {
+    const int was = wn_step_plumbing_on();
+    if (on >= 0) g_step_plumbing.store(on ? 1 : 0, std::memory_order_relaxed);
+    return was;
+}
+
+int wn_pack_blocks(int n) { return n > 0 ? (int)(((int64_t)n + WN_PACK_BLOCK - 1) / WN_PACK_BLOCK) : 0; }
+
+int wn_pack_weights_multi(const float* flat, const wn_pack_desc* desc, int ndesc, int64_t total_blocks, wn_stream_t stream) {
+    if (ndesc < 0) return wn_set_error_msg(-4, "wn_pack_weights_multi: 'ndesc' must be >= 0");
+    if (total_blocks < 0 || total_blocks > 0x7fffffffLL) return wn_set_error_msg(-4, "wn_pack_weights_multi: 'total_blocks' out of range");
+    if (ndesc > 0) WN_REQUIRE("wn_pack_weights_multi", desc);
+    if (ndesc > 0 && total_blocks > 0) WN_REQUIRE("wn_pack_weights_multi", flat);
+    return wn_launch_pack_multi(flat, reinterpret_cast<const WnPackDesc*>(desc), ndesc, (long)total_blocks, (hipStream_t)stream);
+}
+
 int wn_chan_gemm(const float* in0, const float* in1, int64_t in_bstride, int in_pitch, int in_lo, int in_hi,
                  int shift0, int shift1, int ks0, int ks1, const uint16_t* wpack, int mt, int m_valid,
                  float* out, int64_t out_bstride, int out_pitch, int out_shift, const float* bias,
@@ -348,6 +376,15 @@
     if (nrows > 0) WN_REQUIRE("wn_chunk_softmax256_ce", x, target);
     return wn_launch_softmax_ce(x, target, probs, dx, loss_part, nrows, inv_n, (hipStream_t)stream);
 }
+int wn_reduce_slabs_to(const int64_t* desc, int n_ops, int64_t total_vec, const float* slab, float* out, const int32_t* map,
+                       float* flat_grad, const int32_t* zero_idx, int64_t n_zero, wn_stream_t stream) {
+    if (n_zero < 0) return wn_set_error_msg(-4, "wn_reduce_slabs_to: 'n_zero' must be >= 0");
+    if (n_ops > 0 && total_vec > 0) WN_REQUIRE("wn_reduce_slabs_to", desc, slab, out, map, flat_grad);
+    if (n_zero > 0) WN_REQUIRE("wn_reduce_slabs_to", zero_idx, flat_grad);
+    return wn_launch_reduce_slabs_to(reinterpret_cast<const long*>(desc), n_ops, total_vec, slab, out, map, flat_grad, zero_idx,
+                                     (long)n_zero, (hipStream_t)stream);
+}
+
 int wn_adam_flat(float* p, const float* g, float* m, float* v, int64_t n, float lr, float beta1,
                  float beta2, float eps, float bias_corr1, float bias_corr2, float gscale, wn_stream_t stream) {
     if (n > 0) WN_REQUIRE("wn_adam_flat", p, g, m, v);
diff --git a/music_amd/csrc/wn_elem.hip b/music_amd/csrc/wn_elem.hip
--- a/music_amd/csrc/wn_elem.hip
+++ b/music_amd/csrc/wn_elem.hip
@@ -197,8 +197,28 @@
     WN_CHECK_LAUNCH();
     return 0;
 }
+__global__ __launch_bounds__(256) void gather_grads4_k(const float* __restrict__ packed, const int32_t* __restrict__ idx,
+                                                       float* __restrict__ flat, int n) {
+    const long i = ((long)blockIdx.x * blockDim.x + threadIdx.x) * 4;
+    if (i >= n) return;
+    if (i + 4 <= n) {
+        const u32x4 s = *reinterpret_cast<const u32x4*>(idx + i);
+        f32x4 r;
+#pragma unroll
+        for (int k = 0; k < 4; ++k) r[k] = (int)s[k] >= 0 ? packed[(int)s[k]] : 0.f;
+        *reinterpret_cast<f32x4*>(flat + i) = r;
+    } else {
+        for (long k = i; k < n; ++k) flat[k] = idx[k] >= 0 ? packed[idx[k]] : 0.f;
+    }
+}
 int wn_launch_gather_grads(const float* packed, const int32_t* idx, float* flat_grad, int n, hipStream_t st) {
     if (n <= 0) return 0;
+    if (wn_step_plumbing_on() && (((uintptr_t)idx | (uintptr_t)flat_grad) & 15) == 0) {
+        const long groups = ((long)n + 3) / 4;
+        hipLaunchKernelGGL(gather_grads4_k, dim3((unsigned)((groups + 255) / 256)), dim3(256), 0, st, packed, idx, flat_grad, n);
+        WN_CHECK_LAUNCH();
+        return 0;
+    }
     hipLaunchKernelGGL(gather_grads_k, dim3((n + 255) / 256), dim3(256), 0, st, packed, idx, flat_grad, n);
     WN_CHECK_LAUNCH();
     return 0;
diff --git a/music_amd/csrc/wn_gemm.hip b/music_amd/csrc/wn_gemm.hip
--- a/music_amd/csrc/wn_gemm.hip
+++ b/music_amd/csrc/wn_gemm.hip
@@ -19,12 +19,124 @@
     }
 }
 
+template <class T>
+__device__ __forceinline__ void pack8(const float* __restrict__ flat, const int32_t* __restrict__ idx, uint16_t* __restrict__ out,
+                                      long p, int ns) {
+    const u32x4 i0 = *reinterpret_cast<const u32x4*>(idx + p), i1 = *reinterpret_cast<const u32x4*>(idx + p + 4);
+    float v[8];
+#pragma unroll
+    for (int j = 0; j < 8; ++j) {
+        const int src = (int)(j < 4 ? i0[j] : i1[j - 4]);
+        v[j] = src >= 0 ? flat[src] : 0.0f;
+    }
+    uint16_t h16[8], l16[8];
+#pragma unroll
+    for (int j = 0; j < 8; ++j) {
+        const typename T::elem h = T::cvt(v[j]);
+        h16[j] = __builtin_bit_cast(uint16_t, h);
+        const typename T::elem l = T::cvt(v[j] - T::back(h));
+        l16[j] = __builtin_bit_cast(uint16_t, l);
+    }
+    u32x4 hv, lv;
+#pragma unroll
+    for (int j = 0; j < 4; ++j) {
+        hv[j] = (uint32_t)h16[2 * j] | ((uint32_t)h16[2 * j + 1] << 16);
+        lv[j] = (uint32_t)l16[2 * j] | ((uint32_t)l16[2 * j + 1] << 16);
+    }
+    const size_t o = (size_t)(p >> 9) * (ns == 3 ? 1024 : 512) + (size_t)(p & 511);
+    *reinterpret_cast<u32x4*>(out + o) = hv;
+    if (ns == 3) *reinterpret_cast<u32x4*>(out + o + 512) = lv;
+}
+template <class T>
+__device__ __forceinline__ void pack_tail(const float* __restrict__ flat, const int32_t* __restrict__ idx, uint16_t* __restrict__ out,
+                                          long p, long n, int ns) {
+    for (long e = p; e < n && e < p + 8; ++e) {
+        const int src = idx[e];
+        const float v = src >= 0 ? flat[src] : 0.0f;
+        const typename T::elem h = T::cvt(v);
+        const size_t o = (size_t)(e >> 9) * (ns == 3 ? 1024 : 512) + (size_t)(e & 511);
+        out[o] = __builtin_bit_cast(uint16_t, h);
+        if (ns == 3) {
+            const typename T::elem l = T::cvt(v - T::back(h));
+            out[o + 512] = __builtin_bit_cast(uint16_t, l);
+        }
+    }
+}
+
+template <class T>
+__global__ __launch_bounds__(256) void pack_weights8_k(const float* __restrict__ flat, const int32_t* __restrict__ idx,
+                                                       uint16_t* __restrict__ out, int n, int ns) {
+    const long p = ((long)blockIdx.x * blockDim.x + threadIdx.x) * 8;
+    if (p + 8 <= n) pack8<T>(flat, idx, out, p, ns);
+    else pack_tail<T>(flat, idx, out, p, n, ns);
+}
+
+static __host__ __device__ inline bool wn_aligned16(const void* a, const void* b) { return (((uintptr_t)a | (uintptr_t)b) & 15) == 0; }
+
 int wn_launch_pack(const float* flat, const int32_t* idx, uint16_t* out, int n, int is_bf16, int ns,
                    hipStream_t st) {
     if (n <= 0) return 0;
+    if (wn_step_plumbing_on() && wn_aligned16(idx, out)) {
+        dim3 g((unsigned)(((long)n + 2047) / 2048)), b(256);
+        if (is_bf16) hipLaunchKernelGGL(pack_weights8_k<BF16>, g, b, 0, st, flat, idx, out, n, ns);
+        else hipLaunchKernelGGL(pack_weights8_k<F16>, g, b, 0, st, flat, idx, out, n, ns);
+        WN_CHECK_LAUNCH();
+        return 0;
+    }
     dim3 g((n + 255) / 256), b(256);
     if (is_bf16) hipLaunchKernelGGL(pack_weights_k<BF16>, g, b, 0, st, flat, idx, out, n, ns);
     else hipLaunchKernelGGL(pack_weights_k<F16>, g, b, 0, st, flat, idx, out, n, ns);
+    WN_CHECK_LAUNCH();
+    return 0;
+}
+
+__global__ __launch_bounds__(256) void pack_multi_k(const float* __restrict__ flat, const WnPackDesc* __restrict__ desc, int ndesc) {
+    long b = blockIdx.x;
+    WnPackDesc e;
+    int d = 0;
+    for (; d < ndesc; ++d) {
+        e = desc[d];
+        const long nb = e.n > 0 ? ((long)e.n + 2047) / 2048 : 0;
+        if (b < nb) break;
+        b -= nb;
+    }
+    if (d == ndesc) return;
+    const long n = e.n, p = b * 2048 + (long)threadIdx.x * 8;
+    if (p >= n) return;
+    const bool whole = p + 8 <= n && wn_aligned16(e.idx, e.out);
+    if (e.mode == WN_PACK_MODE_COPY32) {
+        float* out = reinterpret_cast<float*>(e.out);
+        if (whole) {
+            const u32x4 i0 = *reinterpret_cast<const u32x4*>(e.idx + p), i1 = *reinterpret_cast<const u32x4*>(e.idx + p + 4);
+            f32x4 v0, v1;
+#pragma unroll
+            for (int j = 0; j < 4; ++j) {
+                const int s0 = (int)i0[j], s1 = (int)i1[j];
+                v0[j] = s0 >= 0 ? flat[s0] : 0.f;
+                v1[j] = s1 >= 0 ? flat[s1] : 0.f;
+            }
+            *reinterpret_cast<f32x4*>(out + p) = v0;
+            *reinterpret_cast<f32x4*>(out + p + 4) = v1;
+        } else {
+            for (long k = p; k < n && k < p + 8; ++k) out[k] = e.idx[k] >= 0 ? flat[e.idx[k]] : 0.f;
+        }
+        return;
+    }
+    uint16_t* out = reinterpret_cast<uint16_t*>(e.out);
+    const int ns = (e.mode == WN_MODE_F16X3 || e.mode == WN_MODE_BF16X3) ? 3 : 1;
+    const bool bf = e.mode == WN_MODE_BF16X3 || e.mode == WN_MODE_BF16X1;
+    if (whole) {
+        if (bf) pack8<BF16>(flat, e.idx, out, p, ns);
+        else pack8<F16>(flat, e.idx, out, p, ns);
+    } else {
+        if (bf) pack_tail<BF16>(flat, e.idx, out, p, n, ns);
+        else pack_tail<F16>(flat, e.idx, out, p, n, ns);
+    }
+}
+
+int wn_launch_pack_multi(const float* flat, const WnPackDesc* desc, int ndesc, long total_blocks, hipStream_t st) {
+    if (ndesc <= 0 || total_blocks <= 0) return 0;
+    hipLaunchKernelGGL(pack_multi_k, dim3((unsigned)total_blocks), dim3(256), 0, st, flat, desc, ndesc);
     WN_CHECK_LAUNCH();
     return 0;
 }
diff --git a/music_amd/csrc/wn_kernels.h b/music_amd/csrc/wn_kernels.h
--- a/music_amd/csrc/wn_kernels.h
+++ b/music_amd/csrc/wn_kernels.h
@@ -54,6 +54,13 @@
 int wn_launch_enc_resblock_fwd(const WnResArgs& a, int ch, int batch, int mode, hipStream_t st);
 int wn_launch_pack(const float* flat, const int32_t* idx, uint16_t* out, int n, int is_bf16, int ns,
                    hipStream_t st);
+int wn_step_plumbing_on();
+struct WnPackDesc {
+    const int32_t* idx; void* out;
+    int32_t n, mode;
+};
+enum { WN_PACK_MODE_COPY32 = 4, WN_PACK_BLOCK = 2048 };
+int wn_launch_pack_multi(const float* flat, const WnPackDesc* desc, int ndesc, long total_blocks, hipStream_t st);
 
 struct WnResArgs {
     const float* x_in; float* x_out; float* z_out;
@@ -167,6 +174,8 @@
 int wn_launch_wgrad2(const WnWgradArgs* a1, const WnWgradArgs* a2, int batch, int mode, hipStream_t st);
 int wn_wgrad_num_slabs(int t_lo, int t_hi, int chunk, int batch);
 int wn_launch_reduce_slabs(const long* desc, int n_ops, long total_vec, const float* slab, float* out, hipStream_t st);
+int wn_launch_reduce_slabs_to(const long* desc, int n_ops, long total_vec, const float* slab, float* out, const int32_t* map,
+                              float* flat, const int32_t* zero_idx, long n_zero, hipStream_t st);
 
 int wn_launch_causal_wgrad_codes(const int32_t* codes, int scrambled, const float* dx, const float* dxq, int dn, int p_lo,
                                  long dx_bstride, int pitch, int ch, int T, int batch, float* slab, hipStream_t st);
diff --git a/music_amd/csrc/wn_wgrad.hip b/music_amd/csrc/wn_wgrad.hip
--- a/music_amd/csrc/wn_wgrad.hip
+++ b/music_amd/csrc/wn_wgrad.hip
@@ -393,9 +393,17 @@
     return wn_launch_wgrad2(&a, nullptr, batch, mode, st);
 }
 
+template <bool TO>
 __global__ __launch_bounds__(256) void reduce_slabs_k(const long* __restrict__ desc, int n_ops, long total_vec,
-                                                      const float* __restrict__ slab, float* __restrict__ out) {
+                                                      const float* __restrict__ slab, float* __restrict__ out,
+                                                      const int32_t* __restrict__ map, float* __restrict__ flat,
+                                                      const int32_t* __restrict__ zero_idx, long n_zero) {
     long v = (long)blockIdx.x * blockDim.x + threadIdx.x;
+    if (TO && v >= total_vec) {
+        const long z = v - total_vec;
+        if (z < n_zero) flat[zero_idx[z]] = 0.f;
+        return;
+    }
     if (v >= total_vec) return;
     int lo = 0, hi = n_ops - 1;
     while (lo < hi) {
@@ -422,19 +430,46 @@
         for (; i < ns; ++i) s8[0] += ld4u(sp + (size_t)i * stride);
         const f32x4 s = ((s8[0] + s8[1]) + (s8[2] + s8[3])) + ((s8[4] + s8[5]) + (s8[6] + s8[7]));
         op[0] = s[0]; op[1] = s[1]; op[2] = s[2]; op[3] = s[3];
+        if (TO) {
+            const int32_t* mp = map + d[4] + e;
+            const int t0 = mp[0], t1 = mp[1], t2 = mp[2], t3 = mp[3];
+            if (t0 >= 0 && ((uintptr_t)(flat + t0) & 15) == 0 && t1 == t0 + 1 && t2 == t0 + 2 && t3 == t0 + 3) {
+                *reinterpret_cast<f32x4*>(flat + t0) = s;
+            } else {
+                if (t0 >= 0) flat[t0] = s[0];
+                if (t1 >= 0) flat[t1] = s[1];
+                if (t2 >= 0) flat[t2] = s[2];
+                if (t3 >= 0) flat[t3] = s[3];
+            }
+        }
     } else {
         for (long k = 0; e + k < n; ++k) {
             float s = 0.f;
             for (int i = 0; i < ns; ++i) s += sp[(size_t)i * stride + k];
             op[k] = s;
+            if (TO) {
+                const int to = map[d[4] + e + k];
+                if (to >= 0) flat[to] = s;
+            }
         }
     }
 }
 
 int wn_launch_reduce_slabs(const long* desc, int n_ops, long total_vec, const float* slab, float* out, hipStream_t st) {
     if (total_vec <= 0 || n_ops <= 0) return 0;
-    hipLaunchKernelGGL(reduce_slabs_k, dim3((unsigned)((total_vec + 255) / 256)), dim3(256), 0, st, desc, n_ops,
-                       total_vec, slab, out);
+    hipLaunchKernelGGL(reduce_slabs_k<false>, dim3((unsigned)((total_vec + 255) / 256)), dim3(256), 0, st, desc, n_ops,
+                       total_vec, slab, out, (const int32_t*)nullptr, (float*)nullptr, (const int32_t*)nullptr, 0L);
     WN_CHECK_LAUNCH();
     return 0;
 }
+
+int wn_launch_reduce_slabs_to(const long* desc, int n_ops, long total_vec, const float* slab, float* out, const int32_t* map,
+                              float* flat, const int32_t* zero_idx, long n_zero, hipStream_t st) {
+    if (total_vec <= 0 || n_ops <= 0) total_vec = 0;
+    if (n_zero < 0) n_zero = 0;
+    if (total_vec + n_zero <= 0) return 0;
+    hipLaunchKernelGGL(reduce_slabs_k<true>, dim3((unsigned)((total_vec + n_zero + 255) / 256)), dim3(256), 0, st, desc, n_ops,
+                       total_vec, slab, out, map, flat, zero_idx, n_zero);
+    WN_CHECK_LAUNCH();
+    return 0;
+}
diff --git a/music_amd/engine.py b/music_amd/engine.py
--- a/music_amd/engine.py
+++ b/music_amd/engine.py
@@ -142,8 +142,14 @@
         self.wt_idx = torch.from_numpy(causal.taps).to(dev)
         self.wt = torch.zeros(causal.taps.size, dtype=torch.float32, device=dev)
 
-    def pack_weights(self):
+    def pack_weights(self, codes=False):
         st = _lib.stream()
+        if self.step_plumbing >= 2:
+            tabs = [(self.pk_f_idx, self.pk_f, self.mode_fwd), (self.pk_b_idx, self.pk_b, self.mode_bwd)]
+            if codes:
+                tabs.append((self.wt_idx, self.wt, _lib.PACK_COPY32))
+                self._wt_fresh = (self.wt.data_ptr(), self._gen + 1)
+            return self.pack_all(tabs, st)
         call("wn_pack_weights", ptr(self.flat), ptr(self.pk_f_idx), ptr(self.pk_f), self.pk_f_idx.numel(), self.mode_fwd, st)
         call("wn_pack_weights", ptr(self.flat), ptr(self.pk_b_idx), ptr(self.pk_b), self.pk_b_idx.numel(), self.mode_bwd, st)
 
@@ -316,7 +322,7 @@
     def loss_and_grad(self, x, target, want_probs=False, codes=None, objective=None, windows=None, window_pos=None):
         def step():
             self.mark("begin")
-            self.pack_weights()
+            self.pack_weights(codes=x is None or getattr(x, "_wn_codes", None) is not None)
             self.mark("pack")
             return self._fused_tail(self.forward_logits(x, codes=codes), target, want_probs, objective, windows, window_pos)
         return self._throttled(step)
diff --git a/music_amd/engine_base.py b/music_amd/engine_base.py
--- a/music_amd/engine_base.py
+++ b/music_amd/engine_base.py
@@ -1,4 +1,5 @@
 import ctypes
+import os
 import weakref
 from collections import namedtuple
 
@@ -244,6 +245,10 @@
         self._throttle = _lib.StepThrottle()
         self._side = None
         self.overlap_wgrad = True
+        self.step_plumbing = int(os.environ.get("WN_STEP_PLUMBING", "1") or 1)
+        self._pack_tab = {}
+        self._wt_fresh = None
+        self._inv_gather = None
 
     def mark(self, name):
         if self.marks is not None and (self.mark_only is None or name in self.mark_only):
@@ -492,11 +497,44 @@
         self.on_side(lambda s2: self.wgrad(bw, B, mode, s2, name, *args))
 
     def reduce_and_gather(self, bw, from_codes, st):
-        call("wn_reduce_slabs", ptr(bw["desc_codes"] if from_codes else bw["desc"]), bw["nops"], bw["vec"], ptr(bw["slab"]), ptr(self.gpack), st)
+        desc = bw["desc_codes"] if from_codes else bw["desc"]
+        to = self._reduce_to(bw) if self.step_plumbing >= 2 and not bw["pair"] else None
+        if to is not None:
+            return call("wn_reduce_slabs_to", ptr(desc), bw["nops"], bw["vec"], ptr(bw["slab"]), ptr(self.gpack), ptr(to[0]),
+                        ptr(self.flat_grad), ptr(to[1]), to[1].numel(), st)
+        call("wn_reduce_slabs", ptr(desc), bw["nops"], bw["vec"], ptr(bw["slab"]), ptr(self.gpack), st)
         if bw["pair"]:
             call("wn_gather_grads2", ptr(self.gpack), ptr(self.gidx_pa), ptr(self.gidx_pb), ptr(self.flat_grad), self.n_gather, st)
         else:
             call("wn_gather_grads", ptr(self.gpack), ptr(self.gidx), ptr(self.flat_grad), self.n_gather, st)
+
+    def _reduce_to(self, bw):
+        if "reduce_to" in bw:
+            return bw["reduce_to"]
+        gidx = self.gidx[:self.n_gather].cpu().numpy().astype(np.int64)
+        src = gidx[gidx >= 0]
+        ok = not getattr(self, "gp_bias_off", None) and len(np.unique(src)) == len(src)
+        if ok:
+            inv = np.full(self.gpack.numel(), -1, dtype=np.int32)
+            inv[src] = np.nonzero(gidx >= 0)[0]
+            reached = np.zeros(self.gpack.numel(), dtype=bool)
+            for _, _, _, _, out_off, n in bw["desc"].cpu().numpy().reshape(-1, 6).tolist():
+                reached[out_off:out_off + n] = True
+            clear = np.nonzero((gidx < 0) | ~reached[np.maximum(gidx, 0)])[0].astype(np.int32)
+            dev = self.flat_grad.device
+            bw["reduce_to"] = (torch.from_numpy(inv).to(dev), torch.from_numpy(clear).to(dev))
+        else:
+            bw["reduce_to"] = None
+        return bw["reduce_to"]
+
+    def pack_all(self, entries, st):
+        key = tuple((i.data_ptr(), o.data_ptr(), i.numel(), m) for i, o, m in entries)
+        if key not in self._pack_tab:
+            tab = (_lib.PackDesc * len(entries))(*[_lib.PackDesc(i.data_ptr(), o.data_ptr(), i.numel(), m) for i, o, m in entries])
+            dev = torch.frombuffer(bytearray(bytes(tab)), dtype=torch.uint8).to(self.flat.device)
+            self._pack_tab[key] = (dev, len(entries), sum(_lib.pack_blocks(i.numel()) for i, _, _ in entries))
+        dev, nd, blocks = self._pack_tab[key]
+        call("wn_pack_weights_multi", ptr(self.flat), ptr(dev), nd, blocks, st)
 
     @staticmethod
     def tagged_codes(x, B, T):
@@ -514,7 +552,8 @@
             return call("wn_chan_gemm", ptr(x), ptr(x), Q * T, T, 0, T, -1, 0, Q // 32, Q // 32, wpack, CH // 16, R, out, CH * pitch, pitch, 0, bias,
                         None, 0, 0, 0, None, 0, 0, 1, T, 0, B, mode, st)
         codes, scrambled = ws["x_codes"]
-        call("wn_gather_grads", ptr(self.flat), ptr(wt_idx), ptr(wt), wt.numel(), st)
+        if self._wt_fresh != (wt.data_ptr(), self._gen):
+            call("wn_gather_grads", ptr(self.flat), ptr(wt_idx), ptr(wt), wt.numel(), st)
         call("wn_causal_fwd_codes", ptr(codes), 1 if scrambled else 0, ptr(wt), bias, R, out, CH * pitch, pitch, CH, Q, T, B, st)
 
     def codes_for_backward(self, ws):
```

Result: no change. 30.01 million (-0.1%).
